# syamajala/cholesky

Measured on AMD Instinct MI355X. Metric: fp64 factorization GF/s (numeric level loop, F_ref flops) on 3-D Laplacian, higher is better.
Workload: dtype f64; 1 GPU; tests/lapl_3375x3375 (reference fixture: 7-point Laplacian, nested-dissection ordering from the fixture files); n=3375, levels=5, separators=31, B_alg_bytes=2932064, parallelism=single GPU, precision=fp64

## Files before the change

### cholesky_amd/_lib.py

```python
import ctypes as C
import os

_HERE = os.path.dirname(os.path.abspath(__file__))
LIB_PATH = os.environ.get("CHOLAMD_LIB") or os.path.join(_HERE, "lib", "libcholamd.so")
HEADER_PATH = os.path.join(os.path.dirname(_HERE), "include", "cholamd.h")


class Filled(C.Structure):
    _fields_ = [("filled", C.c_int), ("sep_x", C.c_int), ("sep_y", C.c_int), ("interval", C.c_int), ("cluster", C.c_int),
                ("lo_x", C.c_int), ("lo_y", C.c_int), ("hi_x", C.c_int), ("hi_y", C.c_int)]


class Op(C.Structure):
    _fields_ = [("op", C.c_int), ("level", C.c_int), ("m", C.c_int), ("n", C.c_int), ("k", C.c_int),
                ("a_sx", C.c_int), ("a_sy", C.c_int), ("a_z", C.c_int), ("b_sx", C.c_int), ("b_sy", C.c_int), ("b_z", C.c_int),
                ("c_sx", C.c_int), ("c_sy", C.c_int), ("c_z", C.c_int)]


class Region(C.Structure):
    _fields_ = [("ptr", C.c_void_p), ("ld", C.c_int), ("lo_x", C.c_int), ("lo_y", C.c_int), ("hi_x", C.c_int), ("hi_y", C.c_int),
                ("tile_row", C.POINTER(C.c_int))]


class SepInfo(C.Structure):
# ... 22 lines not shown
    L.cholamd_read_clusters.argtypes = [C.c_char_p, vp, vp, vp, i64, C.POINTER(i64)]
    L.cholamd_read_matrix.argtypes = [C.c_char_p, ci, vp, vp, vp]
    L.cholamd_read_vector.argtypes = [C.c_char_p, ci, vp]
    L.cholamd_write_solution.argtypes = [C.c_char_p, vp, ci, ci]
    L.cholamd_plan_create.argtypes = [C.c_char_p, C.c_char_p, C.c_char_p, C.POINTER(vp)]
    L.cholamd_plan_create_from_arrays.argtypes = [ci, ci, vp, vp, vp, vp, vp, i64, i64, vp, vp, vp, C.c_char_p, C.POINTER(vp)]
    L.cholamd_plan_destroy.argtypes = [vp]
    L.cholamd_generate_laplacian.argtypes = [ci, ci, ci, ci, ci, C.POINTER(vp)]
    L.cholamd_problem_destroy.argtypes = [vp]
    L.cholamd_problem_n.argtypes = [vp]
    L.cholamd_problem_nz.argtypes = [vp]
    L.cholamd_problem_write.argtypes = [vp, C.c_char_p]
    L.cholamd_plan_create_from_problem.argtypes = [vp, C.POINTER(vp)]
    L.cholamd_problem_rhs.argtypes = [vp, vp]
    for f in ("n", "nz", "levels", "num_separators", "max_int_size", "num_blocks"):
        getattr(L, "cholamd_plan_" + f).argtypes = [vp]
    for f in ("arena_doubles", "dropped_entries", "num_ops", "nnz_a", "nnz_l", "alg_bytes"):
        fn = getattr(L, "cholamd_plan_" + f)
        fn.argtypes = [vp]
        fn.restype = i64
    L.cholamd_plan_nnz_tiles.argtypes = [vp]
    L.cholamd_plan_nnz_tiles.restype = i64
    L.cholamd_plan_fmin.argtypes = [vp]
    L.cholamd_plan_fmin.restype = cd
    L.cholamd_plan_banner.argtypes = [vp]
    L.cholamd_plan_banner.restype = C.c_char_p
    for f in ("perm", "sep_sizes", "sep_offsets", "tree", "blocks", "ops"):
        getattr(L, "cholamd_plan_" + f).argtypes = [vp, vp]
    L.cholamd_plan_snapshot_count.argtypes = [vp, ci]
    L.cholamd_plan_snapshot_count.restype = i64
    L.cholamd_plan_snapshot.argtypes = [vp, ci, vp]
    L.cholamd_plan_counts.argtypes = [vp, ci, vp, vp]
    L.cholamd_plan_flops.argtypes = [vp]
    L.cholamd_plan_flops.restype = cd
    L.cholamd_plan_fill_host.argtypes = [vp, vp]
    L.cholamd_plan_arena_to_dense.argtypes = [vp, vp, vp]
    L.cholamd_plan_entries.argtypes = [vp, vp, vp]
    L.cholamd_plan_value_map.argtypes = [vp, vp]
    L.cholamd_plan_fill_host_values.argtypes = [vp, vp, i64, vp]
    L.cholamd_device_set_values.argtypes = [vp, vp, i64, ci, vp]
    L.cholamd_device_values_status.argtypes = [vp, vp, vp]
    L.cholamd_plan_fill_host_part.argtypes = [vp, vp, ci, ci, C.POINTER(i64)]
    L.cholamd_plan_level_work_counts.argtypes = [vp, ci, ci, ci, vp]
    L.cholamd_plan_level_work_volume.argtypes = [vp, ci, ci, ci, ci, vp]
    L.cholamd_plan_program_check.argtypes = [vp, ci, ci]
    L.cholamd_plan_program_check_opts.argtypes = [vp, ci, ci, ci, ci]
    L.cholamd_plan_program_counts.argtypes = [vp, ci, vp]
    L.cholamd_plan_program_jobs.argtypes = [vp, ci, i64, vp]
    L.cholamd_plan_program_jobs.restype = i64
    L.cholamd_plan_write_matrix.argtypes = [vp, vp, C.c_char_p, ci]
    L.cholamd_plan_write_debug_log.argtypes = [vp, vp]
    L.cholamd_device_create.argtypes = [vp, ci, C.POINTER(vp)]
    L.cholamd_device_destroy.argtypes = [vp]
    L.cholamd_device_set_partition.argtypes = [vp, ci, ci]
    L.cholamd_device_set_option.argtypes = [vp, C.c_char_p, ci]
    L.cholamd_comm_unique_id.argtypes = [vp]
    L.cholamd_comm_create.argtypes = [vp, ci, ci, vp, C.POINTER(vp)]
    L.cholamd_comm_create_local.argtypes = [vp, ci, vp]
    L.cholamd_factor_multi.argtypes = [vp, vp, vp, ci, vp]
    L.cholamd_gather_factor.argtypes = [vp, vp, ci, vp]
    L.cholamd_comm_adopt.argtypes = [vp, ci, ci, C.POINTER(vp)]
    L.cholamd_comm_destroy.argtypes = [vp]
    L.cholamd_comm_destroy.restype = None
    L.cholamd_comm_allreduce.argtypes = [vp, vp, i64, vp]
    L.cholamd_device_tail_offset.argtypes = [vp]
    L.cholamd_device_tail_offset.restype = i64
    L.cholamd_exchange_tail.argtypes = [vp, vp, vp, vp]
    L.cholamd_factor_sharded.argtypes = [vp, vp, vp, vp]
    L.cholamd_factor_sharded_f32.argtypes = [vp, vp, vp, vp]
    L.cholamd_gather_to_root.argtypes = [vp, vp, ci, vp, vp]
    L.cholamd_exchange_volume.argtypes = [vp, vp]
    L.cholamd_plan_exchange_volume.argtypes = [vp, ci, ci, ci, vp]
    L.cholamd_plan_exchange_pieces.argtypes = [vp, ci, ci, ci, vp]
    L.cholamd_plan_solve_counts.argtypes = [vp, ci, ci, ci, vp]
    L.cholamd_plan_solve_skips.argtypes = [vp, ci, vp, vp]
    L.cholamd_solve_sharded.argtypes = [vp, vp, vp, vp, vp, vp]
    L.cholamd_solve_sharded_f32.argtypes = [vp, vp, vp, vp, vp, vp]
    L.cholamd_solve_refine_sharded.argtypes = [vp, vp, vp, vp, ci, C.c_double, vp, vp, vp, vp]
    L.cholamd_solve_multi.argtypes = [vp, vp, vp, vp, vp, ci, vp]
    L.cholamd_solve_refine_multi.argtypes = [vp, vp, vp, vp, ci, C.c_double, vp, vp, vp, ci, vp]
    L.cholamd_follow_rounds.argtypes = [ci, ci, ci, vp, vp]
    L.cholamd_plan_program_followers.argtypes = [vp, i64, vp]
    L.cholamd_plan_program_followers.restype = i64
    L.cholamd_factor_multi_f32.argtypes = [vp, vp, vp, ci, vp]
    L.cholamd_gather_factor_f32.argtypes = [vp, vp, ci, vp]
    L.cholamd_device_alloc.argtypes = [vp, i64, C.POINTER(vp)]
    L.cholamd_device_free.argtypes = [vp, vp]
    L.cholamd_device_upload.argtypes = [vp, vp, vp, i64, vp]
    L.cholamd_device_download.argtypes = [vp, vp, vp, i64, vp]
    L.cholamd_device_sync.argtypes = [vp, vp]
    L.cholamd_device_fill.argtypes = [vp, vp, vp]
    L.cholamd_factor.argtypes = [vp, vp, vp]
    L.cholamd_factor_levels.argtypes = [vp, vp, ci, ci, vp]
    L.cholamd_device_program_trace.argtypes = [vp, vp, vp, i64, vp, C.POINTER(ci)]
    L.cholamd_debug_live_buffers.argtypes = []
    L.cholamd_debug_live_buffers.restype = i64
    L.cholamd_factor_info.argtypes = [vp, C.POINTER(ci)]
    L.cholamd_solve.argtypes = [vp, vp, vp, vp, vp]
    L.cholamd_device_fill_f32.argtypes = [vp, vp, vp]
    L.cholamd_factor_f32.argtypes = [vp, vp, vp]
    L.cholamd_factor_levels_f32.argtypes = [vp, vp, ci, ci, vp]
    L.cholamd_solve_f32.argtypes = [vp, vp, vp, vp, vp]
    L.cholamd_solve_refine.argtypes = [vp, vp, vp, vp, ci, cd, C.POINTER(ci), C.POINTER(cd), vp]
    L.cholamd_residual.argtypes = [vp, vp, vp, vp, C.POINTER(cd), vp]
    L.cholamd_solve_nrhs.argtypes = [vp, vp, vp, i64, vp, i64, ci, vp]
    L.cholamd_solve_nrhs_f32.argtypes = [vp, vp, vp, i64, vp, i64, ci, vp]
    L.cholamd_solve_refine_nrhs.argtypes = [vp, vp, vp, i64, vp, i64, ci, ci, cd, C.POINTER(ci), vp, vp]
    L.cholamd_apply.argtypes = [vp, vp, vp, vp]
    L.cholamd_apply_nrhs.argtypes = [vp, vp, i64, vp, i64, ci, vp]
    L.cholamd_plan_apply_host.argtypes = [vp, vp, vp, vp]
    for name in ("cholamd_solve_pcg", "cholamd_solve_pcg_f32"):
        getattr(L, name).argtypes = [vp, vp, vp, vp, ci, cd, ci, vp, vp, vp, vp]
    for name in ("cholamd_solve_pcg_nrhs", "cholamd_solve_pcg_nrhs_f32"):
        getattr(L, name).argtypes = [vp, vp, vp, i64, vp, i64, ci, ci, cd, ci, vp, vp, vp, vp]
    L.cholamd_solve_half.argtypes = [vp, vp, vp, vp, ci, vp]
    L.cholamd_solve_half_f32.argtypes = [vp, vp, vp, vp, ci, vp]
    L.cholamd_solve_half_nrhs.argtypes = [vp, vp, vp, i64, vp, i64, ci, ci, vp]
    L.cholamd_solve_half_nrhs_f32.argtypes = [vp, vp, vp, i64, vp, i64, ci, ci, vp]
    for name in ("cholamd_multiply_half", "cholamd_multiply_half_f32"):
        getattr(L, name).argtypes = [vp, vp, vp, vp, ci, vp]
    for name in ("cholamd_multiply", "cholamd_multiply_f32"):
        getattr(L, name).argtypes = [vp, vp, vp, vp, vp]
    for name in ("cholamd_factor_residual", "cholamd_factor_residual_f32"):
        getattr(L, name).argtypes = [vp, vp, vp, C.POINTER(cd), vp]
    for name in ("cholamd_multiply_half_nrhs", "cholamd_multiply_half_nrhs_f32"):
        getattr(L, name).argtypes = [vp, vp, vp, i64, vp, i64, ci, ci, vp]
    for name in ("cholamd_multiply_nrhs", "cholamd_multiply_nrhs_f32"):
        getattr(L, name).argtypes = [vp, vp, vp, i64, vp, i64, ci, vp]
    L.cholamd_plan_multiply_host.argtypes = [vp, vp, ci, vp, vp]
    L.cholamd_plan_multiply_host_nrhs.argtypes = [vp, vp, ci, vp, i64, vp, i64, ci]
    L.cholamd_plan_multiply_counts.argtypes = [vp, vp]
    L.cholamd_plan_solve_det_host.argtypes = [vp, vp, ci, vp, vp]
    L.cholamd_plan_solve_det_host_nrhs.argtypes = [vp, vp, ci, vp, i64, vp, i64, ci]
    L.cholamd_plan_solve_det_counts.argtypes = [vp, vp]
    L.cholamd_plan_solve_det_lists.argtypes = [vp, ci, vp, vp, vp]
    L.cholamd_factor_logdet.argtypes = [vp, vp, C.POINTER(cd), vp]
    L.cholamd_factor_logdet_f32.argtypes = [vp, vp, C.POINTER(cd), vp]
    L.cholamd_factor_diag.argtypes = [vp, vp, vp, vp]
    L.cholamd_factor_diag_f32.argtypes = [vp, vp, vp, vp]
    L.cholamd_plan_diag_list.argtypes = [vp, vp, vp, vp, vp, vp, vp]
    L.cholamd_selinv.argtypes = [vp, vp, vp, vp]
    L.cholamd_selinv_diag.argtypes = [vp, vp, vp, vp]
    L.cholamd_selinv_entries.argtypes = [vp, vp, vp, i64, vp]
    L.cholamd_plan_selinv_blocks.argtypes = [vp, ci]
    L.cholamd_plan_selinv_front.argtypes = [vp, ci, ci, ci, vp, vp, vp]
    L.cholamd_values_grad_pairs.argtypes = [vp, vp, i64, vp, i64, ci, cd, cd, vp, i64, vp]
    L.cholamd_values_grad_logdet.argtypes = [vp, vp, cd, cd, vp, i64, vp]
    L.cholamd_plan_values_grad_pairs_host.argtypes = [vp, vp, i64, vp, i64, ci, cd, cd, vp, i64]
    L.cholamd_plan_values_grad_logdet_host.argtypes = [vp, vp, cd, cd, vp, i64]
    L.cholamd_plan_duplicate_entries.argtypes = [vp]
    L.cholamd_plan_duplicate_entries.restype = i64
    L.cholamd_plan_schur_size.argtypes = [vp, ci]
    L.cholamd_plan_schur_dofs.argtypes = [vp, ci, vp]
    L.cholamd_plan_schur_list.argtypes = [vp, ci, i64, vp]
    L.cholamd_plan_schur_host.argtypes = [vp, ci, vp, vp, i64]
    L.cholamd_schur_factor.argtypes = [vp, vp, ci, vp]
    L.cholamd_schur.argtypes = [vp, vp, ci, vp, i64, vp]
    for f in (L.cholamd_schur_condense, L.cholamd_schur_condense_f32, L.cholamd_schur_expand, L.cholamd_schur_expand_f32):
        f.argtypes = [vp, vp, ci, vp, vp, vp, vp]
    for f in (L.cholamd_schur_condense_nrhs, L.cholamd_schur_condense_nrhs_f32, L.cholamd_schur_expand_nrhs, L.cholamd_schur_expand_nrhs_f32):
        f.argtypes = [vp, vp, ci, vp, i64, vp, i64, vp, i64, ci, vp]
    L.cholamd_device_schur_launches.argtypes = [vp, vp]
    L.cholamd_plan_schur_condense_host_nrhs.argtypes = [vp, ci, vp, vp, i64, vp, i64, vp, i64, ci]
    L.cholamd_plan_schur_expand_host_nrhs.argtypes = [vp, ci, vp, vp, i64, vp, i64, vp, i64, ci]
    L.cholamd_plan_schur_det_counts.argtypes = [vp, ci, vp]
    L.cholamd_plan_schur_det_lists.argtypes = [vp, ci, ci, vp, vp, vp]
# ... 66 lines not shown
```

### cholesky_amd/csrc/chol_api.cpp

```cpp
#include "chol_device.h"

int no_device_error()
{
  chol_set_error("no usable HIP device (libcholamd has no CPU fallback)");
  return CHOLAMD_ERR_NO_DEVICE;
}
bool ranges_overlap(const void *a, size_t na, const void *b, size_t nb)
{
  const char *pa = (const char *)a, *pb = (const char *)b;
  return pa < pb + nb && pb < pa + na;
}

extern "C" int cholamd_device_count(void)
{
  int n = 0;
  if (hipGetDeviceCount(&n) != hipSuccess) return 0;
  return n;
}

#define CHOL_POISON_GUARD ((size_t)64 << 10)
static bool poison_on()
{
  const char *e = std::getenv("CHOLAMD_POISON");
  return e && *e && atoi(e) != 0;
// ... 109 lines not shown
      d->prog_ready = d->n_job > 0;
    }
  }
  return 0;
}

extern "C" int cholamd_device_create(const cholamd_plan *plan, int device_id, cholamd_device **out)
{
  *out = nullptr;
  if (!plan) { chol_set_error("null plan"); return CHOLAMD_ERR_ARG; }
  int ndev = 0;
  if (hipGetDeviceCount(&ndev) != hipSuccess || ndev <= 0) return no_device_error();
  if (device_id < 0 || device_id >= ndev) { chol_set_error("device %d out of range (%d devices)", device_id, ndev); return CHOLAMD_ERR_NO_DEVICE; }
  HIPCHK(hipSetDevice(device_id));
  cholamd_device *d = new cholamd_device();
  d->plan = plan; d->dev = device_id;
  chol_sched_opts_from_env(&d->opt);
  { const char *e = getenv("CHOLAMD_SOLVE_REFERENCE_SHAPE"); d->solve_reference_shape = e && *e && atoi(e) != 0; }
  { const char *e = getenv("CHOLAMD_SOLVE_DETERMINISTIC"); d->solve_deterministic = e && *e && atoi(e) != 0; }
  { const char *e = getenv("CHOLAMD_SOLVE_DETERMINISTIC_BLOCK"); d->solve_deterministic_block = e && *e && atoi(e) != 0; }
  { const char *e = getenv("CHOLAMD_SCHUR_DETERMINISTIC"); d->schur_deterministic = e && *e && atoi(e) != 0; }
  { const char *e = getenv("CHOLAMD_MULTIPLY_NRHS_MIN"); d->multiply_nrhs_min = e && *e ? atoi(e) : 0; }
  int rc = build_levels(d);
  if (!rc) rc = d->ws.alloc((size_t)(plan->ws_doubles > 0 ? plan->ws_doubles : 1));
  if (!rc) rc = d->info.alloc_zero(4);
  if (!rc) rc = d->progress.alloc_zero((size_t)(plan->nsep + 2));
  if (!rc) rc = d->a_dst.upload(plan->a_dst, (size_t)plan->nnz_a);
  if (!rc) rc = d->a_val.upload(plan->a_val, (size_t)plan->nnz_a);
  if (!rc) rc = d->perm.upload(plan->perm, (size_t)plan->n);
  if (rc) { cholamd_device_destroy(d); return rc; }
  *out = d;
  return 0;
}

extern "C" void cholamd_device_destroy(cholamd_device *d)
{
  if (!d) return;
  (void)hipSetDevice(d->dev);
  for (auto &a : d->vmm) {
    (void)hipDeviceSynchronize();
    (void)hipMemUnmap(a.va, a.total);
    for (auto h : a.handles) (void)hipMemRelease(h);
    (void)hipMemAddressFree(a.va, a.total);
  }
  for (auto &t : d->tl) { d->pool.push_back(t.a); d->pool.push_back(t.b); }
  for (auto e : d->pool) (void)hipEventDestroy(e);
  delete d;
}

extern "C" int cholamd_device_set_partition(cholamd_device *d, int rank, int world)
{
  HIPCHK(hipSetDevice(d->dev));
  if (world < 1 || (world & (world - 1)) || rank < 0 || rank >= world || chol_split_level(world) > d->plan->levels - 1) {
    chol_set_error("bad partition: rank %d of %d for a %d-level tree", rank, world, d->plan->levels);
    return CHOLAMD_ERR_ARG;
  }
  d->rank = rank; d->world = world;
  free_solve_lists(d);
  return build_levels(d);
}

extern "C" int cholamd_device_bcast_phases(const cholamd_device *d)
{
  int n = 0;
  for (const level_dev &l : d->lv) for (const chol_phase &ph : l.phase) n += ph.kind == 6;
  return n;
}
extern "C" int cholamd_device_set_option(cholamd_device *d, const char *name, int value)
{
  HIPCHK(hipSetDevice(d->dev));
  const std::string n(name ? name : "");
  bool rebuild = true;
  if (n == "split_min") d->opt.split_min = value;
  else if (n == "split_nb") d->opt.split_nb = value;
  else if (n == "fuse") d->opt.fuse = value != 0;
  else if (n == "fuse_update_max") d->opt.fuse_update_max = value;
  else if (n == "mt_min_tiles") d->opt.mt_min_tiles = value;
  else if (n == "cells") d->opt.cells = value != 0;
  else if (n == "program") d->opt.program = value != 0;
  else if (n == "follow") d->opt.follow = value != 0;
  else if (n == "super_blocks") d->opt.super_blocks = value;
  else if (n == "follow_tail") d->opt.follow_tail = value;
  else if (n == "follow_tail_split") d->opt.follow_tail_split = value;
  else if (n == "staged") d->opt.staged = value != 0;
  else if (n == "fine_upd") d->opt.fine_upd = value != 0;
  else if (n == "skyline") d->opt.skyline = value != 0;
  else if (n == "merge_targets") d->opt.merge_targets = value != 0;
  else if (n == "leaf_envelope") d->opt.leaf_envelope = value != 0;
  else if (n == "trsm_wt_min") d->opt.trsm_wt_min = value < 0 ? 0 : value;
  else if (n == "stage_chunk") d->opt.stage_chunk = value < 0 ? 0 : value;
  else if (n == "dist_top") d->opt.dist_top = value;
  else if (n == "solve_reference_shape") { d->solve_reference_shape = value != 0; rebuild = false; }
  else if (n == "solve_deterministic") { d->solve_deterministic = value != 0; rebuild = false; }
  else if (n == "solve_deterministic_block") { d->solve_deterministic_block = value != 0; rebuild = false; }
  else if (n == "schur_deterministic") { d->schur_deterministic = value != 0; rebuild = false; }
  else if (n == "multiply_nrhs_min") { d->multiply_nrhs_min = value; rebuild = false; }
  else { chol_set_error("unknown option '%s'", n.c_str()); return CHOLAMD_ERR_ARG; }
  return rebuild ? build_levels(d) : 0;
}

extern "C" int cholamd_device_alloc(cholamd_device *d, int64_t doubles, double **dptr)
{
  HIPCHK(hipSetDevice(d->dev));
  HIPCHK(fp_malloc((void **)dptr, (size_t)doubles * sizeof(double)));
  return 0;
}
extern "C" int cholamd_device_free(cholamd_device *d, double *dptr)
{
  HIPCHK(hipSetDevice(d->dev));
  HIPCHK(hipFree(dptr));
  return 0;
}
extern "C" int cholamd_device_upload(cholamd_device *d, double *d_dst, const double *h_src, int64_t doubles, void *stream)
{
  HIPCHK(hipSetDevice(d->dev));
  HIPCHK(hipMemcpyAsync(d_dst, h_src, (size_t)doubles * sizeof(double), hipMemcpyHostToDevice, (hipStream_t)stream));
  HIPCHK(hipStreamSynchronize((hipStream_t)stream));
  return 0;
}
extern "C" int cholamd_device_download(cholamd_device *d, double *h_dst, const double *d_src, int64_t doubles, void *stream)
{
  HIPCHK(hipSetDevice(d->dev));
  HIPCHK(hipMemcpyAsync(h_dst, d_src, (size_t)doubles * sizeof(double), hipMemcpyDeviceToHost, (hipStream_t)stream));
  HIPCHK(hipStreamSynchronize((hipStream_t)stream));
  return 0;
}
extern "C" int cholamd_device_sync(cholamd_device *d, void *stream)
{
  HIPCHK(hipSetDevice(d->dev));
  HIPCHK(hipStreamSynchronize((hipStream_t)stream));
  return 0;
}

static void owned_ranges(const cholamd_device *d, std::vector<std::pair<int64_t, int64_t>> &out)
{
  const cholamd_plan *p = d->plan;
  out.clear();
  if (d->world <= 1 || d->rank == 0) { out.push_back({ 0, p->arena }); return; }
  for (int s = 1; s <= p->nsep; s++) {
    const int o = chol_owner_of(p, s, d->world);
    if (o >= 0 && o != d->rank) continue;
    const int64_t lo = p->panel_off[s], hi = s < p->nsep ? p->panel_off[s + 1] : p->arena;
    if (!out.empty() && out.back().second == lo) out.back().second = hi; else out.push_back({ lo, hi });
  }
}
static int clear_owned(cholamd_device *d, void *arena, size_t elem, hipStream_t st)
{
  bool sharded = false;
  for (const auto &v : d->vmm) if (v.va == arena) sharded = true;
  if (!sharded) { HIPCHK(hipMemsetAsync(arena, 0, (size_t)d->plan->arena * elem, st)); return 0; }
  std::vector<std::pair<int64_t, int64_t>> r;
  owned_ranges(d, r);
  for (auto &x : r) HIPCHK(hipMemsetAsync((char *)arena + (size_t)x.first * elem, 0, (size_t)(x.second - x.first) * elem, st));
  return 0;
}
#define CHOL_VMM_CHUNK ((size_t)2 << 20)
#define CHOL_VMM_SCRATCH ((size_t)64 << 20)
extern "C" int cholamd_device_alloc_arena(cholamd_device *d, int elem_bytes, void **dptr, int64_t *backed_bytes)
{
  HIPCHK(hipSetDevice(d->dev));
  if (elem_bytes != 4 && elem_bytes != 8) { chol_set_error("alloc_arena: element size %d", elem_bytes); return CHOLAMD_ERR_ARG; }
  const size_t full = (size_t)d->plan->arena * (size_t)elem_bytes;
  if (d->world <= 1 || d->rank == 0) {
    HIPCHK(fp_malloc(dptr, full > 0 ? full : 1));
    if (backed_bytes) *backed_bytes = (int64_t)full;
    return 0;
// ... 1880 lines not shown
```

### cholesky_amd/csrc/chol_kernels.hip

```cpp
#include <hip/hip_runtime.h>
#include <float.h>
#include <stdint.h>

#include "chol_plan.h"
#include "chol_kernels.h"

typedef double d4 __attribute__((ext_vector_type(4)));

__device__ __forceinline__ void lds_barrier()
{
  asm volatile("s_waitcnt lgkmcnt(0)\n\ts_barrier" ::: "memory");
}


template <bool PUB> __device__ __forceinline__ void gstore(double *p, double v)
{
  if (PUB) __hip_atomic_store(p, v, __ATOMIC_RELAXED, __HIP_MEMORY_SCOPE_AGENT);
  else *p = v;
}
template <bool PUB> __device__ __forceinline__ double gload(const double *p)
{
  if (PUB) return __hip_atomic_load(p, __ATOMIC_RELAXED, __HIP_MEMORY_SCOPE_AGENT);
  return *p;
}
// ... 727 lines not shown
{
  while (__builtin_amdgcn_readfirstlane(__hip_atomic_load(flag, __ATOMIC_RELAXED, __HIP_MEMORY_SCOPE_WORKGROUP)) < target)
    __builtin_amdgcn_s_sleep(1);
  asm volatile("" ::: "memory");
}
__device__ __forceinline__ int lds_wait_ge_v(int *flag, int target)
{
  int v;
  while ((v = __builtin_amdgcn_readfirstlane(__hip_atomic_load(flag, __ATOMIC_RELAXED, __HIP_MEMORY_SCOPE_WORKGROUP))) < target)
    __builtin_amdgcn_s_sleep(1);
  asm volatile("" ::: "memory");
  return v;
}
__device__ __forceinline__ void lds_wait_both_ge(int *pair, int target)
{
  for (;;) {
    const long long v = __hip_atomic_load((long long *)pair, __ATOMIC_RELAXED, __HIP_MEMORY_SCOPE_WORKGROUP);
    const int lo = __builtin_amdgcn_readfirstlane((int)v), hi = __builtin_amdgcn_readfirstlane((int)(v >> 32));
    if (lo >= target && hi >= target) break;
    __builtin_amdgcn_s_sleep(1);
  }
  asm volatile("" ::: "memory");
}
__device__ __forceinline__ void lds_set(int *flag, int value, int lane)
{
  asm volatile("s_waitcnt lgkmcnt(0)" ::: "memory");
  if (lane == 0) __hip_atomic_store(flag, value, __ATOMIC_RELAXED, __HIP_MEMORY_SCOPE_WORKGROUP);
}
__device__ __forceinline__ void lds_wait_set(int *flag, int *info, int lane)
{
  for (int it = 0; __builtin_amdgcn_readfirstlane(__hip_atomic_load(flag, __ATOMIC_RELAXED, __HIP_MEMORY_SCOPE_WORKGROUP)) == 0; ++it) {
    if (it >= (1 << 25)) { if (lane == 0) report_stall(info); break; }
    __builtin_amdgcn_s_sleep(1);
  }
  asm volatile("" ::: "memory");
}
__device__ __forceinline__ void lds_inc(int *cnt, int lane)
{
  asm volatile("s_waitcnt lgkmcnt(0)" ::: "memory");
  if (lane == 0) __hip_atomic_fetch_add(cnt, 1, __ATOMIC_RELAXED, __HIP_MEMORY_SCOPE_WORKGROUP);
}
template <bool PUB> __device__ __forceinline__ d4 load_tile(const double *A, int lda, int n, int ti, int tj, int r15, int g)
{
  const int row = ti * TS + r15;
  const bool rowok = row < n;
  const double *src = A + row + (int64_t)(tj * TS + g) * lda;
  d4 v;
#pragma unroll
  for (int q = 0; q < 4; ++q) {
    const int c = g + 4 * q, col = tj * TS + c;
    double e = (row == col) ? 1.0 : 0.0;
    if (rowok && col < n) e = (ti > tj || c <= r15) ? gload<PUB>(&src[(int64_t)(4 * q) * lda]) : 0.0;
    v[q] = e;
  }
  return v;
}
#define FOLLOW_SLOTS 4
#define FOLLOW_LOADS ((CHOL_FOLLOW_MAXT * TS * TS + RR_THREADS - 1) / RR_THREADS)
template <int SLEEP = 0>
__device__ __forceinline__ void wait_list(const chol_wait *__restrict__ wl, int n, const int *ctr, const int *__restrict__ ctr_total, int epoch, int lane, int *info)
{
  for (int b0 = 0; b0 < n; b0 += 64) {
    int c = 0, need = 0;
    const bool mine = b0 + lane < n;
    if (mine) { const chol_wait wt = wl[b0 + lane]; c = wt.ctr; need = wt.value + epoch * ctr_total[wt.ctr]; }
    for (int it = 0;; ++it) {
      const bool ok = !mine || __hip_atomic_load(&ctr[c], __ATOMIC_RELAXED, __HIP_MEMORY_SCOPE_AGENT) >= need;
      if (!__ballot(!ok)) break;
      if (it >= (1 << 21)) { if (lane == 0) report_stall(info); break; }
#ifndef WAIT_SLEEP
#define WAIT_SLEEP 32
#endif
      __builtin_amdgcn_s_sleep(SLEEP ? SLEEP : WAIT_SLEEP);
    }
  }
}
__device__ __forceinline__ bool wait_list_holds(const chol_wait *__restrict__ wl, int n, const int *ctr, const int *__restrict__ ctr_total, int epoch, int lane)
{
  bool ok = true;
  for (int b0 = 0; b0 < n; b0 += 64)
    if (b0 + lane < n) { const chol_wait wt = wl[b0 + lane]; ok = ok && __hip_atomic_load(&ctr[wt.ctr], __ATOMIC_RELAXED, __HIP_MEMORY_SCOPE_AGENT) >= wt.value + epoch * ctr_total[wt.ctr]; }
  return !__ballot(!ok);
}
struct follow_args { const chol_ext *ext; int n_ext; const int *ctr; const int *ctr_total; int epoch; const chol_wait *wl; int n_wl; unsigned long long *stamp, *xstamp; };
__device__ __forceinline__ int ext_ready(const follow_args &f, int from, int lane)
{
  bool ok = true;
  if (from + lane < f.n_ext) {
    const int c = f.ext[from + lane].ctr;
    ok = __hip_atomic_load(&f.ctr[c], __ATOMIC_RELAXED, __HIP_MEMORY_SCOPE_AGENT) - f.epoch * f.ctr_total[c] >= f.ext[from + lane].need;
  }
  const unsigned long long notok = __ballot(!ok);
  const int lead = notok ? __builtin_ctzll(notok) : 64;
  return min(from + lead, f.n_ext);
}
template <bool UPD, bool PUB, bool TR = false>
__device__ __forceinline__ void follow_external(const double *__restrict__ base, const follow_args f, int T, int n, double *sE, d4 (&tile)[11], d4 (&stage)[3],
                                                const int (&ijp)[12], int w, int lane, int tid, int *info, const double *A, int lda, int r15, int g, int *sReady)
{
  const int lp = lane;
  int buf = 0;
  int ready = 0, ng = 0;
  double va[FOLLOW_LOADS], vb[FOLLOW_LOADS];
#ifndef FOLLOW_OWN_SLEEP
#define FOLLOW_OWN_SLEEP 4
#endif
#ifndef FOLLOW_OWN_LAST_MAX
#define FOLLOW_OWN_LAST_MAX 0
#endif
  static_assert(CHOL_FOLLOW_PAIR_MAXT == RR_MAXT, "a pair of followed column tiles shares one LDS buffer of RR_MAXT tiles");
  const int own_at = f.n_ext <= FOLLOW_OWN_LAST_MAX ? f.n_ext : chol_follow_own_at(f.n_ext, T);
#define EXT_ROUND(I_) chol_follow_round(I_, f.n_ext, T)
#define EXT_LOAD(I_, V_)                                                                                             \
  {                                                                                                                  \
    const chol_ext xl_ = f.ext[I_];                                                                                  \
    const double *src_ = base + xl_.off;                                                                             \
    _Pragma("unroll") for (int it = 0; it < FOLLOW_LOADS; ++it) {                                                    \
      const int idx = tid + it * RR_THREADS;                                                                         \
      const int row = (idx >> 8) * TS + (idx & 15), col = (idx >> 4) & 15;                                           \
      V_[it] = (idx < T * TS * TS && row < n && col < xl_.ncol) ? gload<true>(&src_[row + (int64_t)col * xl_.ld]) : 0.0; \
    }                                                                                                                \
  }
#define EXT_LOAD_ROUND(I_)                                                                                           \
  {                                                                                                                  \
    EXT_LOAD(I_, va);                                                                                                \
    ng = EXT_ROUND(I_);                                                                                              \
    if (ng == 2) { EXT_LOAD((I_) + 1, vb); }                                                                         \
  }
#define EXT_UPDATE(acc_, ti_, tj_)                                                                                   \
  {                                                                                                                  \
    _Pragma("unroll") for (int st = 0; st < 4; ++st)                                                                 \
      acc_ = __builtin_amdgcn_mfma_f64_16x16x4f64(sB[(tj_) * (TS * TS) + st * 64 + lp], -sB[(ti_) * (TS * TS) + st * 64 + lp], acc_, 0, 0, 0); \
    if (G == 2) {                                                                                                    \
      _Pragma("unroll") for (int st = 0; st < 4; ++st)                                                               \
        acc_ = __builtin_amdgcn_mfma_f64_16x16x4f64(sB2[(tj_) * (TS * TS) + st * 64 + lp], -sB2[(ti_) * (TS * TS) + st * 64 + lp], acc_, 0, 0, 0); \
    }                                                                                                                \
  }
#define OWN_TILES()                                                                                                  \
  {                                                                                                                  \
  \
      if (!UPD) wait_list<FOLLOW_OWN_SLEEP>(f.wl, f.n_wl, f.ctr, f.ctr_total, f.epoch, lane, info);  \
      if (TR && !UPD && f.xstamp && lane == 0) f.xstamp[0] = __builtin_amdgcn_s_memrealtime(); \
      lds_barrier(); \
      if (UPD) { \
        int rx = r15, gx = g;  \
        asm volatile("" : "+v"(rx), "+v"(gx)); \
    _Pragma("unroll")                                                                                            \
        for (int it = 0; it < 3; ++it) { \
          const int u = min(w + it * RR_NW, 2 * T - 2); \
          stage[it] += load_tile<PUB>(A, lda, n, u < T ? u : u - T + 1, u < T ? 0 : 1, rx, gx); \
        } \
        __builtin_amdgcn_sched_barrier(0);  \
    _Pragma("unroll")                                                                                            \
        for (int s = 0; s < FOLLOW_SLOTS; ++s) \
          if (ijp[s] != 0xffff) tile[s] += load_tile<PUB>(A, lda, n, ijp[s] & 0xff, ijp[s] >> 8, rx, gx); \
        __builtin_amdgcn_sched_barrier(0); \
      } \
 \
  }
  for (int i = 0; i < f.n_ext;) {
    if (f.n_wl > 0 && i == own_at) OWN_TILES();
    if (ng == 0) {
      const int need = i + EXT_ROUND(i);
      if (ready < need) {
        if (!UPD) {
          ready = ext_ready(f, i, lane);
          for (int it = 0; ready < need; ++it) {
            if (it >= (1 << 24)) { if (lane == 0) report_stall(info); ready = f.n_ext; break; }
#ifndef EXT_SLEEP
#define EXT_SLEEP 4
#endif
            __builtin_amdgcn_s_sleep(EXT_SLEEP);
            ready = ext_ready(f, i, lane);
          }
          if (lane == 0) __hip_atomic_store(sReady, ready, __ATOMIC_RELAXED, __HIP_MEMORY_SCOPE_WORKGROUP);
        } else {
          for (int it = 0;; ++it) {
            ready = __builtin_amdgcn_readfirstlane(__hip_atomic_load(sReady, __ATOMIC_RELAXED, __HIP_MEMORY_SCOPE_WORKGROUP));
            if (ready >= need) break;
            if (it >= (1 << 25)) { if (lane == 0) report_stall(info); ready = f.n_ext; break; }
            __builtin_amdgcn_s_sleep(2);
          }
        }
      }
      EXT_LOAD_ROUND(i);
    }
    const int G = ng;
    if (TR && !UPD && f.xstamp && lane == 0 && i < 44) { f.xstamp[1] = f.n_ext; f.xstamp[2 + i] = __builtin_amdgcn_s_memrealtime(); }
    double *sB = sE + buf * (RR_MAXT * TS * TS), *sB2 = sB + T * TS * TS;
#pragma unroll
    for (int it = 0; it < FOLLOW_LOADS; ++it) {
      const int idx = tid + it * RR_THREADS;
      if (idx < T * TS * TS) { sB[idx] = va[it]; if (G == 2) sB2[idx] = vb[it]; }
    }
    const int j = i + G;
    ng = 0;
    int pv = 0, pneed = 0;
    bool polled = false;
    if (j < f.n_ext && j + EXT_ROUND(j) <= ready) { EXT_LOAD_ROUND(j); }
    else if (j < f.n_ext && !UPD) {
      polled = true;
      if (j + lane < f.n_ext) { const int c = f.ext[j + lane].ctr; pv = __hip_atomic_load(&f.ctr[c], __ATOMIC_RELAXED, __HIP_MEMORY_SCOPE_AGENT); pneed = f.epoch * f.ctr_total[c] + f.ext[j + lane].need; }
    }
    lds_barrier();
    if (UPD) {
#pragma unroll
      for (int it = 0; it < 3; ++it) {
        const int u = w + it * RR_NW;
        if (u < 2 * T - 1) { const int tj = u < T ? 0 : 1, ti = u < T ? u : u - T + 1; EXT_UPDATE(stage[it], ti, tj); }
      }
#pragma unroll
      for (int s = 0; s < FOLLOW_SLOTS; ++s)
        if (ijp[s] != 0xffff) { const int ti = ijp[s] & 0xff, tj = ijp[s] >> 8; EXT_UPDATE(tile[s], ti, tj); }
    }
    buf ^= 1;
    if (polled) {
      const unsigned long long notok = __ballot(j + lane < f.n_ext && pv < pneed);
      const int r2 = min(j + (notok ? __builtin_ctzll(notok) : 64), f.n_ext);
      if (r2 > ready) { ready = r2; if (lane == 0) __hip_atomic_store(sReady, ready, __ATOMIC_RELAXED, __HIP_MEMORY_SCOPE_WORKGROUP); }
    } else if (UPD && j < f.n_ext && ready < j + EXT_ROUND(j)) {
      const int r2 = __builtin_amdgcn_readfirstlane(__hip_atomic_load(sReady, __ATOMIC_RELAXED, __HIP_MEMORY_SCOPE_WORKGROUP));
      ready = r2 > ready ? r2 : ready;
    }
    i = j;
  }
  if (f.n_wl > 0 && own_at >= f.n_ext) OWN_TILES();
#undef OWN_TILES
#undef EXT_LOAD_ROUND
#undef EXT_ROUND
#undef EXT_UPDATE
#undef EXT_LOAD
}

template <bool PUB, bool FOLLOW = false, bool TR = false>
__device__ __forceinline__ void potrf_rr_body(double *__restrict__ base, double *__restrict__ ws, const chol_potrf_desc d, int *__restrict__ info,
                                              int *__restrict__ progress, int progress_base, double *smem, const unsigned char *__restrict__ sky, const follow_args fa = follow_args(), const int tid = threadIdx.x)
{
  double (*const sRaw)[TS * TS] = (double (*)[TS * TS])(smem);
  double (*const sSol)[RR_MAXT][TS * TS] = (double (*)[RR_MAXT][TS * TS])(smem + RR_OFF_SOL);
  double (*const sDg)[TS * TS] = (double (*)[TS * TS])(smem + RR_OFF_DG);
  double (*const sLW)[4 * TS][TS + 1] = (double (*)[4 * TS][TS + 1])(smem + RR_OFF_LW);
  double (*const sConv)[TS + 1] = (double (*)[TS + 1])(smem + RR_OFF_CONV);
  double (*const sOv)[TS * TS] = (double (*)[TS * TS])(smem + RR_OFF_OV);
  unsigned short *const sIJ = (unsigned short *)(smem + RR_OFF_IJ);
  int *const sFlag = (int *)(smem + RR_OFF_FLAG);
  unsigned char *const sKm = (unsigned char *)(smem + RR_OFF_KM);
  int *const sMask = (int *)(smem + RR_OFF_MASK);
  unsigned char *const sSky = (unsigned char *)(smem + RR_OFF_SKY);
  int *const fL = &sFlag[0], *const fP = &sFlag[1], *const cSol = &sFlag[2], *const cUpd = &sFlag[3];
  int *const cRaw = &sFlag[4];
  int *const fA = &sFlag[6];
  int *const fD = &sFlag[7];
  int *const f00 = &sFlag[8];

  double *A = base + d.a_off;
  double *W = ws + d.dinv_off;
  const int n = d.n, lda = d.lda;
  const int T = (n + TS - 1) / TS;
  const int ntl = T * (T + 1) / 2;
  const int lane = tid & 63;
  const int wave = __builtin_amdgcn_readfirstlane(tid >> 6);
  const int r15 = lane & 15, g = lane >> 4;
  const int lp0 = g * TS + r15;

#define PSTAMP(i_) do { if (TR && fa.xstamp && fa.n_ext == 0 && tid == 64) fa.xstamp[24 + (i_)] = __builtin_amdgcn_s_memrealtime(); } while (0)
  PSTAMP(0);
  d4 stage[3];
  const bool stage_early = !(FOLLOW && fa.n_ext > 0) && wave != 0;
  if (stage_early) {
#pragma unroll
    for (int it = 0; it < 3; ++it) {
      const int u = min(wave - 1 + it * RR_NW, 2 * T - 2);
      stage[it] = load_tile<PUB>(A, lda, n, u < T ? u : u - T + 1, u < T ? 0 : 1, r15, g);
    }
  }
  const unsigned char *const tab = d.tab > 0 ? sky - __builtin_offsetof(chol_potrf_desc, sky) + d.tab : nullptr;
  if (tab) {
    static_assert((RR_MAXT * RR_NW) % 1 == 0 && RR_THREADS >= RR_MAXT * RR_NW + RR_SLOTS * RR_NW / 2 + RR_SLOTS * RR_NW / 4, "one pass copies the tables");
    if (tid < RR_MAXT * RR_NW) sMask[tid] = ((const int *)(tab + CHOL_RR_TAB_MASK))[tid];
    else if (tid < RR_MAXT * RR_NW + RR_SLOTS * RR_NW / 2) ((int *)sIJ)[tid - RR_MAXT * RR_NW] = ((const int *)(tab + CHOL_RR_TAB_IJ))[tid - RR_MAXT * RR_NW];
    else if (tid < RR_MAXT * RR_NW + RR_SLOTS * RR_NW / 2 + RR_SLOTS * RR_NW / 4) ((int *)sKm)[tid - RR_MAXT * RR_NW - RR_SLOTS * RR_NW / 2] = ((const int *)(tab + CHOL_RR_TAB_KM))[tid - RR_MAXT * RR_NW - RR_SLOTS * RR_NW / 2];
  } else {
    for (int t = tid; t < RR_SLOTS * RR_NW; t += RR_THREADS) { sIJ[t] = (unsigned short)0xffff; sKm[t] = 0; }
    for (int t = tid; t < RR_MAXT * RR_NW; t += RR_THREADS) sMask[t] = 0;
  }
  if (tid < 24) sSky[tid] = sky[tid];
  if (tid < 10) sFlag[tid] = 0;
  if (tid < TS * TS) sConv[TS + (tid >> 4)][tid & 15] = (tid >> 4) == (tid & 15) ? 1.0 : 0.0;
  __syncthreads();
  PSTAMP(1);
  const int ntl2 = (T - 2) * (T - 1) / 2;
  if (!tab) {
  for (int t = tid + 2 * T - 1; t < ntl; t += RR_THREADS) {
    int ti, tj, ow, os;
    tile_of_index(t, T, ti, tj);
    rr_owner(ntl - 1 - t, ntl2, ow, os);
    sIJ[os * RR_NW + ow] = (unsigned short)(ti | (tj << 8));
    const int kmin = max(sky[min(ti, 23)], sky[min(tj, 23)]);
    sKm[os * RR_NW + ow] = kmin | (tj < sky[min(ti, 23)] ? CHOL_RR_KM_ZERO : 0);
    const int last = ti == tj ? tj - 2 : tj - 1;
    for (int k = min(kmin, last); k <= last; ++k) atomicOr(&sMask[k * RR_NW + ow], 1 << os);
  }
  for (int t = tid; t < T * T; t += RR_THREADS) {
    const int k = t / T, i = t % T;
    if (i >= k + 2 && sky[min(i, 23)] <= k) {
      const int hv = i % RR_NHEAVY;
      atomicOr(&sMask[k * RR_NW + hv + hv / 3], 1 << (i < k + 2 + RR_NHEAVY ? RR_M_SOLVE0 : RR_M_SOLVE1));
    }
  }
  __syncthreads();
  }
  PSTAMP(2);

  if (wave == 0) {
    __builtin_amdgcn_s_setprio(3);
    if (FOLLOW && fa.n_ext > 0) {
      d4 tdummy[RR_RSLOTS], sdummy[3];
      int idummy[RR_SLOTS];
      follow_external<false, PUB, TR>(base, fa, T, n, smem + RR_OFF_SOL, tdummy, sdummy, idummy, 0, lane, tid, info, A, lda, r15, g, &sFlag[5]);
      lds_barrier();
      if (TR && fa.stamp && lane == 0) *fa.stamp = __builtin_amdgcn_s_memrealtime();
    }
    __builtin_amdgcn_s_setprio(3);
    lds_wait_ge(f00, 1);
    d4 dk;
#pragma unroll
    for (int q = 0; q < 4; ++q) dk[q] = sDg[0][q * 64 + lp0];
    STAMP_DECL;
    POLL_DECL;
    for (int k = 0; k < T; ++k) {
      STAMPK(0);
      double a[TS], unused;
#pragma unroll
      for (int q = 0; q < 4; ++q) sConv[r15][g + 4 * q] = dk[q];
#pragma unroll
      for (int c = 0; c < TS; ++c) a[c] = sConv[lane & 31][c];
      const int cupd_early = __hip_atomic_load(cUpd, __ATOMIC_RELAXED, __HIP_MEMORY_SCOPE_WORKGROUP);
      STAMPK(1);
      if (TR && fa.xstamp && lane == 0 && k < 24) fa.xstamp[72 + k] = __builtin_amdgcn_s_memrealtime();
      const bool more = k + 1 < T;
      const int kn = more ? k + 1 : k;
      long long fl = 0;
      d4 raw, dn;
      const int bad = chol16_rows(a, unused, r15, [&]() {
        fl = __hip_atomic_load((long long *)fA, __ATOMIC_RELAXED, __HIP_MEMORY_SCOPE_WORKGROUP);
        asm volatile("" ::: "memory");
#pragma unroll
        for (int q = 0; q < 4; ++q) { raw[q] = sRaw[kn][q * 64 + lp0]; dn[q] = sDg[kn & 1][q * 64 + lp0]; }
      });
      STAMPK(2);
      if (bad && k * TS + bad <= n && lane == 0) {
        if (atomicCAS(&info[0], 0, d.col0 + k * TS + bad) == 0) info[1] = d.sep;
      }
      const int par = k & 1;
      if (__builtin_amdgcn_readfirstlane(cupd_early) < RR_NW * k) { POLL_ADD(2, 1); lds_wait_ge(cUpd, RR_NW * k); }
#pragma unroll
      for (int c = 0; c < TS; ++c) sLW[par][lane][c] = a[c];
      double wv[4];
#pragma unroll
      for (int st = 0; st < 4; ++st) wv[st] = sLW[par][TS + 4 * st + g][r15];
      lds_set(fL, k + 1, lane);
      STAMPK(3);
      if (!more) break;
      if (__builtin_amdgcn_readfirstlane((int)fl) < k + 1 || __builtin_amdgcn_readfirstlane((int)(fl >> 32)) < k + 1) {
        POLL_ADD(0, 1);
        lds_wait_both_ge(fA, k + 1);
#pragma unroll
        for (int q = 0; q < 4; ++q) { raw[q] = sRaw[k + 1][q * 64 + lp0]; dn[q] = sDg[(k + 1) & 1][q * 64 + lp0]; }
      }
      STAMPK(4);
      const d4 p = solve16(raw, wv);
#pragma unroll
      for (int q = 0; q < 4; ++q) sSol[par][k + 1][q * 64 + lp0] = p[q];
#pragma unroll
      for (int st = 0; st < 4; ++st) dn = __builtin_amdgcn_mfma_f64_16x16x4f64(p[st], -p[st], dn, 0, 0, 0);
      __builtin_amdgcn_sched_barrier(0);
      lds_set(fP, k + 1, lane);
      STAMPK(5);
      dk = dn;
      STAMPK(6);
    }
    STAMP_FLUSH;
    POLL_FLUSH;
    __builtin_amdgcn_s_setprio(0);
  } else {
    d4 tile[RR_RSLOTS];
    const int w = wave - 1;
    const int hw = rr_heavy_index(w);
    int ijp[RR_SLOTS];
#pragma unroll
    for (int s = 0; s < RR_SLOTS; ++s) ijp[s] = __builtin_amdgcn_readfirstlane((int)sIJ[s * RR_NW + w]);
    int kmn[RR_SLOTS];
#pragma unroll
    for (int s = 0; s < RR_SLOTS; ++s) kmn[s] = __builtin_amdgcn_readfirstlane((int)sKm[s * RR_NW + w]);
    unsigned zmask = 0;
#pragma unroll
    for (int s = 0; s < RR_SLOTS; ++s) { zmask |= (kmn[s] & CHOL_RR_KM_ZERO) ? 1u << s : 0u; kmn[s] &= CHOL_RR_KM_ZERO - 1; }
    PSTAMP(5);

    if (FOLLOW && fa.n_ext > 0) {
      const bool early = fa.n_wl == 0;
      const d4 zero4 = { 0.0, 0.0, 0.0, 0.0 };
#pragma unroll
      for (int it = 0; it < 3; ++it) {
        const int u = min(w + it * RR_NW, 2 * T - 2);
        stage[it] = zero4;
        if (early) stage[it] = load_tile<PUB>(A, lda, n, u < T ? u : u - T + 1, u < T ? 0 : 1, r15, g);
      }
#pragma unroll
      for (int s = 0; s < FOLLOW_SLOTS; ++s) {
        d4 v = zero4;
        if (early && ijp[s] != 0xffff) v = load_tile<PUB>(A, lda, n, ijp[s] & 0xff, ijp[s] >> 8, r15, g);
        tile[s] = v;
      }
      follow_external<true, PUB, TR>(base, fa, T, n, smem + RR_OFF_SOL, tile, stage, ijp, w, lane, tid, info, A, lda, r15, g, &sFlag[5]);
#pragma unroll
      for (int s = FOLLOW_SLOTS; s < RR_RSLOTS; ++s) tile[s] = zero4;
      lds_barrier();
    } else {
    PSTAMP(6);
#pragma unroll
    for (int s = 0; s < RR_RSLOTS; ++s) {
      d4 v = { 0.0, 0.0, 0.0, 0.0 };
      if (ijp[s] != 0xffff && !(zmask & (1u << s))) v = load_tile<PUB>(A, lda, n, ijp[s] & 0xff, ijp[s] >> 8, r15, g);
      tile[s] = v;
    }
    }
    PSTAMP(3);
#pragma unroll
    for (int it = 0; it < 3; ++it) {
      const int u = w + it * RR_NW;
      if (u < 2 * T - 1) {
        const int tj = u < T ? 0 : 1, ti = u < T ? u : u - T + 1;
        double *park = ti == tj ? &sDg[ti][0] : tj == 0 ? &sRaw[ti][0] : &sSol[1][ti][0];
#pragma unroll
        for (int q = 0; q < 4; ++q) park[q * 64 + lp0] = stage[it][q];
        if (u == 0) lds_set(f00, 1, lane);
        if (ti == 1) lds_set(tj == 0 ? fA : fD, 1, lane);
        if (tj == 0 && ti > 0) lds_inc(cRaw, lane);
      }
    }
    if (ijp[RR_RSLOTS] != 0xffff) {
      const d4 v = load_tile<PUB>(A, lda, n, ijp[RR_RSLOTS] & 0xff, ijp[RR_RSLOTS] >> 8, r15, g);
#pragma unroll
      for (int q = 0; q < 4; ++q) sOv[hw][q * 64 + lp0] = v[q];
    }
    lds_inc(cUpd, lane);
    PSTAMP(4);
    STAMP_DECL;
    POLL_DECL;
    for (int k = 0; k < T; ++k) {
      STAMPK(0);
      int lp = lp0;
      asm volatile("" : "+v"(lp));
      int k2 = k + 2;
      asm volatile("" : "+s"(k2));
      const int par = k & 1;
      const int mk = __builtin_amdgcn_readfirstlane(sMask[k * RR_NW + w]);
      POLL_WAIT(0, fL, k + 1);
      STAMPK(1);
      POLL_WAIT(1, cRaw, (k + 1) * (T - 1) - k * (k + 1) / 2);
      STAMPK(2);
      if (mk & ((1 << RR_M_SOLVE0) | (1 << RR_M_SOLVE1))) {
        const int i0 = k + 2 + ((hw + RR_NHEAVY - ((k + 2) % RR_NHEAVY)) % RR_NHEAVY), i1 = i0 + RR_NHEAVY;
        double wv[4];
#pragma unroll
        for (int st = 0; st < 4; ++st) wv[st] = sLW[par][TS + 4 * st + g][r15];
        double *const col = A + (int64_t)(k * TS + g) * lda;
        if (((mk >> RR_M_SOLVE0) & 3) == 3) {
          const int row0 = i0 * TS + r15, row1 = i1 * TS + r15;
          d4 raw0, raw1, x0 = { 0.0, 0.0, 0.0, 0.0 }, x1 = { 0.0, 0.0, 0.0, 0.0 };
#pragma unroll
          for (int q = 0; q < 4; ++q) { raw0[q] = sRaw[i0][q * 64 + lp]; raw1[q] = sRaw[i1][q * 64 + lp]; }
#pragma unroll
          for (int st = 0; st < 4; ++st) {
            x0 = __builtin_amdgcn_mfma_f64_16x16x4f64(wv[st], raw0[st], x0, 0, 0, 0);
            x1 = __builtin_amdgcn_mfma_f64_16x16x4f64(wv[st], raw1[st], x1, 0, 0, 0);
          }
#pragma unroll
          for (int q = 0; q < 4; ++q) {
            sSol[par][i0][q * 64 + lp] = x0[q];
            sSol[par][i1][q * 64 + lp] = x1[q];
            if (row0 < n) gstore<PUB>(&col[row0 + (int64_t)(4 * q) * lda], x0[q]);
            if (row1 < n) gstore<PUB>(&col[row1 + (int64_t)(4 * q) * lda], x1[q]);
          }
        } else {
          const int i = (mk & (1 << RR_M_SOLVE0)) ? i0 : i1;
          const int row = i * TS + r15;
          d4 raw, x = { 0.0, 0.0, 0.0, 0.0 };
#pragma unroll
          for (int q = 0; q < 4; ++q) raw[q] = sRaw[i][q * 64 + lp];
#pragma unroll
          for (int st = 0; st < 4; ++st) x = __builtin_amdgcn_mfma_f64_16x16x4f64(wv[st], raw[st], x, 0, 0, 0);
#pragma unroll
          for (int q = 0; q < 4; ++q) {
            sSol[par][i][q * 64 + lp] = x[q];
            if (row < n) gstore<PUB>(&col[row + (int64_t)(4 * q) * lda], x[q]);
          }
        }
      }
      STAMPK(3);
      lds_inc(cSol, lane);
      POLL_WAIT(2, cSol, RR_NW * (k + 1));
      STAMPK(4);
      if (k + 1 < T) POLL_WAIT(3, fP, k + 1);
      STAMPK(5);
      const double *const sS = &sSol[par][0][0];
      if (k == 0) {
        for (int i = 2 + w; i < T; i += RR_NW) {
          d4 acc;
#pragma unroll
          for (int q = 0; q < 4; ++q) acc[q] = sSol[1][i][q * 64 + lp];
          if (sSky[min(i, 23)] == 0) {
#pragma unroll
          for (int st = 0; st < 4; ++st)
            acc = __builtin_amdgcn_mfma_f64_16x16x4f64(sS[1 * (TS * TS) + st * 64 + lp], -sS[i * (TS * TS) + st * 64 + lp], acc, 0, 0, 0);
          }
#pragma unroll
          for (int q = 0; q < 4; ++q) sRaw[i][q * 64 + lp] = acc[q];
          lds_inc(cRaw, lane);
          if (i == 2) lds_set(fA, 2, lane);
        }
      }
// ... 367 lines not shown
  __shared__ double smem[RR_SMEM_DOUBLES];
  const int wave = __builtin_amdgcn_readfirstlane(threadIdx.x >> 6);
  const int lane = threadIdx.x & 63;
  const int grp = wave >> 2;
  const int n_tg = (n_trsm + 2) / 3;
  if ((int)blockIdx.x < n_potrf) {
    potrf_rr_body<true>(base, ws, pdescs[blockIdx.x], info, progress + blockIdx.x, progress_base, smem, pdescs[blockIdx.x].sky);
  } else if ((int)blockIdx.x < n_potrf + n_tg) {
    double (*sX)[3][TS * TS] = (double (*)[3][TS * TS])smem;
    const int id = ((int)blockIdx.x - n_potrf) * 3 + grp;
    chol_trsm_desc d = tdescs[min(id, n_trsm - 1)];
    if (id >= n_trsm) d.m = 0;
    trsm_rr_body<true, FUSED_SLOTS>(base, ws, d, sX[grp], wave & 3, lane, progress + d.flag, progress_base, info);
    if (n_task > 0) {
      asm volatile("s_waitcnt vmcnt(0)" ::: "memory");
      lds_barrier();
      if (threadIdx.x == 0) __hip_atomic_fetch_add(done, 1, __ATOMIC_RELAXED, __HIP_MEMORY_SCOPE_AGENT);
    }
  } else {
    double (*sAcc)[3][3][4][64] = (double (*)[3][3][4][64])smem;
    const int u = (int)blockIdx.x - n_potrf - n_tg;
    int round = 0;
    for (int t0 = u * 3; t0 < n_task; t0 += n_upd_wg * 3, ++round) {
      const int tid = t0 + grp;
      const bool live = tid < n_task;
      update_task_body<true>(base, tasks[live ? tid : t0], srcs, sAcc[round & 1][grp], wave & 3, lane, live, round == 0 ? done : nullptr, done_target, info);
    }
  }
}

#define PROG_XFLAGS 32
#define PROG_OFF_XFLAG (3 * RR_MAXT * TS * TS)
static_assert(PROG_XFLAGS >= 4 * ((CHOL_RR_MAXN / TS + 3) / 4) && PROG_XFLAGS >= 4 * FUSED_SLOTS && PROG_OFF_XFLAG + (3 * PROG_XFLAGS + 1) / 2 <= RR_SMEM_DOUBLES, "the strips' slots and flags fit the image");
static_assert(CHOL_RR_MAXN <= RR_MAXT * TS && CHOL_FUSE_MAXN <= CHOL_RR_MAXN, "one slot per column tile of the widest strip");
template <bool TR>
__global__ __launch_bounds__(RR_THREADS) void k_program(double *__restrict__ base, double *__restrict__ ws, const chol_job *__restrict__ jobs, int njobs,
                                                        const chol_wait *__restrict__ waits, const chol_potrf_desc *__restrict__ pdescs,
                                                        const chol_trsm_desc *__restrict__ tdescs, const chol_upd_task *__restrict__ tasks,
                                                        const chol_upd_src *__restrict__ srcs, const chol_ext *__restrict__ exts,
                                                        int *__restrict__ ctr, const int *__restrict__ ctr_total, int epoch, int *__restrict__ head, int head_base,
                                                        int *__restrict__ info, int *__restrict__ info_next, unsigned long long *__restrict__ trace)
{
  if (info_next && blockIdx.x == 0 && threadIdx.x == 0) { info_next[0] = 0; info_next[1] = 0; }
  __shared__ double smem[RR_SMEM_DOUBLES];
  __shared__ int s_job;
  const int wave_id = __builtin_amdgcn_readfirstlane(threadIdx.x >> 6);
  for (;;) {
#ifdef TID_PLAIN
    int tid = threadIdx.x;
#else
    int tid = wave_id * 64 + (int)__builtin_amdgcn_mbcnt_hi(~0u, __builtin_amdgcn_mbcnt_lo(~0u, 0u));
#endif
    asm volatile("" : "+v"(tid));
    const int wave = wave_id;
    const int lane = tid & 63;
    const int grp = wave >> 2;
    __syncthreads();
    if (tid == 0) s_job = atomicAdd(head, 1) - head_base;
    __syncthreads();
    const int j = s_job;
    if (j >= njobs) break;
    const chol_job jb = jobs[j];
    if (TR && trace && tid == 0) { trace[4 * j] = __builtin_amdgcn_s_memrealtime(); trace[4 * j + 3] = blockIdx.x; }
    int *const xflags = (int *)(smem + PROG_OFF_XFLAG);
    if (jb.kind == 1 && tid < 3 * PROG_XFLAGS) xflags[tid] = 0;
    bool fenced = false;
    chol_upd_task tpre;
    if (jb.kind == 2) {
      const int tk = jb.first + min(jb.mode == 0 ? wave : grp, jb.n - 1);
      tpre = tasks[tk];
      int touch = 0;
      for (int sx = tpre.src_begin; sx < tpre.src_end; ++sx) touch += srcs[sx].k;
      asm volatile("" :: "s"(touch));
    }
    if (jb.n_pre > 0 && !(jb.kind == 0 && jb.n_ext > 0)) {
      if (wave == 0) wait_list(waits + jb.wait_first, jb.n_pre, ctr, ctr_total, epoch, lane, info);
      lds_barrier();
      fenced = true;
    }
    if (TR && trace && tid == 0) trace[4 * j + 1] = __builtin_amdgcn_s_memrealtime();
    if (jb.kind == 0) {
      const chol_potrf_desc pd = pdescs[jb.first];
      follow_args fa;
      fa.ext = exts + jb.ext_first; fa.n_ext = jb.n_ext; fa.ctr = ctr; fa.ctr_total = ctr_total; fa.epoch = epoch; fa.wl = waits + jb.wait_first; fa.n_wl = jb.n_wait; fa.stamp = TR && trace ? &trace[4 * j + 1] : nullptr; fa.xstamp = TR && trace ? &trace[4 * njobs + CHOL_TRACE_X * j] : nullptr;
      potrf_rr_body<true, true, TR>(base, ws, pd, info, ctr + pd.ctr, epoch * ctr_total[pd.ctr], smem, pdescs[jb.first].sky, fa, tid);
    } else if (jb.kind == 1) {
      double (*sX)[RR_MAXT][TS * TS] = (double (*)[RR_MAXT][TS * TS])smem;
      chol_trsm_desc d = tdescs[jb.first + min(grp, jb.n - 1)];
      if (grp >= jb.n) d.m = 0;
      if (!fenced) lds_barrier();
      if (d.band > 0)
        trsm_rr_body<true, (CHOL_RR_MAXN / TS + 3) / 4, true, TR, true>(base, ws, d, sX[grp], wave & 3, lane, ctr + d.flag, epoch * ctr_total[d.flag], info, d.chan >= 0 ? ctr + d.chan : nullptr,
                                                                         TR && trace && grp == 0 ? &trace[4 * njobs + CHOL_TRACE_X * j] : nullptr, xflags + grp * PROG_XFLAGS);
      else
        trsm_rr_body<true, FUSED_SLOTS, false, TR, true>(base, ws, d, sX[grp], wave & 3, lane, ctr + d.flag, epoch * ctr_total[d.flag], info, d.chan >= 0 ? ctr + d.chan : nullptr,
                                                         TR && trace && grp == 0 ? &trace[4 * njobs + CHOL_TRACE_X * j] : nullptr, xflags + grp * PROG_XFLAGS);
    } else {
      stage_waits sw;
      sw.w = waits + jb.wait_first + jb.n_pre; sw.n = jb.n_wait - jb.n_pre; sw.ctr = ctr; sw.ctr_total = ctr_total; sw.epoch = epoch; sw.info = info;
      unsigned long long *const xs = TR && trace && wave == 0 ? &trace[4 * njobs + CHOL_TRACE_X * j] : nullptr;
      if (jb.mode == 0) {
        for (int t0 = jb.first; t0 < jb.first + jb.n; t0 += RR_NW + 1) {
          const int tk = t0 + wave;
          if (tk < jb.first + jb.n) update_task_wave<true, TR>(base, t0 == jb.first ? tpre : tasks[tk], srcs, lane, sw, xs);
        }
      } else {
        double (*sAcc)[3][3][4][64] = (double (*)[3][3][4][64])smem;
        int round = 0;
        for (int t0 = jb.first; t0 < jb.first + jb.n; t0 += 3, ++round) {
          const int tk = t0 + grp;
          const bool live = tk < jb.first + jb.n;
          update_task_body<true, TR>(base, t0 == jb.first ? tpre : tasks[live ? tk : t0], srcs, sAcc[round & 1][grp], wave & 3, lane, live, nullptr, 0, info, sw, xs);
        }
      }
    }
    if (jb.sig[0] >= 0) {
      asm volatile("s_waitcnt vmcnt(0)" ::: "memory");
      lds_barrier();
      if (tid == 0) {
        __hip_atomic_fetch_add(&ctr[jb.sig[0]], jb.sig_add, __ATOMIC_RELAXED, __HIP_MEMORY_SCOPE_AGENT);
        if (jb.sig[1] >= 0) __hip_atomic_fetch_add(&ctr[jb.sig[1]], jb.sig_add, __ATOMIC_RELAXED, __HIP_MEMORY_SCOPE_AGENT);
      }
    }
    if (TR && trace && tid == 0) trace[4 * j + 2] = __builtin_amdgcn_s_memrealtime();
  }
}

#define TW_MAXT ((CHOL_TRSM_W_MAXN + TS - 1) / TS)
template <int T, int NT> __device__ __forceinline__ void trsm_w_solve(d4 (&tile)[NT], const double *s0, double *__restrict__ B, int n, int ldb,
                                                              bool vrow, int r15, int g)
{
#pragma unroll
  for (int J = 0; J < T; ++J) {
    const double *sd = s0 + (J * T - J * (J - 1) / 2) * (TS * TS);
    double wv[4];
#pragma unroll
    for (int st = 0; st < 4; ++st) wv[st] = sd[st * 64];
    const d4 x = solve16(tile[J], wv);
    if (vrow) {
      int ro = r15;
      asm volatile("" : "+v"(ro));
#pragma unroll
      for (int q = 0; q < 4; ++q) {
        const int col = J * TS + g + 4 * q;
        if (J + 1 < T || col < n) B[ro + (int64_t)col * ldb] = x[q];
      }
    }
    double nx[4];
#pragma unroll
    for (int st = 0; st < 4; ++st) {
      nx[st] = -x[st];
      asm volatile("" : "+v"(nx[st]));
    }
#pragma unroll
    for (int j = J + 1; j < T; ++j) {
      d4 acc = tile[j];
#pragma unroll
      for (int st = 0; st < 4; ++st) acc = __builtin_amdgcn_mfma_f64_16x16x4f64(sd[(j - J) * (TS * TS) + st * 64], nx[st], acc, 0, 0, 0);
      tile[j] = acc;
    }
  }
}
__global__ __launch_bounds__(256) void k_trsm_w(double *__restrict__ base, const double *__restrict__ ws,
                                                const chol_trsm_desc *__restrict__ descs, int ndesc)
{
  __shared__ double sT[TW_MAXT * (TW_MAXT + 1) / 2][TS * TS];
  const int tid = threadIdx.x, lane = tid & 63;
// ... 1389 lines not shown
```

### cholesky_amd/csrc/chol_plan.h

```cpp
#ifndef CHOL_PLAN_H
#define CHOL_PLAN_H

#include <stdint.h>
#include "cholamd.h"

#ifdef __cplusplus
extern "C" {
#endif

#define CHOL_ENTRY_OUT 0
#define CHOL_ENTRY_IN 1
#define CHOL_ENTRY_DROPPED 2
#define CHOL_NB 16
#define CHOL_RR_MAXN 272
#ifndef CHOL_FOLLOW_ALL_MAXT
#define CHOL_FOLLOW_ALL_MAXT 4
#endif
#define CHOL_FOLLOW_TAIL 3
#define CHOL_FOLLOW_MAXT 10
#define CHOL32_TRSM_GROUP 16
#define CHOL32_MAXN 128

typedef struct {
  int n_int;
// ... 41 lines not shown
#define CHOL_RR_TAB_MASK 0
#define CHOL_RR_TAB_IJ (CHOL_RR_MAXT * CHOL_RR_NW * 4)
#define CHOL_RR_TAB_KM (CHOL_RR_TAB_IJ + CHOL_RR_SLOTS * CHOL_RR_NW * 2)
#define CHOL_RR_TAB_BYTES ((CHOL_RR_TAB_KM + CHOL_RR_SLOTS * CHOL_RR_NW + 15) / 16 * 16)
#ifdef __HIPCC__
#define CHOL_HD __host__ __device__ __forceinline__
#else
#define CHOL_HD static inline
#endif
CHOL_HD void chol_rr_tile_of_index(int idx, int T, int *ti, int *tj)
{
  int j = 0;
  while (j < T && idx >= T - j) { idx -= T - j; ++j; }
  if (j >= T) { *ti = -1; *tj = 1 << 20; } else { *ti = j + idx; *tj = j; }
}
CHOL_HD void chol_rr_owner(int idx, int ntl2, int *w, int *slot)
{
  if (ntl2 <= CHOL_RR_HEAVY_ONLY) { const int off = idx % CHOL_RR_NHEAVY; *w = off + off / 3; *slot = idx / CHOL_RR_NHEAVY; return; }
  const int cyc = idx / 51, pos = idx % 51;
  const int round = pos < 11 ? 0 : pos < 20 ? 1 : pos < 31 ? 2 : pos < 40 ? 3 : 4;
  const int off = pos - (round == 0 ? 0 : round == 1 ? 11 : round == 2 ? 20 : round == 3 ? 31 : 40);
  if (off < CHOL_RR_NHEAVY) {
    *w = off + off / 3;
    *slot = cyc * 5 + round;
  } else {
    *w = off == CHOL_RR_NHEAVY ? 3 : 7;
    *slot = cyc * 3 + round / 2;
  }
}
void chol_potrf_table(int n, const unsigned char *sky, unsigned char *out);

typedef struct {
  int64_t l_off;
  int64_t dinv_off;
  int64_t b_off;
  int n, ldl, m, ldb;
  int flag;
  int chan;
  int band, pad;
} chol_trsm_desc;

#define CHOL_TRSM_W_MAXN 64
#define CHOL_TRSM_WT_MAXN 144
#define CHOL_TRSM_WT_GROUP 12
#define CHOL_TRSM_WT_MIN 2048
#define CHOL_FUSE_MAXN 192
#define CHOL_FUSE_UPDATE_MAX 0
#define CHOL_TRSM_ROWS 16

typedef struct {
  int64_t a_off, b_off;
  int lda, ldb, k;
  int range;
  int stage, pad;
} chol_upd_src;

typedef struct {
  int64_t c_off;
  int ldc;
  short mv, nv;
  int lower;
  int src_begin, src_end;
  int ar, br;
  int blk;
} chol_upd_task;

typedef struct { int ctr, value; } chol_wait;
typedef struct {
  int kind;
  int first, n;
  int wait_first, n_wait;
  int sig[2], sig_add;
  int ext_first, n_ext;
  int mode, n_pre;
} chol_job;
typedef struct {
  int64_t off;
  int ld, ncol;
  int ctr, need;
} chol_ext;
#define CHOL_FOLLOW_PAIR_MAXT 17
#define CHOL_FOLLOW_SINGLE_TAIL 0
#define CHOL_FOLLOW_OWN_BEFORE 2
#if defined(__HIPCC__)
#define CHOL_HD __host__ __device__ __forceinline__
#else
#define CHOL_HD static inline
#endif
CHOL_HD int chol_follow_round(int i, int n_ext, int T)
{
  const int pair_lim = 2 * T <= CHOL_FOLLOW_PAIR_MAXT ? n_ext - CHOL_FOLLOW_SINGLE_TAIL : 0;
  return i + 1 < pair_lim ? 2 : 1;
}
CHOL_HD int chol_follow_own_at(int n_ext, int T)
{
  int own_at = 0;
  for (int i = 0; i < n_ext; i += chol_follow_round(i, n_ext, T))
    if (i <= n_ext - CHOL_FOLLOW_OWN_BEFORE) own_at = i;
  return own_at;
}

typedef struct {
  int n_job; chol_job *job;
  int n_wait; chol_wait *wait;
  int n_ext; chol_ext *ext;
  int n_ctr; int *ctr_total;
  int follow;
} chol_program;

typedef struct {
  int kind;
  int first, n, first2, n2, first3, n3;
} chol_phase;
typedef struct { int64_t off, count; int owner, heap; } chol_bcast;
static inline unsigned chol_top_contributors(int heap, int world)
{
  int d = 0, l = 0;
  while ((1 << d) < world) d++;
  while ((heap >> (l + 1)) > 0) l++;
  const int lo = (heap << (d - l)) - (1 << d), hi = ((heap + 1) << (d - l)) - (1 << d);
  unsigned m = 0u;
  for (int g = lo; g < hi; g++) m |= 1u << g;
  return m;
}

#define CHOL_DIST_MIN 1024
#define CHOL_MT_MIN_TILES 8192
typedef struct {
  int split_min, split_nb;
  int fuse;
  int fuse_update_max;
  int mt_min_tiles;
  int trsm_group;
  int trsm_wt_min;
  int cells;
  int program;
  int follow;
  int dist_top;
  int skyline;
  int stage_chunk;
  int fine_upd;
  int staged;
  int follow_tail_split;
  int follow_tail;
  int merge_targets;
  int leaf_envelope;
  int super_blocks;
} chol_sched_opts;
#define CHOL_SUPER_BLOCKS 3
#define CHOL_STAGE_CHUNK 0
void chol_sched_opts_default(chol_sched_opts *o);
void chol_sched_opts_from_env(chol_sched_opts *o);

#define CHOL_SPLIT_MIN 144
#ifndef CHOL_PROG_SPLIT_MIN
#define CHOL_PROG_SPLIT_MIN 176
#endif
#define CHOL_SPLIT_NB 144

typedef struct {
  int level;
  int n_phase; chol_phase *phase;
  int n_potrf; chol_potrf_desc *potrf;
  int n_trsm; chol_trsm_desc *trsm;
  int n_task; chol_upd_task *task;
  int n_task_mt; chol_upd_task *task_mt;
  int n_src; chol_upd_src *src;
  int n_bcast; chol_bcast *bcast;
} chol_level_work;

typedef struct {
  int64_t a_off; int n, lda; int x_off; int sep;
  int64_t dinv_off;
  int band;
} chol_trsv_desc;
typedef struct {
  int64_t a_off; int m, n, lda; int x_off, y_off;
  int c_lo;
} chol_gemv_desc;

struct cholamd_plan {
  int n, nz_file, levels, nsep, max_int_size;
  char banner[160];
  MM_typecode typecode;
  int *perm;
  int *iperm;
  int *sep_of_pos;
  int *sep_size, *sep_off;
  int *tree;
  int *heap_of, *level_of;
  chol_clusters *cl;
  int nblk; chol_block *blk;
  int *blk_index;
  int64_t *panel_off; int *panel_ld, *panel_rows;
  int compact;
  int64_t arena_dense;
  int64_t arena;
  int64_t ws_doubles;
  int64_t *dinv_off;
  int64_t nnz_a, dropped; int64_t *a_dst; double *a_val;
  int64_t *csr_ptr; int *csr_col; double *csr_val;
  int *e_row, *e_col, *a_src, *csr_src; unsigned char *e_cls;
  int64_t duplicates; int dup_first;
  int64_t *snap_n; cholamd_filled **snap;
  int64_t nops, cap_ops; cholamd_op *ops;
  int64_t calls[16][4]; double flops[16][4];
  int64_t nnz_l;
  int64_t nnz_tiles;
  double fmin;
};

int chol_values_grad_plan_ok(const struct cholamd_plan *p, int64_t count, const char *what);
int chol_plan_finish(struct cholamd_plan *p, int nz, const int *a_row, const int *a_col, const double *a_val);
const chol_block *chol_plan_block(const struct cholamd_plan *p, int r, int c);
int chol_ntiles(const struct cholamd_plan *p, int sep, int interval);
int chol_build_program(const struct cholamd_plan *p, const chol_sched_opts *opts, chol_level_work *w, chol_program *prog);
void chol_program_free(chol_program *prog);
int chol_program_check(const struct cholamd_plan *p, const chol_sched_opts *opts, int workers);
int chol_program_check_built(const struct cholamd_plan *p, const chol_sched_opts *opts, int workers, const chol_level_work *w, const chol_program *g);
int chol_build_level_work(const struct cholamd_plan *p, const chol_sched_opts *opts , int level, int rank, int world, chol_level_work *out);
void chol_level_work_free(chol_level_work *w);
int chol_owner_of(const struct cholamd_plan *p, int label, int world);
int chol_split_level(int world);
typedef struct {
  int n_trsv; chol_trsv_desc *trsv;
  int n_fw; chol_gemv_desc *fw;
  int n_grp; int *grp_start; int *grp_rows;
  int n_bw; chol_gemv_desc *bw; int *bw_start;
  int n_ifw; int *ifw;
  int n_ibw; int *ibw;
// ... 97 lines not shown
```

### cholesky_amd/csrc/chol_schedule.c

```c
#define _GNU_SOURCE
#include <stdlib.h>
#include <string.h>

#include "chol_plan.h"
#include "cholamd.h"

typedef struct cholamd_plan plan_t;
#define BIDX(p, r, c) ((p)->blk_index[(size_t)(r) * ((p)->nsep + 1) + (c)])

int chol_split_level(int world)
{
  int d = 0;
  while ((1 << d) < world) d++;
  return d;
}

int chol_owner_of(const plan_t *p, int label, int world)
{
  int d = chol_split_level(world), lvl = p->level_of[label];
  if (lvl < d) return -1;
  return (p->heap_of[label] >> (lvl - d)) - (1 << d);
}

typedef struct {
  int64_t key;
  int64_t seq;
  int64_t c_off, a_off, b_off;
  int ldc, lda, ldb, m, n, k, syrk;
  int bc, crow, ccol;
  int src_sep;
} upd_tuple;

typedef struct { int i, e, bc, crow, ccol, m, n, syrk; int64_t c_off; int ldc, dead; } tgt_group;
static int cmp_group_rows(const void *x, const void *y)
{
  const tgt_group *a = x, *b = y;
  if (a->bc != b->bc) return a->bc < b->bc ? -1 : 1;
  if (a->ccol != b->ccol) return a->ccol < b->ccol ? -1 : 1;
  if (a->n != b->n) return a->n < b->n ? -1 : 1;
  return a->crow < b->crow ? -1 : (a->crow > b->crow);
}
static int cmp_group_first(const void *x, const void *y)
{
  const tgt_group *a = x, *b = y;
  return a->i < b->i ? -1 : (a->i > b->i);
}
static int cmp_group_source(const void *x, const void *y, void *tu_)
{
  const tgt_group *a = x, *b = y;
  const upd_tuple *cmp_group_tu = tu_;
  const int sa = cmp_group_tu[a->i].src_sep, sb = cmp_group_tu[b->i].src_sep;
  if (sa != sb) return sa < sb ? -1 : 1;
  return a->i < b->i ? -1 : (a->i > b->i);
}
static int same_sources(const upd_tuple *tu, const tgt_group *a, const tgt_group *b, int dr, int dc);

static int cmp_tuple(const void *x, const void *y)
{
  const upd_tuple *a = x, *b = y;
  if (a->key != b->key) return a->key < b->key ? -1 : 1;
  return a->seq < b->seq ? -1 : (a->seq > b->seq);
}

static int same_sources(const upd_tuple *tu, const tgt_group *a, const tgt_group *b, int dr, int dc)
{
  if (a->e - a->i != b->e - b->i) return 0;
  for (int q = 0; q < a->e - a->i; q++) {
    const upd_tuple *x = &tu[a->i + q], *y = &tu[b->i + q];
    if (x->src_sep != y->src_sep || x->lda != y->lda || x->ldb != y->ldb || x->k != y->k || y->a_off != x->a_off + dr || y->b_off != x->b_off + dc) return 0;
  }
  return 1;
}

static void index_snapshot(const plan_t *p, int lbl, int64_t *first, int *count)
{
  for (int b = 0; b < p->nblk; b++) { first[b] = 0; count[b] = 0; }
  const cholamd_filled *v = p->snap[lbl];
  for (int64_t i = 0; i < p->snap_n[lbl]; i++) {
    int b = BIDX(p, v[i].sep_x, v[i].sep_y);
    if (count[b] == 0) first[b] = i;
    count[b]++;
  }
}

typedef struct { int64_t c_off; int ldc, m, n, syrk, src_begin, src_end, blk, ar0, br0; } upd_target;
typedef struct { chol_level_work *w; const chol_sched_opts *o; int force_fine; int cur_blk; const int *follow_lim;
  int dist_world, dist_rank; const struct cholamd_plan *dist_plan; int tgt_sep, tgt_col0; int cap_b;
  const int *sw_of;
  int cur_band; const int *bw_of;
  int cap_p, cap_t, cap_k, cap_km, cap_s, cap_ph; upd_target *pend; int n_pend, cap_pend; } builder;
static int env_int(const char *name, int dflt) { const char *e = getenv(name); return e && *e ? atoi(e) : dflt; }
void chol_sched_opts_default(chol_sched_opts *o)
{
  o->split_min = CHOL_SPLIT_MIN; o->split_nb = CHOL_SPLIT_NB; o->fuse = 1; o->fuse_update_max = CHOL_FUSE_UPDATE_MAX;
  o->mt_min_tiles = CHOL_MT_MIN_TILES; o->trsm_wt_min = CHOL_TRSM_WT_MIN; o->trsm_group = 0; o->cells = 1; o->program = 1; o->follow = 1; o->super_blocks = CHOL_SUPER_BLOCKS; o->dist_top = 2; o->follow_tail = CHOL_FOLLOW_TAIL; o->follow_tail_split = CHOL_FOLLOW_TAIL; o->staged = 1; o->fine_upd = 1; o->skyline = 1; o->stage_chunk = CHOL_STAGE_CHUNK; o->merge_targets = 1; o->leaf_envelope = 1;
}
void chol_sched_opts_from_env(chol_sched_opts *o)
{
  chol_sched_opts_default(o);
  o->split_min = env_int("CHOLAMD_SPLIT_MIN", o->split_min);
  o->split_nb = env_int("CHOLAMD_SPLIT_NB", o->split_nb);
  o->fuse = !env_int("CHOLAMD_NO_FUSE", 0);
  o->fuse_update_max = env_int("CHOLAMD_FUSE_UPDATE_MAX", o->fuse_update_max);
  o->mt_min_tiles = env_int("CHOLAMD_MT_MIN_TILES", o->mt_min_tiles);
  o->trsm_wt_min = env_int("CHOLAMD_TRSM_WT_MIN", o->trsm_wt_min);
  o->cells = !env_int("CHOLAMD_NO_CELLS", 0);
  o->program = !env_int("CHOLAMD_NO_PROGRAM", 0);
  o->follow = !env_int("CHOLAMD_NO_FOLLOW", 0);
  o->dist_top = env_int("CHOLAMD_DIST_TOP", o->dist_top);
  o->super_blocks = env_int("CHOLAMD_SUPER_BLOCKS", o->super_blocks);
  o->follow_tail = env_int("CHOLAMD_FOLLOW_TAIL", o->follow_tail);
  o->follow_tail_split = env_int("CHOLAMD_FOLLOW_TAIL_SPLIT", o->follow_tail_split);
  o->staged = !env_int("CHOLAMD_NO_STAGED", 0);
  o->fine_upd = !env_int("CHOLAMD_NO_FINE_UPD", 0);
  o->skyline = !env_int("CHOLAMD_NO_SKYLINE", 0);
  o->merge_targets = !env_int("CHOLAMD_NO_MERGE_TARGETS", 0);
  o->leaf_envelope = !env_int("CHOLAMD_NO_LEAF_ENVELOPE", 0);
  o->stage_chunk = env_int("CHOLAMD_STAGE_CHUNK", o->stage_chunk);
}
static int split_nb(const chol_sched_opts *o) { int v = o->split_nb; if (v > CHOL_RR_MAXN) v = CHOL_RR_MAXN; v = (v + 15) / 16 * 16; if (v < 16) v = 16; return v; }
static int pivot_blocks(const chol_sched_opts *o, int n) { return n > o->split_min || n > CHOL_RR_MAXN ? (n + split_nb(o) - 1) / split_nb(o) : 1; }
static int pivot_block_width(const chol_sched_opts *o, int n) { const int nb = pivot_blocks(o, n); return nb == 1 ? n : ((n + nb - 1) / nb + 15) / 16 * 16; }


static void push_phase_f(builder *B, int kind, int first, int n, int force);
static void push_phase(builder *B, int kind, int first, int n) { push_phase_f(B, kind, first, n, 0); }
static void push_phase_f(builder *B, int kind, int first, int n, int force)
{
  if (n <= 0 && !force) return;
  if (n < 0) n = 0;
  chol_level_work *w = B->w;
  if (w->n_phase == B->cap_ph) { B->cap_ph = B->cap_ph ? 2 * B->cap_ph : 16; w->phase = realloc(w->phase, B->cap_ph * sizeof(chol_phase)); }
  chol_phase ph = { kind, first, n, 0, 0, 0, 0 };
  w->phase[w->n_phase++] = ph;
}
void chol_potrf_table(int n, const unsigned char *sky, unsigned char *out)
{
  int *mask = (int *)(out + CHOL_RR_TAB_MASK);
  unsigned short *ij = (unsigned short *)(out + CHOL_RR_TAB_IJ);
  unsigned char *km = out + CHOL_RR_TAB_KM;
  memset(out, 0, CHOL_RR_TAB_BYTES);
  for (int t = 0; t < CHOL_RR_SLOTS * CHOL_RR_NW; t++) ij[t] = 0xffff;
  const int T = (n + CHOL_NB - 1) / CHOL_NB, ntl = T * (T + 1) / 2, ntl2 = (T - 2) * (T - 1) / 2;
  for (int t = 2 * T - 1; t < ntl; t++) {
    int ti, tj, ow, os;
    chol_rr_tile_of_index(t, T, &ti, &tj);
    chol_rr_owner(ntl - 1 - t, ntl2, &ow, &os);
    ij[os * CHOL_RR_NW + ow] = (unsigned short)(ti | (tj << 8));
    const int si = sky[ti < 23 ? ti : 23], sj = sky[tj < 23 ? tj : 23], kmin = si > sj ? si : sj;
    km[os * CHOL_RR_NW + ow] = (unsigned char)(kmin | (tj < si ? CHOL_RR_KM_ZERO : 0));
    const int last = ti == tj ? tj - 2 : tj - 1;
    for (int k = kmin < last ? kmin : last; k <= last; k++) mask[k * CHOL_RR_NW + ow] |= 1 << os;
  }
  for (int k = 0; k < T; k++)
    for (int i = k + 2; i < T; i++)
      if (sky[i < 23 ? i : 23] <= k) {
        const int hv = i % CHOL_RR_NHEAVY;
        mask[k * CHOL_RR_NW + hv + hv / 3] |= 1 << (i < k + 2 + CHOL_RR_NHEAVY ? CHOL_RR_M_SOLVE0 : CHOL_RR_M_SOLVE1);
      }
}
static void push_potrf(builder *B, chol_potrf_desc d)
{
  chol_level_work *w = B->w;
  if (w->n_potrf == B->cap_p) { B->cap_p = B->cap_p ? 2 * B->cap_p : 32; w->potrf = realloc(w->potrf, B->cap_p * sizeof(chol_potrf_desc)); }
  w->potrf[w->n_potrf++] = d;
}
static void push_trsm_run(builder *B, int64_t l_off, int64_t dinv_off, int64_t b_off, int n, int ld, int m, int flag)
{
  chol_level_work *w = B->w;
  for (int r0 = 0; r0 < m; r0 += CHOL_TRSM_ROWS) {
    if (w->n_trsm == B->cap_t) { B->cap_t = B->cap_t ? 2 * B->cap_t : 64; w->trsm = realloc(w->trsm, B->cap_t * sizeof(chol_trsm_desc)); }
    const int mm = m - r0 < CHOL_TRSM_ROWS ? m - r0 : CHOL_TRSM_ROWS;
    chol_trsm_desc td = { l_off, dinv_off, b_off + r0, n, ld, mm, ld, flag, -1, B->cur_band, 0 };
    w->trsm[w->n_trsm++] = td;
  }
}
static void pad_trsm_group(builder *B, int phase_first, int group, int64_t l_off, int64_t dinv_off, int64_t b_off, int n, int ld, int flag)
{
  chol_level_work *w = B->w;
  while ((w->n_trsm - phase_first) % group != 0) {
    if (w->n_trsm == B->cap_t) { B->cap_t = B->cap_t ? 2 * B->cap_t : 64; w->trsm = realloc(w->trsm, B->cap_t * sizeof(chol_trsm_desc)); }
    chol_trsm_desc td = { l_off, dinv_off, b_off, n, ld, 0, ld, flag, -1, B->cur_band, 0 };
    w->trsm[w->n_trsm++] = td;
  }
}
static int push_src(builder *B, chol_upd_src sd)
{
  chol_level_work *w = B->w;
  if (w->n_src == B->cap_s) { B->cap_s = B->cap_s ? 2 * B->cap_s : 256; w->src = realloc(w->src, B->cap_s * sizeof(chol_upd_src)); }
  w->src[w->n_src] = sd;
  return w->n_src++;
}
#ifndef MT_ORDER
#define MT_ORDER 8
#endif
// ... 656 lines not shown
          w->src[q].stage = st;
        }
        for (int a = tk->src_begin + 1; a < tk->src_end; a++) {
          const chol_upd_src x = w->src[a];
          int b = a - 1;
          while (b >= tk->src_begin && w->src[b].stage > x.stage) { w->src[b + 1] = w->src[b]; b--; }
          w->src[b + 1] = x;
        }
      }
    } else for (int t = i; t < e; t++) for (int q = w->task[t].src_begin; q < w->task[t].src_end; q++) w->src[q].stage = 0;
    const int hpc = p->heap_of[Bc->c] / 2;
    const int is_par = P->c_updp && Bc->r != Bc->c && hpc >= 1 && Bc->r == p->tree[hpc];
    j->sig[0] = c_upd[Bc->c]; j->sig[1] = Bc->r == Bc->c ? c_updd[Bc->c] : is_par ? P->c_updp[Bc->c] : -1; j->sig_add = 1;
    cnt_upd[Bc->c]++;
    if (Bc->r == Bc->c) cnt_updd[Bc->c]++;
    if (is_par) P->cnt_updp[Bc->c]++;
    i = e;
  }
}

static unsigned char **leaf_skylines(const plan_t *p)
{
  const int ns = p->nsep, L = p->levels;
  unsigned char **sky = calloc(ns + 1, sizeof(unsigned char *));
  int **first = calloc(ns + 1, sizeof(int *));
  for (int h = 1 << (L - 1); h <= ns; h++) {
    const int s = p->tree[h], n = p->sep_size[s];
    if (n <= 0) continue;
    first[s] = malloc(n * sizeof(int));
    for (int r = 0; r < n; r++) first[s][r] = r;
  }
  for (int64_t e = 0; e < p->nnz_a; e++) {
    const int64_t off = p->a_dst[e];
    int lo = 1, hi = ns;
    while (lo < hi) { const int mid = (lo + hi + 1) / 2; if (p->panel_off[mid] <= off) lo = mid; else hi = mid - 1; }
    const int s = lo;
    if (!first[s]) continue;
    const int64_t rel = off - p->panel_off[s];
    const int ld = p->panel_ld[s], row = (int)(rel % ld), col = (int)(rel / ld);
    if (row < p->sep_size[s] && col < first[s][row]) first[s][row] = col;
  }
  for (int s = 1; s <= ns; s++) {
    if (!first[s]) continue;
    const int n = p->sep_size[s], T = (n + CHOL_NB - 1) / CHOL_NB;
    sky[s] = malloc(T);
    for (int i = 0; i < T; i++) {
      int f = n;
      for (int r = i * CHOL_NB; r < n && r < (i + 1) * CHOL_NB; r++) if (first[s][r] < f) f = first[s][r];
      sky[s][i] = (unsigned char)(f / CHOL_NB);
    }
    free(first[s]);
  }
  free(first);
  return sky;
}
static void free_skylines(unsigned char **sky, int ns) { if (!sky) return; for (int s = 1; s <= ns; s++) free(sky[s]); free(sky); }
static int **leaf_row_first(const plan_t *p)
{
  const int ns = p->nsep, L = p->levels;
  int **first = calloc(ns + 1, sizeof(int *));
  for (int h = 1 << (L - 1); h <= ns; h++) {
    const int s = p->tree[h], n = p->sep_size[s], ld = p->panel_ld[s];
    if (n <= 0) continue;
    first[s] = malloc((size_t)ld * sizeof(int));
    for (int r = 0; r < ld; r++) first[s][r] = r < n ? r : n;
  }
  for (int64_t e = 0; e < p->nnz_a; e++) {
    const int64_t off = p->a_dst[e];
    int lo = 1, hi = ns;
    while (lo < hi) { const int mid = (lo + hi + 1) / 2; if (p->panel_off[mid] <= off) lo = mid; else hi = mid - 1; }
    const int s = lo;
    if (!first[s]) continue;
    const int64_t rel = off - p->panel_off[s];
    const int ld = p->panel_ld[s], row = (int)(rel % ld), col = (int)(rel / ld);
    if (col < first[s][row]) first[s][row] = col;
  }
  return first;
}

typedef struct { int64_t off; int ld, k, ctr, need; } early_src;
#ifndef EARLY_CHUNK
#define EARLY_CHUNK 2
#endif
static void emit_early_cells(pbuild *P, builder *B, const plan_t *p, int64_t c_off, int ldc, int lim, int blk, const early_src *es, int nes,
                             const int *c_upd, const int *c_updd, int *snap_upd, int *cnt_upd, int *cnt_updd)
{
  chol_level_work *w = B->w;
  int nst = 0, maxch = 0;
  for (int q = 0; q < nes; q++) if (es[q].k > 0) { const int ch = ((es[q].k + CHOL_NB - 1) / CHOL_NB + EARLY_CHUNK - 1) / EARLY_CHUNK; nst += ch; if (ch > maxch) maxch = ch; }
  if (nst == 0) return;
  int *sc = malloc(nst * sizeof(int)), *sn = malloc(nst * sizeof(int)), *sq = malloc(nst * sizeof(int)), *sch = malloc(nst * sizeof(int));
  nst = 0;
  for (int c = 0; c < maxch; c++)
    for (int q = 0; q < nes; q++) {
      if (es[q].k <= 0) continue;
      const int et = (es[q].k + CHOL_NB - 1) / CHOL_NB;
      if (c * EARLY_CHUNK >= et) continue;
      const int last = (c + 1) * EARLY_CHUNK < et ? (c + 1) * EARLY_CHUNK - 1 : et - 1;
      sc[nst] = es[q].ctr - (et - 1) + last; sn[nst] = es[q].need; sq[nst] = q; sch[nst] = c; nst++;
    }
  const int staged = B->o->staged;
  const int k0 = w->n_task, Tl = (lim + CHOL_NB - 1) / CHOL_NB;
  for (int I = 0; I < Tl; I++)
    for (int J = 0; J <= I; J++) {
      const int sb = w->n_src;
      for (int z = 0; z < nst; z++) {
        const early_src *e = &es[sq[z]];
        const int col0 = sch[z] * EARLY_CHUNK * CHOL_NB, kc = e->k - col0 < EARLY_CHUNK * CHOL_NB ? e->k - col0 : EARLY_CHUNK * CHOL_NB;
        chol_upd_src sd = { e->off + CHOL_NB * I + (int64_t)col0 * e->ld, e->off + CHOL_NB * J + (int64_t)col0 * e->ld, e->ld, e->ld, kc, 0, staged ? z + 1 : 0, 0 };
        push_src(B, sd);
      }
      if (w->n_task == B->cap_k) { B->cap_k = B->cap_k ? 2 * B->cap_k : 256; w->task = realloc(w->task, B->cap_k * sizeof(chol_upd_task)); }
      chol_upd_task *t = &w->task[w->n_task++];
      memset(t, 0, sizeof *t);
      t->c_off = c_off + CHOL_NB * I + (int64_t)(CHOL_NB * J) * ldc; t->ldc = ldc;
      t->mv = (short)(lim - CHOL_NB * I < CHOL_NB ? lim - CHOL_NB * I : CHOL_NB);
      t->nv = (short)(lim - CHOL_NB * J < CHOL_NB ? lim - CHOL_NB * J : CHOL_NB);
      t->lower = I == J;
      t->src_begin = sb; t->src_end = w->n_src;
      t->blk = blk;
    }
  const int col_sep = p->blk[blk].c;
  snap_upd[col_sep] = cnt_upd[col_sep];
  emit_update_jobs(P, B, p, k0, c_upd, c_updd, snap_upd, cnt_upd, cnt_updd, sc, sn, nst, staged ? sq : NULL);
  free(sc); free(sn); free(sq); free(sch);
}

static chol_sched_opts chol_program_opts(const chol_sched_opts *o)
{
  chol_sched_opts r = *o;
  if (r.split_min == CHOL_SPLIT_MIN && r.split_nb == CHOL_SPLIT_NB) r.split_min = CHOL_PROG_SPLIT_MIN;
  return r;
}
int chol_build_program(const plan_t *p, const chol_sched_opts *opts, chol_level_work *w, chol_program *pg)
{
  memset(w, 0, sizeof *w);
  memset(pg, 0, sizeof *pg);
  w->level = -1;
  chol_sched_opts dflt, prog;
  if (!opts) { chol_sched_opts_default(&dflt); opts = &dflt; }
  prog = chol_program_opts(opts); opts = &prog;
  builder Bd; memset(&Bd, 0, sizeof Bd); Bd.w = w; Bd.o = opts; Bd.force_fine = 1;
  builder *B = &Bd;
  pbuild Pd; memset(&Pd, 0, sizeof Pd); Pd.pg = pg;
  pbuild *P = &Pd;
  const int L = p->levels, ns = p->nsep;
  int rc = 0;
  unsigned char **sky = opts->skyline ? leaf_skylines(p) : calloc(ns + 1, sizeof(unsigned char *));
  int *bw_of = malloc((ns + 1) * sizeof(int)), *band_of = calloc(ns + 1, sizeof(int));
  for (int s = 1; s <= ns; s++) {
    const int n = p->sep_size[s];
    bw_of[s] = pivot_block_width(opts, n);
    if (sky[s] && n > CHOL_FUSE_MAXN && n <= CHOL_RR_MAXN && pivot_blocks(opts, n) > 1) {
      int band = 1;
      for (int i = 0; i * CHOL_NB < n; i++) if (i - sky[s][i] > band) band = i - sky[s][i];
      if (band <= 4) { bw_of[s] = n; band_of[s] = band; }
    }
  }
  B->bw_of = bw_of;
  int *sw_of = malloc((ns + 1) * sizeof(int));
  for (int s = 1; s <= ns; s++) {
    sw_of[s] = bw_of[s];
    if (band_of[s] && opts->staged && opts->stage_chunk > 0 && opts->stage_chunk * CHOL_NB < p->sep_size[s]) sw_of[s] = opts->stage_chunk * CHOL_NB;
  }
  B->sw_of = sw_of;
  for (int s = 1; s <= ns && !rc; s++) {
    const int bw = bw_of[s];
    if ((bw > CHOL_FUSE_MAXN && !band_of[s]) || bw > CHOL_RR_MAXN) { chol_set_error("program launch: pivot block of %d columns (separator %d) exceeds %d", bw, s, CHOL_FUSE_MAXN); rc = CHOLAMD_ERR_ARG; }
  }
  {
    double est = 0;
    for (int s = 1; s <= ns; s++) {
      const int n = p->sep_size[s], rows = p->panel_rows[s];
      if (n <= 0) continue;
      const int bw = bw_of[s], nbk = (n + bw - 1) / bw;
      for (int st = 0; st + 1 < nbk; st++) est += (double)((rows - (st + 1) * bw) / 16 + 1) * ((n - (st + 1) * bw) / 16 + 1);
      est += (double)(rows / 16 + 1) * (n / 16 + 1) * (L - 1 - p->level_of[s]);
    }
    if (est > 2.0 * PROG_MAX_TASKS) { chol_set_error("program launch: about %.0f update tasks", est); rc = CHOLAMD_ERR_ARG; }
  }
  if (rc) { free_skylines(sky, ns); free(bw_of); free(band_of); free(sw_of); return rc; }
  const int follow = opts->follow && opts->cells;
  pg->follow = follow;
  int64_t *first = malloc(p->nblk * sizeof(int64_t));
  int *count = malloc(p->nblk * sizeof(int));
  int *c_upd = malloc((ns + 1) * sizeof(int)), *c_updd = malloc((ns + 1) * sizeof(int));
  if (opts->fine_upd && opts->follow && opts->cells) { P->c_updp = malloc((ns + 1) * sizeof(int)); P->cnt_updp = calloc(ns + 1, sizeof(int)); }
  int *cnt_upd = calloc(ns + 1, sizeof(int)), *cnt_updd = calloc(ns + 1, sizeof(int)), *snap_upd = calloc(ns + 1, sizeof(int));
  int *nblk_of = calloc(ns + 1, sizeof(int));
  pblock **pb = calloc(ns + 1, sizeof(pblock *));
  int *follow_lim = calloc(p->nblk, sizeof(int));
  for (int s = 1; s <= ns; s++) {
    c_upd[s] = new_ctr(P, 0); c_updd[s] = new_ctr(P, 0);
    if (P->c_updp) P->c_updp[s] = new_ctr(P, 0);
    const int n = p->sep_size[s];
    const int bw = bw_of[s], nbk = n > 0 ? (n + bw - 1) / bw : 0;
    nblk_of[s] = nbk;
    pb[s] = calloc(nbk > 0 ? nbk : 1, sizeof(pblock));
    for (int st = 0; st < nbk; st++) {
      pblock *b = &pb[s][st];
      b->c0 = st * bw; b->nb = n - b->c0 < bw ? n - b->c0 : bw;
      b->potrf = -1; b->ch_below = b->ch_par = b->ch_rest = -1;
      b->c_prog = new_ctr(P, (b->nb + CHOL_NB - 1) / CHOL_NB);
      b->c_strips = new_ctr(P, 0);
    }
  }
  int *est_start = calloc(ns + 1, sizeof(int));
  for (int h = ns; h >= 1; h--) {
    int st0 = 0;
    for (int c = 2 * h; c <= 2 * h + 1 && c <= ns; c++) {
      const int k = p->tree[c];
      const int end = est_start[k] + (p->sep_size[k] + CHOL_NB - 1) / CHOL_NB;
      if (end > st0) st0 = end;
    }
    est_start[p->tree[h]] = st0;
  }
  #define EMIT_POTRF(s_, st_, ext_first_)                                                                        \
    do {                                                                                                          \
      pblock *b_ = &pb[s_][st_];                                                                                  \
      const int ld_ = p->panel_ld[s_];                                                                            \
      const int64_t diag_ = p->panel_off[s_] + b_->c0 + (int64_t)b_->c0 * ld_;                                    \
      const int64_t dinv_ = p->dinv_off[s_] + (int64_t)(b_->c0 / CHOL_NB) * CHOL_NB * CHOL_NB;                    \
      chol_potrf_desc pd_ = { diag_, dinv_, b_->nb, ld_, s_, b_->c0, b_->c_prog, 0, { 0 } };                      \
      if (sky[s_])                               \
        for (int i_ = 0; i_ * CHOL_NB < b_->nb && i_ < 24; i_++) {                                                \
          const int f_ = sky[s_][b_->c0 / CHOL_NB + i_] - b_->c0 / CHOL_NB;                                       \
          pd_.sky[i_] = (unsigned char)(f_ > 0 ? f_ : 0);                                                         \
        }                                                                                                         \
      push_potrf(B, pd_);                                                                                         \
      b_->potrf = w->n_potrf - 1;                                                                                 \
      const int wf_ = pg->n_wait;                                                                                 \
      add_wait(P, c_updd[s_], cnt_updd[s_]);                                                                      \
      chol_job *j_ = add_job(P, 0, b_->potrf, 1, wf_);                                                            \
      j_->ext_first = (ext_first_); j_->n_ext = pg->n_ext - (ext_first_);                                         \
      b_->emitted = 1;                                                                                            \
    } while (0)

  for (int level = L - 1; level >= 0 && !rc; level--) {
    const int lbl = L - 1 - level;
    index_snapshot(p, lbl, first, count);
    const cholamd_filled *snap = p->snap[lbl];
    const int h0 = 1 << level, h1 = (1 << (level + 1)) - 1;
    int *hs = malloc((h1 - h0 + 1) * sizeof(int)), nh = 0, steps = 0;
    for (int h = h0; h <= h1; h++) {
      const int s = p->tree[h];
      if (count[BIDX(p, s, s)] == 0 || p->sep_size[s] == 0) continue;
      hs[nh++] = h;
      if (nblk_of[s] > steps) steps = nblk_of[s];
    }
    for (int st = 0; st < steps; st++) {
      for (int q = 0; q < nh; q++) {
        const int s = p->tree[hs[q]];
        if (st < nblk_of[s] && !pb[s][st].emitted) EMIT_POTRF(s, st, pg->n_ext);
      }
      for (int q = 0; q < nh; q++) {
        const int h = hs[q], s = p->tree[h], n = p->sep_size[s], ld = p->panel_ld[s];
        if (st >= nblk_of[s]) continue;
        pblock *b = &pb[s][st];
        const int c0 = b->c0, nb = b->nb;
        const int64_t diag = p->panel_off[s] + c0 + (int64_t)c0 * ld;
        const int64_t dinv = p->dinv_off[s] + (int64_t)(c0 / CHOL_NB) * CHOL_NB * CHOL_NB;
        const int64_t colbase = (int64_t)c0 * ld;
        const int below = n - c0 - nb;
        const int t0 = w->n_trsm;
        B->cur_band = band_of[s];
        int nb1 = 0;
        if (below > 0) {
          nb1 = pb[s][st + 1].nb;
          const int fol = follow && (nb1 + CHOL_NB - 1) / CHOL_NB <= CHOL_FOLLOW_MAXT;
          if (fol) { b->ns_below = (nb1 + CHOL_TRSM_ROWS - 1) / CHOL_TRSM_ROWS; b->ch_below = new_ctr(P, b->ns_below); for (int e = 1; e < (nb + CHOL_NB - 1) / CHOL_NB; e++) new_ctr(P, b->ns_below); }
          push_trsm_run(B, diag, dinv, p->panel_off[s] + (c0 + nb) + colbase, nb, ld, nb1, b->c_prog);
          for (int i = w->n_trsm - (nb1 + CHOL_TRSM_ROWS - 1) / CHOL_TRSM_ROWS; i < w->n_trsm; i++) w->trsm[i].chan = fol ? b->ch_below : -1;
        }
        int par_lim = 0;
        const int hp = h / 2;
        if (hp >= 1 && follow) {
          const int par = p->tree[hp];
          if (nblk_of[par] > 0 && (pb[par][0].nb + CHOL_NB - 1) / CHOL_NB <= CHOL_FOLLOW_MAXT && count[BIDX(p, par, s)] > 0) {
            par_lim = pb[par][0].nb;
            const int tb = w->n_trsm;
            const int nstr = push_block_rows(B, p, par, s, 0, par_lim, snap, first, count, diag, dinv, nb, ld, colbase, b->c_prog, -2);
            if (nstr > 0) {
              b->ns_par = nstr; b->ch_par = new_ctr(P, nstr);
              for (int e = 1; e < (nb + CHOL_NB - 1) / CHOL_NB; e++) new_ctr(P, nstr);
              for (int i = tb; i < w->n_trsm; i++) w->trsm[i].chan = b->ch_par;
              b->par_off = p->blk[BIDX(p, par, s)].off + colbase;
            } else par_lim = 0;
          }
        }
        const int t_rest = w->n_trsm;
        if (below - nb1 > 0) push_trsm_run(B, diag, dinv, p->panel_off[s] + (c0 + nb + nb1) + colbase, nb, ld, below - nb1, b->c_prog);
        for (int ha = hp; ha >= 1; ha /= 2) {
          const int anc = p->tree[ha];
          if (BIDX(p, anc, s) < 0) continue;
          push_block_rows(B, p, anc, s, ha == hp ? par_lim : 0, p->sep_size[anc], snap, first, count, diag, dinv, nb, ld, colbase, b->c_prog, -1);
        }
        if (sw_of[s] < bw_of[s] && w->n_trsm > t_rest) {
          b->ns_rest = w->n_trsm - t_rest; b->ch_rest = new_ctr(P, b->ns_rest);
          for (int e = 1; e < (nb + CHOL_NB - 1) / CHOL_NB; e++) new_ctr(P, b->ns_rest);
          for (int i = t_rest; i < w->n_trsm; i++) w->trsm[i].chan = b->ch_rest;
        }
        B->cur_band = 0;
        b->n_groups = emit_trsm_jobs(P, B, t0, c_upd[s], cnt_upd[s], b->c_strips, b->ch_par, P->c_updp ? P->c_updp[s] : -1, P->c_updp ? P->cnt_updp[s] : 0, b->ch_below, c_updd[s], cnt_updd[s]);
        pg->ctr_total[b->c_strips] = b->n_groups;
      }
      for (int q = 0; q < nh; q++) {
        const int s = p->tree[hs[q]];
        if (st + 1 >= nblk_of[s] || pb[s][st].ch_below < 0) continue;
        const pblock *b = &pb[s][st];
        const int ld = p->panel_ld[s];
        ext_item *items = NULL; int nit = 0, capit = 0;
        const int64_t e_off = p->panel_off[s] + (b->c0 + b->nb) + (int64_t)b->c0 * ld;
        const int nb1 = pb[s][st + 1].nb, nt = (b->nb + CHOL_NB - 1) / CHOL_NB;
        int bt = 0;
        if (opts->follow_tail_split > 0 && (nb1 + CHOL_NB - 1) / CHOL_NB > CHOL_FOLLOW_ALL_MAXT && nt > opts->follow_tail_split) bt = nt - opts->follow_tail_split;
        if (bt > 0 && sky[s]) {
          int fmin = 1 << 20;
          for (int i = (b->c0 + b->nb) / CHOL_NB; i * CHOL_NB < b->c0 + b->nb + nb1; i++) if (sky[s][i] < fmin) fmin = sky[s][i];
          if (fmin - b->c0 / CHOL_NB >= bt) bt = 0;
        }
        if (bt > 0) {
          const early_src es = { e_off, ld, bt * CHOL_NB, b->ch_below + bt - 1, b->ns_below };
          emit_early_cells(P, B, p, p->panel_off[s] + (b->c0 + b->nb) + (int64_t)(b->c0 + b->nb) * ld, ld, nb1, BIDX(p, s, s), &es, 1, c_upd, c_updd, snap_upd, cnt_upd, cnt_updd);
        }
        const int ef = pg->n_ext;
        push_ext_items(&items, &nit, &capit, e_off, ld, b->nb, b->ch_below, b->ns_below, 0, bt);
        for (int i = 0; i < nit; i++) add_ext(P, items[i].x);
        free(items);
        EMIT_POTRF(s, st + 1, ef);
      }
      {
        memcpy(snap_upd, cnt_upd, (ns + 1) * sizeof(int));
        for (int q = 0; q < nh; q++) {
          const int h = hs[q], s = p->tree[h], n = p->sep_size[s], ld = p->panel_ld[s];
          if (st >= nblk_of[s]) continue;
          const pblock *b = &pb[s][st];
          const int c0 = b->c0, nb = b->nb, below = n - c0 - nb;
          if (below <= 0) continue;
          const int64_t colbase = (int64_t)c0 * ld;
          const int64_t x_piv = p->panel_off[s] + (c0 + nb) + colbase;
          const int hpp_ = h / 2, par_ = hpp_ >= 1 ? p->tree[hpp_] : -1, blkp_ = par_ >= 0 ? BIDX(p, par_, s) : -1;
          const int fast = P->c_updp && b->ch_par >= 0 && b->ch_below >= 0 && blkp_ >= 0 && count[blkp_] > 0;
          const int fast_cols = fast ? pb[s][st + 1].nb : 0;
          if (fast) {
            const chol_block *Bk = &p->blk[blkp_];
            const int plim = pb[par_][0].nb, kf0 = w->n_task, ntl_ = (nb + CHOL_NB - 1) / CHOL_NB;
            B->cur_blk = blkp_;
            int run_lo = -1, run_hi = -1;
            for (int q2 = 0; q2 <= count[blkp_]; q2++) {
              int a0 = -1, a1 = -1;
              if (q2 < count[blkp_]) {
                const cholamd_filled *f = &snap[first[blkp_] + q2];
                a0 = f->lo_x - Bk->lo_x; a1 = f->hi_x - Bk->lo_x + 1;
                if (a1 > plim) a1 = plim;
                if (a0 >= a1) continue;
                if (run_hi == a0) { run_hi = a1; continue; }
              }
              if (run_lo >= 0) {
                const int sb_ = w->n_src;
                for (int c = 0; c * EARLY_CHUNK < ntl_; c++) {
                  const int col0 = c * EARLY_CHUNK * CHOL_NB, kc = nb - col0 < EARLY_CHUNK * CHOL_NB ? nb - col0 : EARLY_CHUNK * CHOL_NB;
                  chol_upd_src sa = { chol_block_row(Bk, run_lo) + colbase + (int64_t)col0 * ld, x_piv + (int64_t)col0 * ld, ld, ld, kc, 0, opts->staged ? 2 * c + 2 : 0, 0 };
                  push_src(B, sa);
                }
                push_tasks(B, chol_block_row(Bk, run_lo) + (int64_t)(c0 + nb) * ld, ld, run_hi - run_lo, fast_cols, 0, sb_, w->n_src);
              }
              run_lo = a0; run_hi = a1;
            }
            flush_targets(B);
            int scf[2 * 32], snf[2 * 32], nwf = 0;
            for (int c = 0; c * EARLY_CHUNK < ntl_ && nwf < 62; c++) {
              const int last = (c + 1) * EARLY_CHUNK < ntl_ ? (c + 1) * EARLY_CHUNK - 1 : ntl_ - 1;
              scf[nwf] = b->ch_par + last; snf[nwf++] = b->ns_par;
              scf[nwf] = b->ch_below + last; snf[nwf++] = b->ns_below;
            }
            emit_update_jobs(P, B, p, kf0, c_upd, c_updd, snap_upd, cnt_upd, cnt_updd, scf, snf, nwf, opts->staged ? scf : NULL);
          }
          const int k0 = w->n_task;
          B->cur_blk = BIDX(p, s, s);
          if (b->ch_below >= 0) {
            const int nb1 = pb[s][st + 1].nb, r2 = below - nb1;
            if (r2 > 0) {
              const int64_t x2 = x_piv + nb1;
              chol_upd_src s1 = { x2, x_piv, ld, ld, nb, 0, 0, 0 }, s2 = { x2, x2, ld, ld, nb, 0, 0, 0 };
              const int i1 = push_src(B, s1);
              push_tasks(B, p->panel_off[s] + (c0 + nb + nb1) + (int64_t)(c0 + nb) * ld, ld, r2, nb1, 0, i1, i1 + 1);
              const int i2 = push_src(B, s2);
              push_tasks(B, p->panel_off[s] + (c0 + nb + nb1) + (int64_t)(c0 + nb + nb1) * ld, ld, r2, r2, 1, i2, i2 + 1);
            }
          } else {
            chol_upd_src sp = { x_piv, x_piv, ld, ld, nb, 0, 0, 0 };
            const int sidx = push_src(B, sp);
            push_tasks(B, p->panel_off[s] + (c0 + nb) + (int64_t)(c0 + nb) * ld, ld, below, below, 1, sidx, sidx + 1);
          }
          const int hpp = h / 2, hgp = h / 4;
          const int par = hpp >= 1 ? p->tree[hpp] : -1;
          const int blk_par = par >= 0 ? BIDX(p, par, s) : -1;
          const int blk_rest = hgp >= 1 && BIDX(p, p->tree[hgp], s) >= 0 ? BIDX(p, p->tree[hgp], s) : blk_par;
          const int fine = P->c_updp && b->ch_par >= 0 && blk_par >= 0 && count[blk_par] > 0;
          const int par_lim = fine ? pb[par][0].nb : 0;
          if (fine) {
            const chol_block *Bk = &p->blk[blk_par];
            B->cur_blk = blk_par;
            int run_lo = -1, run_hi = -1;
            for (int q2 = 0; q2 <= count[blk_par]; q2++) {
              int a0 = -1, a1 = -1;
              if (q2 < count[blk_par]) {
                const cholamd_filled *f = &snap[first[blk_par] + q2];
                a0 = f->lo_x - Bk->lo_x; a1 = f->hi_x - Bk->lo_x + 1;
                if (a1 > par_lim) a1 = par_lim;
                if (a0 >= a1) continue;
                if (run_hi == a0) { run_hi = a1; continue; }
              }
              if (run_lo >= 0 && below > fast_cols) {
                chol_upd_src sa = { chol_block_row(Bk, run_lo) + colbase, x_piv + fast_cols, ld, ld, nb, 0, 0, 0 };
                const int si = push_src(B, sa);
                push_tasks(B, chol_block_row(Bk, run_lo) + (int64_t)(c0 + nb + fast_cols) * ld, ld, run_hi - run_lo, below - fast_cols, 0, si, si + 1);
              }
              run_lo = a0; run_hi = a1;
            }
          }
          B->cur_blk = blk_rest;
          for (int ha = hpp; ha >= 1; ha /= 2) {
            const int anc = p->tree[ha], ba = BIDX(p, anc, s);
            if (ba < 0) continue;
            const chol_block *Bk = &p->blk[ba];
            const int lo = (fine && ha == hpp) ? par_lim : 0;
            int run_lo = -1, run_hi = -1;
            for (int q2 = 0; q2 <= count[ba]; q2++) {
              int a0 = -1, a1 = -1;
              if (q2 < count[ba]) {
                const cholamd_filled *f = &snap[first[ba] + q2];
                a0 = f->lo_x - Bk->lo_x; a1 = f->hi_x - Bk->lo_x + 1;
                if (a0 < lo) a0 = lo;
                if (a0 >= a1) continue;
                if (run_hi == a0) { run_hi = a1; continue; }
              }
              if (run_lo >= 0) {
                chol_upd_src sa = { chol_block_row(Bk, run_lo) + colbase, x_piv, ld, ld, nb, 0, 0, 0 };
                const int si = push_src(B, sa);
                push_tasks(B, chol_block_row(Bk, run_lo) + (int64_t)(c0 + nb) * ld, ld, run_hi - run_lo, below, 0, si, si + 1);
              }
              run_lo = a0; run_hi = a1;
            }
          }
          flush_targets(B);
          const int sc[1] = { b->c_strips }, sn[1] = { b->n_groups };
          emit_update_jobs(P, B, p, k0, c_upd, c_updd, snap_upd, cnt_upd, cnt_updd, sc, sn, 1, NULL);
        }
      }
    }
    if (level == 0) { free(hs); break; }
    memset(follow_lim, 0, p->nblk * sizeof(int));
    if (follow)
      for (int hp = h0 / 2; hp <= h1 / 2; hp++) {
        const int par = p->tree[hp];
        if (nblk_of[par] == 0 || pb[par][0].emitted || count[BIDX(p, par, par)] == 0) continue;
        int kids[2] = { p->tree[2 * hp], p->tree[2 * hp + 1] };
        if (p->sep_size[kids[0]] > p->sep_size[kids[1]]) { const int t = kids[0]; kids[0] = kids[1]; kids[1] = t; }
        const int ef = pg->n_ext;
        int all = 1;
        for (int c = 0; c < 2; c++)
          for (int st = 0; st < nblk_of[kids[c]]; st++)
            if (count[BIDX(p, par, kids[c])] > 0 && pb[kids[c]][st].ch_par < 0) all = 0;
        if (!all) continue;
        ext_item *items = NULL; int nit = 0, capit = 0;
        const int lim = pb[par][0].nb, wide = opts->follow_tail > 0 && (lim + CHOL_NB - 1) / CHOL_NB > CHOL_FOLLOW_ALL_MAXT;
        early_src es[2 * 32]; int nes = 0;
        for (int c = 0; c < 2; c++) {
          int total = 0;
          for (int st = 0; st < nblk_of[kids[c]]; st++) total += (pb[kids[c]][st].nb + CHOL_NB - 1) / CHOL_NB;
          const int bt = wide && total > opts->follow_tail ? total - opts->follow_tail : 0;
          int before = 0;
          for (int st = 0; st < nblk_of[kids[c]]; st++) {
            const pblock *b = &pb[kids[c]][st];
            const int nt = (b->nb + CHOL_NB - 1) / CHOL_NB;
            const int et = bt - before < 0 ? 0 : bt - before > nt ? nt : bt - before;
            if (b->ch_par >= 0) {
              if (et > 0 && nes < 64) { const early_src e1 = { b->par_off, p->panel_ld[kids[c]], et * CHOL_NB < b->nb ? et * CHOL_NB : b->nb, b->ch_par + et - 1, b->ns_par }; es[nes++] = e1; }
              push_ext_items(&items, &nit, &capit, b->par_off, p->panel_ld[kids[c]], b->nb, b->ch_par, b->ns_par, est_start[kids[c]] + before, et);
            }
            before += nt;
          }
        }
        if (nes > 0) {
          const chol_block *Bp = &p->blk[BIDX(p, par, par)];
          emit_early_cells(P, B, p, Bp->off, Bp->ld, lim, BIDX(p, par, par), es, nes, c_upd, c_updd, snap_upd, cnt_upd, cnt_updd);
        }
        qsort(items, nit, sizeof(ext_item), cmp_ext_item);
        for (int i = 0; i < nit; i++) add_ext(P, items[i].x);
        free(items);
        if (pg->n_ext == ef) continue;
        follow_lim[BIDX(p, par, par)] = pb[par][0].nb;
        EMIT_POTRF(par, 0, ef);
      }
    {
      int cap_u = 256, ntu = 0;
      upd_tuple *tu = malloc(cap_u * sizeof(upd_tuple));
      int64_t seq = 0;
      for (int q = 0; q < nh; q++) {
        const int h = hs[q], s = p->tree[h], n = p->sep_size[s];
        for (int hp = h / 2; hp >= 1; hp /= 2) {
          const int par = p->tree[hp], bb = BIDX(p, par, s);
          const chol_block *Bb = &p->blk[bb];
          for (int hg = hp; hg >= 1; hg /= 2) {
            const int gp = p->tree[hg], ba = BIDX(p, gp, s), bc = BIDX(p, gp, par);
            const chol_block *Ba = &p->blk[ba], *Bc = &p->blk[bc];
            for (int i = 0; i < count[ba]; i++) {
              const cholamd_filled *fa = &snap[first[ba] + i];
              for (int j = 0; j < count[bb]; j++) {
                const cholamd_filled *fb_ = &snap[first[bb] + j];
                if (gp == par && fb_->cluster > fa->cluster) continue;
                if (ntu == cap_u) { cap_u *= 2; tu = realloc(tu, cap_u * sizeof(upd_tuple)); }
                upd_tuple *u = &tu[ntu++];
                const int crow = fa->lo_x - Bc->lo_x, ccol = fb_->lo_x - Bc->lo_y;
                u->key = ((int64_t)bc << 40) | ((int64_t)crow << 20) | (int64_t)ccol;
                u->seq = seq++;
                u->c_off = chol_block_row(Bc, crow) + (int64_t)ccol * Bc->ld; u->ldc = Bc->ld;
                u->a_off = chol_block_row(Ba, fa->lo_x - Ba->lo_x); u->lda = Ba->ld;
                u->b_off = chol_block_row(Bb, fb_->lo_x - Bb->lo_x); u->ldb = Bb->ld;
                u->m = fa->hi_x - fa->lo_x + 1; u->n = fb_->hi_x - fb_->lo_x + 1; u->k = n;
                u->syrk = (gp == par && fb_->cluster == fa->cluster);
                u->bc = bc; u->crow = crow; u->ccol = ccol; u->src_sep = s;
              }
            }
          }
        }
      }
      qsort(tu, ntu, sizeof(upd_tuple), cmp_tuple);
      const int k0 = w->n_task;
      memcpy(snap_upd, cnt_upd, (ns + 1) * sizeof(int));
      int any_follow = 0;
      for (int b = 0; b < p->nblk; b++) any_follow |= follow_lim[b] > 0;
      if (any_follow && !tuples_are_small(opts, tu, ntu)) { chol_set_error("program launch: followers need the grid-cell extend-add"); rc = CHOLAMD_ERR_ARG; }
      if (!rc) {
        if (tuples_are_small(opts, tu, ntu) || any_follow) { B->follow_lim = follow_lim; emit_cell_tasks(B, p, tu, ntu); B->follow_lim = NULL; }
        else {
          for (int i = 0; i < ntu;) {
            int e = i + 1;
            while (e < ntu && tu[e].key == tu[i].key) e++;
            const int sb = w->n_src;
            for (int q = i; q < e; q++) { chol_upd_src sd = { tu[q].a_off, tu[q].b_off, tu[q].lda, tu[q].ldb, tu[q].k, 0, -(64 * tu[q].src_sep + 63) - 1, 0 }; push_src(B, sd); }
            B->cur_blk = tu[i].bc;
            push_tasks(B, tu[i].c_off, tu[i].ldc, tu[i].m, tu[i].n, tu[i].syrk, sb, w->n_src);
            i = e;
          }
          flush_targets(B);
        }
        typedef struct { int i, e, prio; } blk_range;
        int nrg = 0, caprg = 64;
        blk_range *rg = malloc(caprg * sizeof(blk_range));
        for (int i = k0; i < w->n_task;) {
          int e = i + 1;
          while (e < w->n_task && w->task[e].blk == w->task[i].blk) e++;
          const chol_block *Bc = &p->blk[w->task[i].blk];
          if (nrg == caprg) { caprg *= 2; rg = realloc(rg, caprg * sizeof(blk_range)); }
          rg[nrg].i = i; rg[nrg].e = e;
          rg[nrg].prio = (L - p->level_of[Bc->c]) * 4 * L + (Bc->r == Bc->c ? 0 : 1 + (p->level_of[Bc->c] - p->level_of[Bc->r]));
          nrg++;
          i = e;
        }
        for (int a = 1; a < nrg; a++) {
          blk_range t = rg[a];
          int b = a - 1;
          while (b >= 0 && rg[b].prio > t.prio) { rg[b + 1] = rg[b]; b--; }
          rg[b + 1] = t;
        }
        for (int q = 0; q < nrg; q++) {
          const int i = rg[q].i, e = rg[q].e;
          const chol_block *Bc = &p->blk[w->task[i].blk];
          const int hpar = p->heap_of[Bc->c], dl = level - p->level_of[Bc->c];
          int nsc = 0, capsc = 1;
          for (int hh = hpar << dl; hh < ((hpar + 1) << dl); hh++) capsc += nblk_of[p->tree[hh]] + 2 * ((p->sep_size[p->tree[hh]] + CHOL_NB - 1) / CHOL_NB);
          int *sc = malloc(capsc * sizeof(int)), *sn = malloc(capsc * sizeof(int)), *ssep = malloc(capsc * sizeof(int)), *sest = malloc(capsc * sizeof(int));
          for (int hh = hpar << dl; hh < ((hpar + 1) << dl); hh++) {
            const int s = p->tree[hh];
            int through = 0;
// ... 1 lines not shown
              const pblock *b = &pb[s][st];
              if (sw_of[s] < bw_of[s] && b->n_groups > 0) {
                const int nt = (b->nb + CHOL_NB - 1) / CHOL_NB, ct = sw_of[s] / CHOL_NB;
                for (int c = 0; c * ct < nt; c++) {
                  const int last = (c + 1) * ct < nt ? (c + 1) * ct - 1 : nt - 1;
                  if (b->ch_par >= 0) { sc[nsc] = b->ch_par + last; sn[nsc] = b->ns_par; ssep[nsc] = 64 * s + c; sest[nsc] = est_start[s] + last + 1; nsc++; }
                  if (b->ch_rest >= 0) { sc[nsc] = b->ch_rest + last; sn[nsc] = b->ns_rest; ssep[nsc] = 64 * s + c; sest[nsc] = est_start[s] + last + 1; nsc++; }
                }
                through += nt;
                continue;
              }
              through += (b->nb + CHOL_NB - 1) / CHOL_NB;
              if (b->n_groups > 0) { sc[nsc] = b->c_strips; sn[nsc] = b->n_groups; ssep[nsc] = 64 * s + st; sest[nsc] = est_start[s] + through; nsc++; }
            }
          }
          for (int a = 1; a < nsc; a++) {
            const int c0_ = sc[a], n0_ = sn[a], s0_ = ssep[a], e0_ = sest[a];
            int b = a - 1;
            while (b >= 0 && sest[b] > e0_) { sc[b + 1] = sc[b]; sn[b + 1] = sn[b]; ssep[b + 1] = ssep[b]; sest[b + 1] = sest[b]; b--; }
            sc[b + 1] = c0_; sn[b + 1] = n0_; ssep[b + 1] = s0_; sest[b + 1] = e0_;
          }
          const int keep = w->n_task;
          w->n_task = e;
          emit_update_jobs(P, B, p, i, c_upd, c_updd, snap_upd, cnt_upd, cnt_updd, sc, sn, nsc, opts->staged ? ssep : NULL);
          w->n_task = keep;
          free(ssep); free(sest);
          free(sc); free(sn);
        }
        free(rg);
      }
      free(tu);
    }
    free(hs);
    if (w->n_task > PROG_MAX_TASKS && !rc) { chol_set_error("program launch: more than %d update tasks", PROG_MAX_TASKS); rc = CHOLAMD_ERR_ARG; }
  }
  #undef EMIT_POTRF
  if (!rc && w->n_task_mt > 0) { chol_set_error("program launch: macro-tile update phases"); rc = CHOLAMD_ERR_ARG; }
  if (!rc && w->n_task > PROG_MAX_TASKS) { chol_set_error("program launch: %d update tasks", w->n_task); rc = CHOLAMD_ERR_ARG; }
  for (int s = 1; s <= ns; s++) { pg->ctr_total[c_upd[s]] = cnt_upd[s]; pg->ctr_total[c_updd[s]] = cnt_updd[s]; if (P->c_updp) pg->ctr_total[P->c_updp[s]] = P->cnt_updp[s]; }
  free(P->c_updp); free(P->cnt_updp); P->c_updp = P->cnt_updp = NULL;
  for (int s = 1; s <= ns; s++) free(pb[s]);
  free_skylines(sky, ns); free(bw_of); free(band_of); free(sw_of);
  free(est_start); free(pb); free(nblk_of); free(first); free(count); free(c_upd); free(c_updd); free(cnt_upd); free(cnt_updd); free(snap_upd); free(follow_lim);
  free(B->pend);
  if (rc) { chol_level_work_free(w); chol_program_free(pg); }
  return rc;
}


typedef struct { int64_t a, b, c, d; } quad;
static int cmp_quad(const void *x, const void *y) { return memcmp(x, y, sizeof(quad)); }
int chol_program_check(const plan_t *p, const chol_sched_opts *opts, int workers)
{
  chol_level_work w;
  chol_program g;
  int rc = chol_build_program(p, opts, &w, &g);
  if (rc) return rc;
  rc = chol_program_check_built(p, opts, workers, &w, &g);
  chol_level_work_free(&w);
  chol_program_free(&g);
  return rc;
}
int chol_program_check_built(const plan_t *p, const chol_sched_opts *opts, int workers, const chol_level_work *wp, const chol_program *gp)
{
  const chol_level_work w = *wp;
  const chol_program g = *gp;
  int rc = 0;
  int *val = calloc(g.n_ctr > 0 ? g.n_ctr : 1, sizeof(int));
  char *state = calloc(g.n_job > 0 ? g.n_job : 1, 1);
  int next = 0, running = 0, done = 0;
  while (done < g.n_job && !rc) {
    while (running < workers && next < g.n_job) { state[next++] = 1; running++; }
    int progressed = 0;
    for (int j = 0; j < next; j++) {
      if (state[j] != 1) continue;
      const chol_job *jb = &g.job[j];
      int ok = 1;
      for (int q = 0; q < jb->n_wait && ok; q++) {
        const chol_wait *wt = &g.wait[jb->wait_first + q];
        if (wt->ctr < 0 || wt->ctr >= g.n_ctr || wt->value > g.ctr_total[wt->ctr]) { chol_set_error("program job %d waits for %d on counter %d (total %d)", j, wt->value, wt->ctr, wt->ctr >= 0 && wt->ctr < g.n_ctr ? g.ctr_total[wt->ctr] : -1); rc = CHOLAMD_ERR_ARG; ok = 0; break; }
        if (val[wt->ctr] < wt->value) ok = 0;
      }
      if (rc) break;
      if (ok && jb->kind == 0)
        for (int x = 0; x < jb->n_ext && ok; x++) {
          const chol_ext *e = &g.ext[jb->ext_first + x];
          if (val[e->ctr] < e->need) ok = 0;
        }
      if (ok && jb->kind == 1 && val[w.trsm[jb->first].flag] < g.ctr_total[w.trsm[jb->first].flag]) ok = 0;
      if (!ok) continue;
      if (jb->kind == 0) val[w.potrf[jb->first].ctr] = g.ctr_total[w.potrf[jb->first].ctr];
      if (jb->kind == 1)
        for (int i = jb->first; i < jb->first + jb->n; i++)
          if (w.trsm[i].chan >= 0 && w.trsm[i].m > 0)
            for (int t = 0; t < (w.trsm[i].n + CHOL_NB - 1) / CHOL_NB; t++) val[w.trsm[i].chan + t]++;
      for (int q = 0; q < 2; q++) if (jb->sig[q] >= 0) val[jb->sig[q]] += jb->sig_add;
      state[j] = 2; running--; done++; progressed = 1;
    }
    if (!rc && !progressed && (running == workers || next == g.n_job)) {
      int j = 0;
      while (j < next && state[j] != 1) j++;
      chol_set_error("program dead-locks with %d resident workgroups: job %d (kind %d) can never run; %d of %d jobs done", workers, j, j < g.n_job ? g.job[j].kind : -1, done, g.n_job);
      rc = CHOLAMD_ERR_ARG;
    }
  }
  for (int c = 0; c < g.n_ctr && !rc; c++)
    if (val[c] != g.ctr_total[c]) { chol_set_error("program counter %d ends at %d, total %d", c, val[c], g.ctr_total[c]); rc = CHOLAMD_ERR_ARG; }
  free(val); free(state);
  if (!rc) {
    quad *a = NULL, *b = NULL;
    int64_t na = 0, nb = 0, ca = 0, cb = 0;
#define PUSHQ(V_, N_, C_, A_, B_, C2_, D_) do { if (N_ == C_) { C_ = C_ ? 2 * C_ : 4096; V_ = realloc(V_, C_ * sizeof(quad)); } quad q_ = { A_, B_, C2_, D_ }; V_[N_++] = q_; } while (0)
    for (int l = 0; l < p->levels && !rc; l++) {
      chol_level_work lw;
      chol_sched_opts lo = *opts; lo.leaf_envelope = 0;
      rc = chol_build_level_work(p, &lo, l, 0, 1, &lw);
      if (rc) break;
      for (int i = 0; i < lw.n_potrf; i++) for (int ct = 0; ct * CHOL_NB < lw.potrf[i].n; ct++) for (int r = ct * CHOL_NB; r < lw.potrf[i].n; r++) PUSHQ(a, na, ca, -1, lw.potrf[i].a_off + r + (int64_t)ct * CHOL_NB * lw.potrf[i].lda, 0, 0);
      for (int i = 0; i < lw.n_trsm; i++) for (int r = 0; r < lw.trsm[i].m; r++) for (int ct = 0; ct * CHOL_NB < lw.trsm[i].n; ct++) PUSHQ(a, na, ca, -1, lw.trsm[i].b_off + r + (int64_t)ct * CHOL_NB * lw.trsm[i].ldb, 0, 0);
      chol_level_work_free(&lw);
    }
    for (int i = 0; i < w.n_potrf; i++) for (int ct = 0; ct * CHOL_NB < w.potrf[i].n; ct++) for (int r = ct * CHOL_NB; r < w.potrf[i].n; r++) PUSHQ(b, nb, cb, -1, w.potrf[i].a_off + r + (int64_t)ct * CHOL_NB * w.potrf[i].lda, 0, 0);
    for (int i = 0; i < w.n_trsm; i++) for (int r = 0; r < w.trsm[i].m; r++) for (int ct = 0; ct * CHOL_NB < w.trsm[i].n; ct++) PUSHQ(b, nb, cb, -1, w.trsm[i].b_off + r + (int64_t)ct * CHOL_NB * w.trsm[i].ldb, 0, 0);
#undef PUSHQ
    if (!rc) {
      qsort(a, na, sizeof(quad), cmp_quad);
      qsort(b, nb, sizeof(quad), cmp_quad);
      if (na != nb || (na > 0 && memcmp(a, b, na * sizeof(quad)))) { chol_set_error("program pivot blocks / TRSM rows differ from the level lists (%lld vs %lld items)", (long long)nb, (long long)na); rc = CHOLAMD_ERR_ARG; }
    }
    free(a); free(b);
  }
  return rc;
}
int cholamd_plan_program_check(const cholamd_plan *p, int follow, int workers)
{
  chol_sched_opts o;
  chol_sched_opts_default(&o);
  o.follow = follow;
  return chol_program_check(p, &o, workers);
}
int cholamd_plan_program_check_opts(const cholamd_plan *p, int follow_tail, int split_min, int split_nb, int workers)
{
  chol_sched_opts o;
  chol_sched_opts_from_env(&o);
  if (follow_tail >= 0) o.follow_tail = follow_tail;
  if (split_min >= 0) o.split_min = split_min;
  if (split_nb >= 0) o.split_nb = split_nb;
  return chol_program_check(p, &o, workers);
}
int64_t cholamd_plan_program_jobs(const cholamd_plan *p, int follow, int64_t cap, int *out)
{
  chol_sched_opts o;
  chol_sched_opts_default(&o);
  o.follow = follow;
  chol_level_work w; chol_program g;
  if (chol_build_program(p, &o, &w, &g)) return -1;
  const int64_t need = (int64_t)8 * g.n_job + (int64_t)3 * g.n_wait + 1;
  if (cap >= need) {
    int64_t k = 0;
    for (int j = 0; j < g.n_job; j++) {
      const chol_job *jb = &g.job[j];
      int a = 0, b = 0;
      if (jb->kind == 0) { a = w.potrf[jb->first].sep; b = w.potrf[jb->first].col0; }
      else if (jb->kind == 1) { for (int i = 0; i < w.n_potrf; i++) if (w.potrf[i].ctr == w.trsm[jb->first].flag) { a = w.potrf[i].sep; b = w.potrf[i].col0; } }
      else { a = p->blk[w.task[jb->first].blk].c; b = p->blk[w.task[jb->first].blk].r; }
      out[k++] = jb->kind; out[k++] = a; out[k++] = b; out[k++] = jb->first; out[k++] = jb->n; out[k++] = jb->sig[0]; out[k++] = jb->kind == 1 ? w.trsm[jb->first].chan : jb->sig[1]; out[k++] = jb->n_wait;
    }
    for (int j = 0; j < g.n_job; j++)
      for (int q = 0; q < g.job[j].n_wait; q++) { out[k++] = j; out[k++] = g.wait[g.job[j].wait_first + q].ctr; out[k++] = g.wait[g.job[j].wait_first + q].value; }
    out[k++] = g.n_job;
  }
  chol_level_work_free(&w); chol_program_free(&g);
  return need;
}
int cholamd_follow_rounds(int n_ext, int tile_columns, int cap, int *rounds_out, int *own_at_out)
{
  int n = 0;
  for (int i = 0; i < n_ext; i += chol_follow_round(i, n_ext, tile_columns), n++)
    if (n < cap && rounds_out) rounds_out[n] = chol_follow_round(i, n_ext, tile_columns);
  if (own_at_out) *own_at_out = chol_follow_own_at(n_ext, tile_columns);
  return n;
}
int64_t cholamd_plan_program_followers(const cholamd_plan *p, int64_t cap, int *out)
{
  chol_sched_opts o;
  chol_sched_opts_default(&o);
  chol_level_work w; chol_program g;
  if (chol_build_program(p, &o, &w, &g)) return -1;
  int64_t n = 0;
  for (int j = 0; j < g.n_job; j++) {
    const chol_job *jb = &g.job[j];
    if (jb->kind != 0 || jb->n_ext <= 0) continue;
    if (4 * n + 3 < cap) { out[4 * n] = j; out[4 * n + 1] = jb->n_ext; out[4 * n + 2] = (w.potrf[jb->first].n + CHOL_NB - 1) / CHOL_NB; out[4 * n + 3] = jb->n_wait; }
    n++;
  }
  chol_level_work_free(&w); chol_program_free(&g);
  return n;
}
int cholamd_plan_program_counts(const cholamd_plan *p, int follow, int out[6])
{
  chol_sched_opts o;
  chol_sched_opts_default(&o);
  o.follow = follow;
  chol_level_work w; chol_program g;
  int rc = chol_build_program(p, &o, &w, &g);
  if (rc) return rc;
  int nf = 0;
  for (int j = 0; j < g.n_job; j++) nf += g.job[j].kind == 0 && g.job[j].n_ext > 0;
  out[0] = g.n_job; out[1] = nf; out[2] = w.n_task; out[3] = w.n_trsm; out[4] = g.n_ctr; out[5] = g.n_ext;
  chol_level_work_free(&w); chol_program_free(&g);
  return 0;
}

static int level_work_volume(const cholamd_plan *p, const chol_sched_opts *o, int level, int rank, int world, int64_t out[6], int64_t counts[3])
{
  chol_level_work w;
  int rc = chol_build_level_work(p, o, level, rank, world, &w);
  if (rc) return rc;
  memset(out, 0, 6 * sizeof(int64_t));
  if (counts) { counts[0] = w.n_task; counts[1] = w.n_task_mt; counts[2] = 0; for (int i = 0; i < w.n_trsm; i++) counts[2] += w.trsm[i].m > 0; }
  for (int i = 0; i < w.n_potrf; i++) out[0] += w.potrf[i].n;
  for (int i = 0; i < w.n_trsm; i++) out[1] += (int64_t)w.trsm[i].m * w.trsm[i].n;
  for (int pass = 0; pass < 2; pass++) {
    const chol_upd_task *T = pass ? w.task_mt : w.task;
    const int nt = pass ? w.n_task_mt : w.n_task;
    for (int i = 0; i < nt; i++) {
      const chol_upd_task *t = &T[i];
      int64_t full = 0;
      for (int c = 0; c < t->nv; c++) full += t->lower ? (t->mv - c > 0 ? t->mv - c : 0) : t->mv;
      for (int q = t->src_begin; q < t->src_end; q++) {
        const chol_upd_src *sd = &w.src[q];
        const int r0 = sd->range & 255, r1 = (sd->range >> 8) & 255, c0 = (sd->range >> 16) & 255, c1 = (sd->range >> 24) & 255;
        out[2] += (sd->range ? (int64_t)(r1 - r0) * (c1 - c0) : full) * sd->k;
      }
    }
  }
  out[3] = w.n_bcast;
  for (int i = 0; i < w.n_bcast; i++) { out[4] += w.bcast[i].count; out[5] = (int64_t)((uint64_t)out[5] * 1000003u + (uint64_t)w.bcast[i].off * 31u + (uint64_t)w.bcast[i].owner + 7u * (uint64_t)w.bcast[i].count);  }
  int nb6 = 0;
  for (int i = 0; i < w.n_phase; i++) if (w.phase[i].kind == 6) nb6 += w.phase[i].n;
  if (nb6 != w.n_bcast) { chol_set_error("internal: %d broadcast entries, %d in phases", w.n_bcast, nb6); rc = CHOLAMD_ERR_ARG; }
  chol_level_work_free(&w);
  return rc;
}
int cholamd_plan_level_work_volume(const cholamd_plan *p, int level, int rank, int world, int dist_top, int64_t out[6])
{
  chol_sched_opts o;
  chol_sched_opts_default(&o);
  o.dist_top = dist_top;
  return level_work_volume(p, &o, level, rank, world, out, NULL);
}
int cholamd_plan_level_work_volume_opts(const cholamd_plan *p, int level, int merge_targets, int mt_min_tiles, int64_t out[9])
{
  chol_sched_opts o;
  chol_sched_opts_default(&o);
  o.merge_targets = merge_targets != 0;
  o.leaf_envelope = 0;
  if (mt_min_tiles >= 0) o.mt_min_tiles = mt_min_tiles;
  return level_work_volume(p, &o, level, 0, 1, out, out + 6);
}

int cholamd_plan_exchange_volume(const cholamd_plan *p, int rank, int world, int dist_top, int64_t out[4])
{
  chol_sched_opts o;
  chol_sched_opts_default(&o);
  o.dist_top = dist_top;
  const int d = chol_split_level(world);
  if (world < 1 || (1 << d) != world || d > p->levels - 1 || rank < 0 || rank >= world) { chol_set_error("bad partition rank %d of %d", rank, world); return CHOLAMD_ERR_ARG; }
  out[0] = out[1] = out[3] = 0;
  out[2] = world > 1 ? p->arena - p->panel_off[p->nsep - (world - 1) + 1] : 0;
  for (int lvl = d - 1; lvl >= 0; lvl--) {
    chol_level_work w;
    int rc = chol_build_level_work(p, &o, lvl, rank, world, &w);
    if (rc) return rc;
    for (int i = 0; i < w.n_bcast; i++) {
      out[3]++;
      const unsigned c = chol_top_contributors(w.bcast[i].heap, world);
      if (w.bcast[i].owner == rank) out[0] += w.bcast[i].count * __builtin_popcount(c & ~(1u << rank));
      else if (c & (1u << rank)) out[1] += w.bcast[i].count;
    }
// ... 1389 lines not shown
```

### cholesky_amd/plan.py

```python
import ctypes as C
import os

import numpy as np

from ._lib import Filled, Op, check, load

OP_NAMES = ("POTRF", "TRSM", "SYRK", "GEMM")


class Plan:
    def __init__(self, matrix_file=None, separator_file=None, clusters_file=None, _handle=None):
        self.L = load()
        if _handle is not None:
            self.h = _handle
        else:
            h = C.c_void_p()
            check(self.L.cholamd_plan_create(os.fsencode(matrix_file), os.fsencode(separator_file), os.fsencode(clusters_file), C.byref(h)),
                  "cholamd_plan_create")
            self.h = h
        g = self.L
        self.n = g.cholamd_plan_n(self.h)
        self.nz = g.cholamd_plan_nz(self.h)
        self.levels = g.cholamd_plan_levels(self.h)
        self.nsep = g.cholamd_plan_num_separators(self.h)
# ... 152 lines not shown
        a = np.zeros(self.arena_doubles, dtype=np.float64)
        tail = C.c_int64(0)
        check(self.L.cholamd_plan_fill_host_part(self.h, a.ctypes.data, rank, world, C.byref(tail)), "cholamd_plan_fill_host_part")
        return a, tail.value

    def level_work_counts(self, level, rank=0, world=1):
        out = np.zeros(4, dtype=np.int32)
        check(self.L.cholamd_plan_level_work_counts(self.h, level, rank, world, out.ctypes.data), "cholamd_plan_level_work_counts")
        return tuple(int(v) for v in out)

    def exchange_volume(self, rank, world, dist_top=2):
        out = np.zeros(4, dtype=np.int64)
        check(self.L.cholamd_plan_exchange_volume(self.h, rank, world, dist_top, out.ctypes.data), "cholamd_plan_exchange_volume")
        return tuple(int(v) for v in out)

    def solve_counts(self, level, rank=0, world=1):
        out = np.zeros(5, dtype=np.int64)
        check(self.L.cholamd_plan_solve_counts(self.h, level, rank, world, out.ctypes.data), "cholamd_plan_solve_counts")
        return tuple(int(v) for v in out)

    def solve_skips(self, level):
        cnt = self.solve_counts(level)
        seps = np.zeros((max(cnt[0], 1), 3), dtype=np.int32)
        runs = np.zeros((max(cnt[1], 1), 5), dtype=np.int32)
        check(self.L.cholamd_plan_solve_skips(self.h, level, seps.ctypes.data, runs.ctypes.data), "cholamd_plan_solve_skips")
        return seps[:cnt[0]], runs[:cnt[1]]

    def diag_list(self):
        m = self.nsep
        a_off = np.zeros(m, dtype=np.int64)
        cols, lda, x_off, sep = (np.zeros(m, dtype=np.int32) for _ in range(4))
        prefix = np.zeros(m + 1, dtype=np.int32)
        n = self.L.cholamd_plan_diag_list(self.h, a_off.ctypes.data, cols.ctypes.data, lda.ctypes.data, x_off.ctypes.data, sep.ctypes.data, prefix.ctypes.data)
        if n < 0:
            check(n, "cholamd_plan_diag_list")
        return a_off[:n], cols[:n], lda[:n], x_off[:n], sep[:n], prefix[:n + 1]

    SELINV_BLOCK = 64
    SELINV_FRONT_MAX = 8192

    def selinv_blocks(self, sep):
        n = self.L.cholamd_plan_selinv_blocks(self.h, int(sep))
        if n < 0:
            check(n, "cholamd_plan_selinv_blocks")
        return n

    def selinv_front(self, sep, block):
        cols = np.zeros(2, dtype=np.int32)
        m = self.L.cholamd_plan_selinv_front(self.h, int(sep), int(block), 0, cols.ctypes.data, None, None)
        if m < 0:
            check(m, "cholamd_plan_selinv_front")
        pos = np.zeros(max(m, 1), dtype=np.int32)
        off = np.zeros((max(m, 1), max(m, 1)), dtype=np.int64)
        m2 = self.L.cholamd_plan_selinv_front(self.h, int(sep), int(block), m, cols.ctypes.data, pos.ctypes.data, off.ctypes.data)
        if m2 < 0:
            check(m2, "cholamd_plan_selinv_front")
        return int(cols[0]), int(cols[1]), pos[:m], off[:m, :m]

    def exchange_pieces(self, world, dist_top=2):
        out = np.zeros((4096, 4), dtype=np.int64)
        n = self.L.cholamd_plan_exchange_pieces(self.h, world, dist_top, len(out), out.ctypes.data)
        if n < 0:
            check(n, "cholamd_plan_exchange_pieces")
        return out[:min(n, len(out))]

    def level_work_volume(self, level, rank=0, world=1, dist_top=2):
        out = np.zeros(6, dtype=np.int64)
        check(self.L.cholamd_plan_level_work_volume(self.h, level, rank, world, dist_top, out.ctypes.data), "cholamd_plan_level_work_volume")
        return tuple(int(v) for v in out)

    def level_work_volume_opts(self, level, merge_targets=1, mt_min_tiles=-1):
        out = np.zeros(9, dtype=np.int64)
        check(self.L.cholamd_plan_level_work_volume_opts(self.h, level, int(merge_targets), int(mt_min_tiles), out.ctypes.data), "cholamd_plan_level_work_volume_opts")
        return tuple(int(v) for v in out)

    def level_mt_fill(self, level):
        out = np.zeros(4, dtype=np.int64)
        check(self.L.cholamd_plan_level_mt_fill(self.h, level, out.ctypes.data), "cholamd_plan_level_mt_fill")
        return tuple(int(v) for v in out)

    def program_check(self, follow=True, workers=64):
        check(self.L.cholamd_plan_program_check(self.h, int(follow), int(workers)), "cholamd_plan_program_check")

    def program_check_opts(self, follow_tail=-1, split_min=-1, split_nb=-1, workers=64):
        check(self.L.cholamd_plan_program_check_opts(self.h, follow_tail, split_min, split_nb, int(workers)), "cholamd_plan_program_check_opts")

    def program_counts(self, follow=True):
        out = np.zeros(6, dtype=np.int32)
        check(self.L.cholamd_plan_program_counts(self.h, int(follow), out.ctypes.data), "cholamd_plan_program_counts")
        return dict(zip(("jobs", "followers", "tasks", "strips", "counters", "followed_panels"), (int(v) for v in out)))

    def program_jobs(self, follow=True):
        need = self.L.cholamd_plan_program_jobs(self.h, int(follow), 0, None)
        buf = np.zeros(need, dtype=np.int32)
        self.L.cholamd_plan_program_jobs(self.h, int(follow), need, buf.ctypes.data)
        nj = int(buf[-1])
        return buf[:8 * nj].reshape(nj, 8), buf[8 * nj:-1].reshape(-1, 3)

    SCHUR_RECORD = 7

    def schur_size(self, k):
        m = self.L.cholamd_plan_schur_size(self.h, int(k))
        if m < 0:
            check(m, "cholamd_plan_schur_size")
        return m

    def schur_dofs(self, k):
        m = self.schur_size(k)
        out = np.zeros(max(m, 1), dtype=np.int32)
        check(min(self.L.cholamd_plan_schur_dofs(self.h, int(k), out.ctypes.data), 0), "cholamd_plan_schur_dofs")
        return out[:m]

    def schur_list(self, k):
        cnt = self.L.cholamd_plan_schur_list(self.h, int(k), 0, None)
        if cnt < 0:
            check(cnt, "cholamd_plan_schur_list")
        out = np.zeros((max(cnt, 1), self.SCHUR_RECORD), dtype=np.int64)
        check(min(self.L.cholamd_plan_schur_list(self.h, int(k), cnt, out.ctypes.data), 0), "cholamd_plan_schur_list")
        return out[:cnt]

    def schur_host(self, k, arena, lds=None):
        arena = np.ascontiguousarray(arena, dtype=np.float64)
        assert arena.size == self.arena_doubles
        m = self.schur_size(k)
        ld = m if lds is None else int(lds)
        buf = np.full((max(m, 1), max(ld, 1)), np.nan, dtype=np.float64)
        check(self.L.cholamd_plan_schur_host(self.h, int(k), arena.ctypes.data, buf.ctypes.data, ld), "cholamd_plan_schur_host")
        return buf[:m, :].T if lds is not None else buf[:m, :m].T

    @staticmethod
    def _colmajor(M, rows, ld, fill):
        k = M.shape[1]
        buf = np.full((max(k, 1), max(ld, 1)), fill, dtype=np.float64)
        buf[:k, :rows] = M.T
        return buf

    def schur_condense_host_nrhs(self, k, arena, B, ldb=None, ldw=None, ldg=None):
        arena = np.ascontiguousarray(arena, dtype=np.float64)
        assert arena.size == self.arena_doubles
        B = np.asarray(B, dtype=np.float64)
        assert B.ndim == 2 and B.shape[0] == self.n
        n, m, c = self.n, self.schur_size(k), B.shape[1]
        ldb, ldw, ldg = int(ldb or n), int(ldw or n), int(ldg or m)
        bb = self._colmajor(B, n, ldb, -3.0)
        wb, gb = np.full((max(c, 1), max(ldw, 1)), np.nan), np.full((max(c, 1), max(ldg, 1)), np.nan)
        check(self.L.cholamd_plan_schur_condense_host_nrhs(self.h, int(k), arena.ctypes.data, bb.ctypes.data, ldb, wb.ctypes.data, ldw, gb.ctypes.data, ldg, c),
              "cholamd_plan_schur_condense_host_nrhs")
        assert np.isnan(wb[:, n:]).all() and np.isnan(gb[:, m:]).all(), "rows behind W or G were written"
        return wb[:c, :n].T.copy(), gb[:c, :m].T.copy()

    def schur_expand_host_nrhs(self, k, arena, W, XT, ldw=None, ldxt=None, ldx=None):
        arena = np.ascontiguousarray(arena, dtype=np.float64)
        assert arena.size == self.arena_doubles
        W, XT = np.asarray(W, dtype=np.float64), np.asarray(XT, dtype=np.float64)
        n, m = self.n, self.schur_size(k)
        assert W.ndim == 2 and W.shape[0] == n and XT.ndim == 2 and XT.shape == (m, W.shape[1])
        c = W.shape[1]
        ldw, ldxt, ldx = int(ldw or n), int(ldxt or m), int(ldx or n)
        wb, tb = self._colmajor(W, n, ldw, -3.0), self._colmajor(XT, m, ldxt, -3.0)
        w0 = wb.copy()
        xb = np.full((max(c, 1), max(ldx, 1)), np.nan)
        check(self.L.cholamd_plan_schur_expand_host_nrhs(self.h, int(k), arena.ctypes.data, wb.ctypes.data, ldw, tb.ctypes.data, ldxt, xb.ctypes.data, ldx, c),
              "cholamd_plan_schur_expand_host_nrhs")
        assert np.isnan(xb[:, n:]).all(), "rows n .. ldx - 1 of X were written"
        assert wb.tobytes() == w0.tobytes(), "the expand wrote W"
        return xb[:c, :n].T.copy()

    def schur_det_counts(self, k):
# ... 159 lines not shown
```

### include/cholamd.h

```cpp
#ifndef CHOLAMD_H
#define CHOLAMD_H

#include <stdint.h>
#include <stdio.h>

#ifdef __cplusplus
extern "C" {
#endif

#define CHOLAMD_OK 0
#define CHOLAMD_ERR_IO (-1)
#define CHOLAMD_ERR_FORMAT (-2)
#define CHOLAMD_ERR_INVARIANT (-3)
#define CHOLAMD_ERR_ARG (-4)
#define CHOLAMD_ERR_NO_DEVICE (-5)
#define CHOLAMD_ERR_HIP (-6)
#define CHOLAMD_ERR_NOMEM (-7)
#define CHOLAMD_ERR_COMM (-9)
#define CHOLAMD_ERR_STALL (-8)

const char *cholamd_last_error(void);
const char *cholamd_version(void);

typedef char MM_typecode[4];
// ... 9 lines not shown
int mm_read_mtx_crd_size(FILE *f, int *M, int *N, int *nz);
int mm_write_banner(FILE *f, MM_typecode matcode);
int mm_write_mtx_crd_size(FILE *f, int M, int N, int nz);
char *mm_typecode_to_str(MM_typecode matcode);

typedef struct cholamd_sepinfo { int levels; int num_separators; } cholamd_sepinfo;

int cholamd_read_separators(const char *file, int dim, int *idx_out, int *sep_out, cholamd_sepinfo *info);

int cholamd_read_clusters(const char *file, int *idx_out, int *interval_out, int *sep_out, int64_t cap, int64_t *count_out);

int cholamd_read_matrix(const char *file, int nz, int *row_out, int *col_out, double *val_out);

int cholamd_read_vector(const char *file, int n, double *out);

typedef struct cholamd_plan cholamd_plan;

typedef struct cholamd_filled {
  int filled;
  int sep_x, sep_y;
  int interval;
  int cluster;
  int lo_x, lo_y, hi_x, hi_y;
} cholamd_filled;

typedef struct cholamd_op {
  int op;
  int level;
  int m, n, k;
  int a_sx, a_sy, a_z;
  int b_sx, b_sy, b_z;
  int c_sx, c_sy, c_z;
} cholamd_op;

int cholamd_plan_create(const char *matrix_file, const char *separator_file, const char *clusters_file, cholamd_plan **out);
int cholamd_plan_create_from_arrays(int n, int levels, const int *perm, const int *sep_sizes,
                                    const int *cl_idx, const int *cl_interval, const int *cl_sep, int64_t cl_count,
                                    int64_t nz, const int *a_row, const int *a_col, const double *a_val,
                                    const char *banner, cholamd_plan **out);
void cholamd_plan_destroy(cholamd_plan *p);

int cholamd_plan_n(const cholamd_plan *p);
int cholamd_plan_nz(const cholamd_plan *p);
int cholamd_plan_levels(const cholamd_plan *p);
int cholamd_plan_num_separators(const cholamd_plan *p);
int cholamd_plan_max_int_size(const cholamd_plan *p);
int cholamd_plan_num_blocks(const cholamd_plan *p);
int64_t cholamd_plan_arena_doubles(const cholamd_plan *p);
int64_t cholamd_plan_arena_dense_doubles(const cholamd_plan *p);
int cholamd_plan_block_tile_map(const cholamd_plan *p, int r, int c, int *out);
int64_t cholamd_plan_dropped_entries(const cholamd_plan *p);
const char *cholamd_plan_banner(const cholamd_plan *p);
void cholamd_plan_perm(const cholamd_plan *p, int *out);
void cholamd_plan_sep_sizes(const cholamd_plan *p, int *out);
void cholamd_plan_sep_offsets(const cholamd_plan *p, int *out);
void cholamd_plan_tree(const cholamd_plan *p, int *out);
void cholamd_plan_blocks(const cholamd_plan *p, int *out);
int64_t cholamd_plan_snapshot_count(const cholamd_plan *p, int interval_lbl);
void cholamd_plan_snapshot(const cholamd_plan *p, int interval_lbl, cholamd_filled *out);
int64_t cholamd_plan_num_ops(const cholamd_plan *p);
void cholamd_plan_ops(const cholamd_plan *p, cholamd_op *out);
void cholamd_plan_counts(const cholamd_plan *p, int level , int64_t calls[4], double flops[4]);
double cholamd_plan_flops(const cholamd_plan *p);
int64_t cholamd_plan_nnz_a(const cholamd_plan *p);
int64_t cholamd_plan_nnz_l(const cholamd_plan *p);
int64_t cholamd_plan_nnz_tiles(const cholamd_plan *p);
double cholamd_plan_fmin(const cholamd_plan *p);
int64_t cholamd_plan_alg_bytes(const cholamd_plan *p);

int cholamd_plan_fill_host(const cholamd_plan *p, double *arena);
int cholamd_plan_entries(const cholamd_plan *p, int *row, int *col);
int cholamd_plan_value_map(const cholamd_plan *p, int64_t *src_out);
int cholamd_plan_fill_host_values(const cholamd_plan *p, const double *vals, int64_t count, double *arena);
int cholamd_plan_diag_list(const cholamd_plan *p, int64_t *a_off, int *cols, int *lda, int *x_off, int *sep, int *prefix);
int cholamd_plan_fill_host_part(const cholamd_plan *p, double *arena, int rank, int world, int64_t *tail_offset_out);
int cholamd_plan_level_work_counts(const cholamd_plan *p, int level, int rank, int world, int out[4]);
int cholamd_plan_level_work_volume_opts(const cholamd_plan *p, int level, int merge_targets, int mt_min_tiles, int64_t out[9]);
int cholamd_plan_level_mt_fill(const cholamd_plan *p, int level, int64_t out[4]);
int cholamd_plan_level_work_volume(const cholamd_plan *p, int level, int rank, int world, int dist_top, int64_t out[6]);
int cholamd_plan_exchange_volume(const cholamd_plan *p, int rank, int world, int dist_top, int64_t out[4]);
int cholamd_plan_exchange_pieces(const cholamd_plan *p, int world, int dist_top, int max, int64_t (*out)[4]);
int cholamd_plan_program_check(const cholamd_plan *p, int follow, int workers);
int cholamd_plan_program_check_opts(const cholamd_plan *p, int follow_tail, int split_min, int split_nb, int workers);
int cholamd_plan_program_counts(const cholamd_plan *p, int follow, int out[6]);
int cholamd_follow_rounds(int n_ext, int tile_columns, int cap, int *rounds_out, int *own_at_out);
int64_t cholamd_plan_program_followers(const cholamd_plan *p, int64_t cap, int *out);
int64_t cholamd_plan_program_jobs(const cholamd_plan *p, int follow, int64_t cap, int *out);
int cholamd_plan_arena_to_dense(const cholamd_plan *p, const double *arena, double *dense);
int cholamd_plan_write_matrix(const cholamd_plan *p, const double *arena, const char *file, int full_precision);
int cholamd_write_solution(const char *file, const double *x, int n, int full_precision);
int cholamd_plan_write_debug_log(const cholamd_plan *p, FILE *f);
int cholamd_plan_write_debug_header(const cholamd_plan *p, FILE *f);
int cholamd_plan_write_blocks_txt(const cholamd_plan *p, const double *arena, const char *file, const char *header);
int cholamd_plan_ntiles_at_level(const cholamd_plan *p, int sep, int level);

typedef struct cholamd_problem cholamd_problem;
int cholamd_generate_laplacian(int nx, int ny, int nz, int levels, int tile, cholamd_problem **out);
void cholamd_problem_destroy(cholamd_problem *g);
int cholamd_problem_n(const cholamd_problem *g);
int cholamd_problem_nz(const cholamd_problem *g);
int cholamd_problem_write(const cholamd_problem *g, const char *prefix);
int cholamd_plan_create_from_problem(const cholamd_problem *g, cholamd_plan **out);
void cholamd_problem_rhs(const cholamd_problem *g, double *b);

typedef struct cholamd_device cholamd_device;

int cholamd_device_count(void);
int cholamd_device_create(const cholamd_plan *plan, int device_id, cholamd_device **out);
void cholamd_device_destroy(cholamd_device *d);
int cholamd_device_alloc(cholamd_device *d, int64_t doubles, double **dptr);
int cholamd_device_free(cholamd_device *d, double *dptr);
int cholamd_device_upload(cholamd_device *d, double *d_dst, const double *h_src, int64_t doubles, void *stream);
int cholamd_device_download(cholamd_device *d, double *h_dst, const double *d_src, int64_t doubles, void *stream);
int cholamd_device_sync(cholamd_device *d, void *stream);
int cholamd_device_fill(cholamd_device *d, double *d_arena, void *stream);
#define CHOLAMD_VALUES_NOCHECK 1
int cholamd_device_set_values(cholamd_device *d, const double *d_vals, int64_t count, int flags, void *stream);
int cholamd_device_values_status(cholamd_device *d, void *stream, int64_t out[4]);
int cholamd_factor(cholamd_device *d, double *d_arena, void *stream);
int cholamd_factor_levels(cholamd_device *d, double *d_arena, int level_hi, int level_lo, void *stream);
int cholamd_device_set_partition(cholamd_device *d, int rank, int world);
int cholamd_device_program_trace(cholamd_device *d, double *d_arena, void *stream, int64_t cap, int64_t *out, int *njobs_out);
int64_t cholamd_debug_live_buffers(void);
int cholamd_factor_debug(cholamd_device *d, double *d_arena, const char *dir, int full_precision, void *stream);
int cholamd_factor_info(cholamd_device *d, int *sep_out);
int cholamd_device_set_option(cholamd_device *d, const char *name, int value);
int cholamd_device_bcast_phases(const cholamd_device *d);
int cholamd_solve(cholamd_device *d, const double *d_arena, const double *d_b, double *d_x, void *stream);
int cholamd_plan_solve_det_host(const cholamd_plan *p, const double *arena_host, int which, const double *b, double *x);
int cholamd_plan_solve_det_host_nrhs(const cholamd_plan *p, const double *arena_host, int which, const double *B, int64_t ldb, double *X, int64_t ldx, int nrhs);
int cholamd_plan_solve_det_counts(const cholamd_plan *p, int64_t out[8]);
int cholamd_plan_solve_det_lists(const cholamd_plan *p, int which, int64_t *steps, int64_t *items, int64_t *srcs);
int cholamd_device_fill_f32(cholamd_device *d, float *d_arena32, void *stream);
int cholamd_factor_f32(cholamd_device *d, float *d_arena32, void *stream);
int cholamd_factor_levels_f32(cholamd_device *d, float *d_arena32, int level_hi, int level_lo, void *stream);
int cholamd_solve_f32(cholamd_device *d, const float *d_arena32, const double *d_b, double *d_x, void *stream);
int cholamd_solve_refine(cholamd_device *d, const float *d_arena32, const double *d_b, double *d_x, int max_iter, double tol,
                         int *iters_out, double *relres_out, void *stream);
int cholamd_residual(cholamd_device *d, const double *d_b, const double *d_x, double *d_r, double *relres_out, void *stream);
int cholamd_solve_nrhs(cholamd_device *d, const double *d_arena, const double *d_B, int64_t ldb, double *d_X, int64_t ldx, int nrhs, void *stream);
int cholamd_solve_nrhs_f32(cholamd_device *d, const float *d_arena32, const double *d_B, int64_t ldb, double *d_X, int64_t ldx, int nrhs, void *stream);
int cholamd_solve_refine_nrhs(cholamd_device *d, const float *d_arena32, const double *d_B, int64_t ldb, double *d_X, int64_t ldx, int nrhs, int max_iter,
                              double tol, int *iters_out, double *relres_out , void *stream);
#define CHOLAMD_PCG_X0 1
int cholamd_apply(cholamd_device *d, const double *d_x, double *d_y, void *stream);
int cholamd_apply_nrhs(cholamd_device *d, const double *d_X, int64_t ldx, double *d_Y, int64_t ldy, int nrhs, void *stream);
int cholamd_plan_apply_host(const cholamd_plan *p, const double *values , const double *x, double *y);
int cholamd_solve_pcg(cholamd_device *d, const double *d_arena, const double *d_b, double *d_x, int max_iter, double tol, int flags,
                      int *iters_out, double *relres_out, int *status_out, void *stream);
int cholamd_solve_pcg_f32(cholamd_device *d, const float *d_arena32, const double *d_b, double *d_x, int max_iter, double tol, int flags,
                          int *iters_out, double *relres_out, int *status_out, void *stream);
int cholamd_solve_pcg_nrhs(cholamd_device *d, const double *d_arena, const double *d_B, int64_t ldb, double *d_X, int64_t ldx, int nrhs, int max_iter, double tol, int flags,
                           int *iters_out, double *relres_out, int *status_out, void *stream);
int cholamd_solve_pcg_nrhs_f32(cholamd_device *d, const float *d_arena32, const double *d_B, int64_t ldb, double *d_X, int64_t ldx, int nrhs, int max_iter, double tol, int flags,
                               int *iters_out, double *relres_out, int *status_out, void *stream);
#define CHOLAMD_HALF_FORWARD  0
#define CHOLAMD_HALF_BACKWARD 1
int cholamd_solve_half(cholamd_device *d, const double *d_arena, const double *d_b, double *d_x, int which, void *stream);
int cholamd_solve_half_f32(cholamd_device *d, const float *d_arena32, const double *d_b, double *d_x, int which, void *stream);
int cholamd_solve_half_nrhs(cholamd_device *d, const double *d_arena, const double *d_B, int64_t ldb, double *d_X, int64_t ldx, int nrhs, int which, void *stream);
int cholamd_solve_half_nrhs_f32(cholamd_device *d, const float *d_arena32, const double *d_B, int64_t ldb, double *d_X, int64_t ldx, int nrhs, int which, void *stream);
int cholamd_factor_logdet(cholamd_device *d, const double *d_arena, double *logdet_out, void *stream);
int cholamd_factor_logdet_f32(cholamd_device *d, const float *d_arena32, double *logdet_out, void *stream);
int cholamd_factor_diag(cholamd_device *d, const double *d_arena, double *d_diag, void *stream);
int cholamd_factor_diag_f32(cholamd_device *d, const float *d_arena32, double *d_diag, void *stream);
int cholamd_multiply_half(cholamd_device *d, const double *d_arena, const double *d_z, double *d_y, int which, void *stream);
int cholamd_multiply_half_f32(cholamd_device *d, const float *d_arena32, const double *d_z, double *d_y, int which, void *stream);
int cholamd_multiply(cholamd_device *d, const double *d_arena, const double *d_z, double *d_y, void *stream);
int cholamd_multiply_f32(cholamd_device *d, const float *d_arena32, const double *d_z, double *d_y, void *stream);
// ... 153 lines not shown
```

Before: 833.9 GF/s.

## Let followed POTRF jobs fold their own tiles last, with the choice made per job by the scheduler

The scheduler now picks, for each following POTRF job, the external-item index at which it adds its own tiles. The choice is stored in the job's mode field, and jobs fed by early update cells defer their own tiles until after all external rounds. The kernel polls the job's own wait list while it processes external tiles and prefetches its own tiles into spare register slots, then folds them in, so the own-tile wait and load overlap the follow loop. The change also adds a round-boundary check on the chosen index and a host-side hazard analysis, at the cost of extra register pressure and more complex kernel control flow.

Result: faster. 853.2 GF/s, median of 6 (+2.3%).

```diff
diff --git a/cholesky_amd/_lib.py b/cholesky_amd/_lib.py
--- a/cholesky_amd/_lib.py
+++ b/cholesky_amd/_lib.py
@@ -128,6 +128,10 @@
     L.cholamd_follow_rounds.argtypes = [ci, ci, ci, vp, vp]
     L.cholamd_plan_program_followers.argtypes = [vp, i64, vp]
     L.cholamd_plan_program_followers.restype = i64
+    L.cholamd_plan_program_follow_own.argtypes = [vp, ci, ci, ci, ci, ci, i64, vp]
+    L.cholamd_plan_program_follow_own.restype = i64
+    L.cholamd_plan_program_check_follow.argtypes = [vp, ci, ci, ci, ci, ci, ci]
+    L.cholamd_plan_program_hazards.argtypes = [vp, ci, ci, ci, ci, ci, vp]
     L.cholamd_factor_multi_f32.argtypes = [vp, vp, vp, ci, vp]
     L.cholamd_gather_factor_f32.argtypes = [vp, vp, ci, vp]
     L.cholamd_device_alloc.argtypes = [vp, i64, C.POINTER(vp)]
diff --git a/cholesky_amd/csrc/chol_api.cpp b/cholesky_amd/csrc/chol_api.cpp
--- a/cholesky_amd/csrc/chol_api.cpp
+++ b/cholesky_amd/csrc/chol_api.cpp
@@ -215,6 +215,7 @@
   else if (n == "super_blocks") d->opt.super_blocks = value;
   else if (n == "follow_tail") d->opt.follow_tail = value;
   else if (n == "follow_tail_split") d->opt.follow_tail_split = value;
+  else if (n == "follow_own") d->opt.follow_own = value < 0 ? 0 : value > 2 ? 2 : value;
   else if (n == "staged") d->opt.staged = value != 0;
   else if (n == "fine_upd") d->opt.fine_upd = value != 0;
   else if (n == "skyline") d->opt.skyline = value != 0;
diff --git a/cholesky_amd/csrc/chol_kernels.hip b/cholesky_amd/csrc/chol_kernels.hip
--- a/cholesky_amd/csrc/chol_kernels.hip
+++ b/cholesky_amd/csrc/chol_kernels.hip
@@ -833,7 +833,8 @@
     if (b0 + lane < n) { const chol_wait wt = wl[b0 + lane]; ok = ok && __hip_atomic_load(&ctr[wt.ctr], __ATOMIC_RELAXED, __HIP_MEMORY_SCOPE_AGENT) >= wt.value + epoch * ctr_total[wt.ctr]; }
   return !__ballot(!ok);
 }
-struct follow_args { const chol_ext *ext; int n_ext; const int *ctr; const int *ctr_total; int epoch; const chol_wait *wl; int n_wl; unsigned long long *stamp, *xstamp; };
+struct follow_args { const chol_ext *ext; int n_ext; const int *ctr; const int *ctr_total; int epoch; const chol_wait *wl; int n_wl; unsigned long long *stamp, *xstamp;
+                     int own_at;  };
 __device__ __forceinline__ int ext_ready(const follow_args &f, int from, int lane)
 {
   bool ok = true;
@@ -856,11 +857,13 @@
 #ifndef FOLLOW_OWN_SLEEP
 #define FOLLOW_OWN_SLEEP 4
 #endif
-#ifndef FOLLOW_OWN_LAST_MAX
-#define FOLLOW_OWN_LAST_MAX 0
-#endif
   static_assert(CHOL_FOLLOW_PAIR_MAXT == RR_MAXT, "a pair of followed column tiles shares one LDS buffer of RR_MAXT tiles");
-  const int own_at = f.n_ext <= FOLLOW_OWN_LAST_MAX ? f.n_ext : chol_follow_own_at(f.n_ext, T);
+  const int own_at = f.own_at;
+  const bool own_last = f.n_wl > 0 && own_at >= f.n_ext;
+  bool own_ok = false;
+  int own_c = 0, own_need = 0, own_v = 0;
+  const bool own_look = !UPD && own_last && f.n_wl <= 64;
+  if (own_look && lane < f.n_wl) { const chol_wait wt = f.wl[lane]; own_c = wt.ctr; own_need = wt.value + f.epoch * f.ctr_total[wt.ctr]; }
 #define EXT_ROUND(I_) chol_follow_round(I_, f.n_ext, T)
 #define EXT_LOAD(I_, V_)                                                                                             \
   {                                                                                                                  \
@@ -953,7 +956,10 @@
       polled = true;
       if (j + lane < f.n_ext) { const int c = f.ext[j + lane].ctr; pv = __hip_atomic_load(&f.ctr[c], __ATOMIC_RELAXED, __HIP_MEMORY_SCOPE_AGENT); pneed = f.epoch * f.ctr_total[c] + f.ext[j + lane].need; }
     }
+    const bool look = own_look && !own_ok;
+    if (look && lane < f.n_wl) own_v = __hip_atomic_load(&f.ctr[own_c], __ATOMIC_RELAXED, __HIP_MEMORY_SCOPE_AGENT);
     lds_barrier();
+    if (look) own_ok = !__ballot(lane < f.n_wl && own_v < own_need);
     if (UPD) {
 #pragma unroll
       for (int it = 0; it < 3; ++it) {
@@ -975,7 +981,26 @@
     }
     i = j;
   }
-  if (f.n_wl > 0 && own_at >= f.n_ext) OWN_TILES();
+  if (own_last) {
+    if (!UPD && !own_ok) wait_list<FOLLOW_OWN_SLEEP>(f.wl, f.n_wl, f.ctr, f.ctr_total, f.epoch, lane, info);
+    if (TR && !UPD && f.xstamp && lane == 0) f.xstamp[0] = __builtin_amdgcn_s_memrealtime();
+    lds_barrier();
+    if (UPD) {
+      int rx = r15, gx = g;
+      asm volatile("" : "+v"(rx), "+v"(gx));
+#pragma unroll
+      for (int it = 0; it < 3; ++it) {
+        const int u = min(w + it * RR_NW, 2 * T - 2);
+        tile[FOLLOW_SLOTS + it] = load_tile<PUB>(A, lda, n, u < T ? u : u - T + 1, u < T ? 0 : 1, rx, gx);
+      }
+#pragma unroll
+      for (int s = 0; s < FOLLOW_SLOTS; ++s) {
+        const d4 zero4 = { 0.0, 0.0, 0.0, 0.0 };
+        tile[FOLLOW_SLOTS + 3 + s] = zero4;
+        if (ijp[s] != 0xffff) tile[FOLLOW_SLOTS + 3 + s] = load_tile<PUB>(A, lda, n, ijp[s] & 0xff, ijp[s] >> 8, rx, gx);
+      }
+    }
+  }
 #undef OWN_TILES
 #undef EXT_LOAD_ROUND
 #undef EXT_ROUND
@@ -1017,6 +1042,7 @@
 #define PSTAMP(i_) do { if (TR && fa.xstamp && fa.n_ext == 0 && tid == 64) fa.xstamp[24 + (i_)] = __builtin_amdgcn_s_memrealtime(); } while (0)
   PSTAMP(0);
   d4 stage[3];
+  const bool own_pending = FOLLOW && fa.n_ext > 0 && fa.n_wl > 0 && fa.own_at >= fa.n_ext;
   const bool stage_early = !(FOLLOW && fa.n_ext > 0) && wave != 0;
   if (stage_early) {
 #pragma unroll
@@ -1165,9 +1191,11 @@
         tile[s] = v;
       }
       follow_external<true, PUB, TR>(base, fa, T, n, smem + RR_OFF_SOL, tile, stage, ijp, w, lane, tid, info, A, lda, r15, g, &sFlag[5]);
-#pragma unroll
-      for (int s = FOLLOW_SLOTS; s < RR_RSLOTS; ++s) tile[s] = zero4;
       lds_barrier();
+      if (own_pending) {
+#pragma unroll
+        for (int it = 0; it < 3; ++it) stage[it] += tile[FOLLOW_SLOTS + it];
+      }
     } else {
     PSTAMP(6);
 #pragma unroll
@@ -1190,6 +1218,17 @@
         if (ti == 1) lds_set(tj == 0 ? fA : fD, 1, lane);
         if (tj == 0 && ti > 0) lds_inc(cRaw, lane);
       }
+    }
+    if (FOLLOW && fa.n_ext > 0) {
+      static_assert(FOLLOW_SLOTS + 3 + FOLLOW_SLOTS <= RR_RSLOTS, "a follower's own tiles in flight fit the register tiles it does not use");
+      if (own_pending) {
+        __builtin_amdgcn_sched_barrier(0);
+#pragma unroll
+        for (int s = 0; s < FOLLOW_SLOTS; ++s) tile[s] += tile[FOLLOW_SLOTS + 3 + s];
+      }
+      const d4 zero4 = { 0.0, 0.0, 0.0, 0.0 };
+#pragma unroll
+      for (int s = FOLLOW_SLOTS; s < RR_RSLOTS; ++s) tile[s] = zero4;
     }
     if (ijp[RR_RSLOTS] != 0xffff) {
       const d4 v = load_tile<PUB>(A, lda, n, ijp[RR_RSLOTS] & 0xff, ijp[RR_RSLOTS] >> 8, r15, g);
@@ -1723,7 +1762,7 @@
     if (jb.kind == 0) {
       const chol_potrf_desc pd = pdescs[jb.first];
       follow_args fa;
-      fa.ext = exts + jb.ext_first; fa.n_ext = jb.n_ext; fa.ctr = ctr; fa.ctr_total = ctr_total; fa.epoch = epoch; fa.wl = waits + jb.wait_first; fa.n_wl = jb.n_wait; fa.stamp = TR && trace ? &trace[4 * j + 1] : nullptr; fa.xstamp = TR && trace ? &trace[4 * njobs + CHOL_TRACE_X * j] : nullptr;
+      fa.ext = exts + jb.ext_first; fa.n_ext = jb.n_ext; fa.ctr = ctr; fa.ctr_total = ctr_total; fa.epoch = epoch; fa.wl = waits + jb.wait_first; fa.n_wl = jb.n_wait; fa.own_at = jb.mode; fa.stamp = TR && trace ? &trace[4 * j + 1] : nullptr; fa.xstamp = TR && trace ? &trace[4 * njobs + CHOL_TRACE_X * j] : nullptr;
       potrf_rr_body<true, true, TR>(base, ws, pd, info, ctr + pd.ctr, epoch * ctr_total[pd.ctr], smem, pdescs[jb.first].sky, fa, tid);
     } else if (jb.kind == 1) {
       double (*sX)[RR_MAXT][TS * TS] = (double (*)[RR_MAXT][TS * TS])smem;
diff --git a/cholesky_amd/csrc/chol_plan.h b/cholesky_amd/csrc/chol_plan.h
--- a/cholesky_amd/csrc/chol_plan.h
+++ b/cholesky_amd/csrc/chol_plan.h
@@ -147,6 +147,7 @@
 #define CHOL_FOLLOW_PAIR_MAXT 17
 #define CHOL_FOLLOW_SINGLE_TAIL 0
 #define CHOL_FOLLOW_OWN_BEFORE 2
+#define CHOL_FOLLOW_OWN 1
 #if defined(__HIPCC__)
 #define CHOL_HD __host__ __device__ __forceinline__
 #else
@@ -211,6 +212,7 @@
   int merge_targets;
   int leaf_envelope;
   int super_blocks;
+  int follow_own;
 } chol_sched_opts;
 #define CHOL_SUPER_BLOCKS 3
 #define CHOL_STAGE_CHUNK 0
diff --git a/cholesky_amd/csrc/chol_schedule.c b/cholesky_amd/csrc/chol_schedule.c
--- a/cholesky_amd/csrc/chol_schedule.c
+++ b/cholesky_amd/csrc/chol_schedule.c
@@ -93,7 +93,7 @@
 void chol_sched_opts_default(chol_sched_opts *o)
 {
   o->split_min = CHOL_SPLIT_MIN; o->split_nb = CHOL_SPLIT_NB; o->fuse = 1; o->fuse_update_max = CHOL_FUSE_UPDATE_MAX;
-  o->mt_min_tiles = CHOL_MT_MIN_TILES; o->trsm_wt_min = CHOL_TRSM_WT_MIN; o->trsm_group = 0; o->cells = 1; o->program = 1; o->follow = 1; o->super_blocks = CHOL_SUPER_BLOCKS; o->dist_top = 2; o->follow_tail = CHOL_FOLLOW_TAIL; o->follow_tail_split = CHOL_FOLLOW_TAIL; o->staged = 1; o->fine_upd = 1; o->skyline = 1; o->stage_chunk = CHOL_STAGE_CHUNK; o->merge_targets = 1; o->leaf_envelope = 1;
+  o->mt_min_tiles = CHOL_MT_MIN_TILES; o->trsm_wt_min = CHOL_TRSM_WT_MIN; o->trsm_group = 0; o->cells = 1; o->program = 1; o->follow = 1; o->super_blocks = CHOL_SUPER_BLOCKS; o->dist_top = 2; o->follow_tail = CHOL_FOLLOW_TAIL; o->follow_tail_split = CHOL_FOLLOW_TAIL; o->staged = 1; o->fine_upd = 1; o->skyline = 1; o->stage_chunk = CHOL_STAGE_CHUNK; o->merge_targets = 1; o->leaf_envelope = 1; o->follow_own = CHOL_FOLLOW_OWN;
 }
 void chol_sched_opts_from_env(chol_sched_opts *o)
 {
@@ -111,6 +111,7 @@
   o->super_blocks = env_int("CHOLAMD_SUPER_BLOCKS", o->super_blocks);
   o->follow_tail = env_int("CHOLAMD_FOLLOW_TAIL", o->follow_tail);
   o->follow_tail_split = env_int("CHOLAMD_FOLLOW_TAIL_SPLIT", o->follow_tail_split);
+  o->follow_own = env_int("CHOLAMD_FOLLOW_OWN", o->follow_own);
   o->staged = !env_int("CHOLAMD_NO_STAGED", 0);
   o->fine_upd = !env_int("CHOLAMD_NO_FINE_UPD", 0);
   o->skyline = !env_int("CHOLAMD_NO_SKYLINE", 0);
@@ -933,13 +934,13 @@
 #ifndef EARLY_CHUNK
 #define EARLY_CHUNK 2
 #endif
-static void emit_early_cells(pbuild *P, builder *B, const plan_t *p, int64_t c_off, int ldc, int lim, int blk, const early_src *es, int nes,
+static int emit_early_cells(pbuild *P, builder *B, const plan_t *p, int64_t c_off, int ldc, int lim, int blk, const early_src *es, int nes,
                              const int *c_upd, const int *c_updd, int *snap_upd, int *cnt_upd, int *cnt_updd)
 {
   chol_level_work *w = B->w;
   int nst = 0, maxch = 0;
   for (int q = 0; q < nes; q++) if (es[q].k > 0) { const int ch = ((es[q].k + CHOL_NB - 1) / CHOL_NB + EARLY_CHUNK - 1) / EARLY_CHUNK; nst += ch; if (ch > maxch) maxch = ch; }
-  if (nst == 0) return;
+  if (nst == 0) return 0;
   int *sc = malloc(nst * sizeof(int)), *sn = malloc(nst * sizeof(int)), *sq = malloc(nst * sizeof(int)), *sch = malloc(nst * sizeof(int));
   nst = 0;
   for (int c = 0; c < maxch; c++)
@@ -975,6 +976,7 @@
   snap_upd[col_sep] = cnt_upd[col_sep];
   emit_update_jobs(P, B, p, k0, c_upd, c_updd, snap_upd, cnt_upd, cnt_updd, sc, sn, nst, staged ? sq : NULL);
   free(sc); free(sn); free(sq); free(sch);
+  return w->n_task > k0;
 }
 
 static chol_sched_opts chol_program_opts(const chol_sched_opts *o)
@@ -1066,7 +1068,7 @@
     }
     est_start[p->tree[h]] = st0;
   }
-  #define EMIT_POTRF(s_, st_, ext_first_)                                                                        \
+  #define EMIT_POTRF(s_, st_, ext_first_, early_)                                                                       \
     do {                                                                                                          \
       pblock *b_ = &pb[s_][st_];                                                                                  \
       const int ld_ = p->panel_ld[s_];                                                                            \
@@ -1084,6 +1086,9 @@
       add_wait(P, c_updd[s_], cnt_updd[s_]);                                                                      \
       chol_job *j_ = add_job(P, 0, b_->potrf, 1, wf_);                                                            \
       j_->ext_first = (ext_first_); j_->n_ext = pg->n_ext - (ext_first_);                                         \
+      if (j_->n_ext > 0)                                                                                          \
+        j_->mode = j_->n_wait > 0 && (opts->follow_own == 2 || (opts->follow_own == 1 && (early_))) ? j_->n_ext   \
+                   : chol_follow_own_at(j_->n_ext, (b_->nb + CHOL_NB - 1) / CHOL_NB);                             \
       b_->emitted = 1;                                                                                            \
     } while (0)
 
@@ -1102,7 +1107,7 @@
     for (int st = 0; st < steps; st++) {
       for (int q = 0; q < nh; q++) {
         const int s = p->tree[hs[q]];
-        if (st < nblk_of[s] && !pb[s][st].emitted) EMIT_POTRF(s, st, pg->n_ext);
+        if (st < nblk_of[s] && !pb[s][st].emitted) EMIT_POTRF(s, st, pg->n_ext, 0);
       }
       for (int q = 0; q < nh; q++) {
         const int h = hs[q], s = p->tree[h], n = p->sep_size[s], ld = p->panel_ld[s];
@@ -1170,15 +1175,16 @@
           for (int i = (b->c0 + b->nb) / CHOL_NB; i * CHOL_NB < b->c0 + b->nb + nb1; i++) if (sky[s][i] < fmin) fmin = sky[s][i];
           if (fmin - b->c0 / CHOL_NB >= bt) bt = 0;
         }
+        int early = 0;
         if (bt > 0) {
           const early_src es = { e_off, ld, bt * CHOL_NB, b->ch_below + bt - 1, b->ns_below };
-          emit_early_cells(P, B, p, p->panel_off[s] + (b->c0 + b->nb) + (int64_t)(b->c0 + b->nb) * ld, ld, nb1, BIDX(p, s, s), &es, 1, c_upd, c_updd, snap_upd, cnt_upd, cnt_updd);
+          early = emit_early_cells(P, B, p, p->panel_off[s] + (b->c0 + b->nb) + (int64_t)(b->c0 + b->nb) * ld, ld, nb1, BIDX(p, s, s), &es, 1, c_upd, c_updd, snap_upd, cnt_upd, cnt_updd);
         }
         const int ef = pg->n_ext;
         push_ext_items(&items, &nit, &capit, e_off, ld, b->nb, b->ch_below, b->ns_below, 0, bt);
         for (int i = 0; i < nit; i++) add_ext(P, items[i].x);
         free(items);
-        EMIT_POTRF(s, st + 1, ef);
+        EMIT_POTRF(s, st + 1, ef, early);
       }
       {
         memcpy(snap_upd, cnt_upd, (ns + 1) * sizeof(int));
@@ -1334,16 +1340,17 @@
             before += nt;
           }
         }
+        int early = 0;
         if (nes > 0) {
           const chol_block *Bp = &p->blk[BIDX(p, par, par)];
-          emit_early_cells(P, B, p, Bp->off, Bp->ld, lim, BIDX(p, par, par), es, nes, c_upd, c_updd, snap_upd, cnt_upd, cnt_updd);
+          early = emit_early_cells(P, B, p, Bp->off, Bp->ld, lim, BIDX(p, par, par), es, nes, c_upd, c_updd, snap_upd, cnt_upd, cnt_updd);
         }
         qsort(items, nit, sizeof(ext_item), cmp_ext_item);
         for (int i = 0; i < nit; i++) add_ext(P, items[i].x);
         free(items);
         if (pg->n_ext == ef) continue;
         follow_lim[BIDX(p, par, par)] = pb[par][0].nb;
-        EMIT_POTRF(par, 0, ef);
+        EMIT_POTRF(par, 0, ef, early);
       }
     {
       int cap_u = 256, ntu = 0;
@@ -1511,6 +1518,11 @@
         if (val[wt->ctr] < wt->value) ok = 0;
       }
       if (rc) break;
+      if (jb->kind == 0 && jb->n_ext > 0) {
+        int at = 0;
+        while (at < jb->mode && at < jb->n_ext) at += chol_follow_round(at, jb->n_ext, (w.potrf[jb->first].n + CHOL_NB - 1) / CHOL_NB);
+        if (at != jb->mode) { chol_set_error("program job %d adds its own tiles at item %d of %d: not the start of a round", j, jb->mode, jb->n_ext); rc = CHOLAMD_ERR_ARG; break; }
+      }
       if (ok && jb->kind == 0)
         for (int x = 0; x < jb->n_ext && ok; x++) {
           const chol_ext *e = &g.ext[jb->ext_first + x];
@@ -1577,6 +1589,17 @@
   if (split_nb >= 0) o.split_nb = split_nb;
   return chol_program_check(p, &o, workers);
 }
+int cholamd_plan_program_check_follow(const cholamd_plan *p, int follow_tail, int follow_tail_split, int follow_own, int split_min, int split_nb, int workers)
+{
+  chol_sched_opts o;
+  chol_sched_opts_from_env(&o);
+  if (follow_tail >= 0) o.follow_tail = follow_tail;
+  if (follow_tail_split >= 0) o.follow_tail_split = follow_tail_split;
+  if (follow_own >= 0) o.follow_own = follow_own;
+  if (split_min >= 0) o.split_min = split_min;
+  if (split_nb >= 0) o.split_nb = split_nb;
+  return chol_program_check(p, &o, workers);
+}
 int64_t cholamd_plan_program_jobs(const cholamd_plan *p, int follow, int64_t cap, int *out)
 {
   chol_sched_opts o;
@@ -1625,6 +1648,135 @@
   }
   chol_level_work_free(&w); chol_program_free(&g);
   return n;
+}
+int64_t cholamd_plan_program_follow_own(const cholamd_plan *p, int follow_tail, int follow_tail_split, int follow_own, int split_min, int split_nb, int64_t cap, int *out)
+{
+  chol_sched_opts o;
+  chol_sched_opts_default(&o);
+  if (follow_tail >= 0) o.follow_tail = follow_tail;
+  if (follow_tail_split >= 0) o.follow_tail_split = follow_tail_split;
+  if (follow_own >= 0) o.follow_own = follow_own;
+  if (split_min >= 0) o.split_min = split_min;
+  if (split_nb >= 0) o.split_nb = split_nb;
+  chol_level_work w; chol_program g;
+  if (chol_build_program(p, &o, &w, &g)) return -1;
+  int64_t n = 0;
+  for (int j = 0; j < g.n_job; j++) {
+    const chol_job *jb = &g.job[j];
+    if (jb->kind != 0 || jb->n_ext <= 0) continue;
+    if (5 * n + 4 < cap) { out[5 * n] = j; out[5 * n + 1] = jb->n_ext; out[5 * n + 2] = (w.potrf[jb->first].n + CHOL_NB - 1) / CHOL_NB; out[5 * n + 3] = jb->mode; out[5 * n + 4] = jb->n_wait; }
+    n++;
+  }
+  chol_level_work_free(&w); chol_program_free(&g);
+  return n;
+}
+typedef struct { int job, add; } hz_sig;
+int cholamd_plan_program_hazards(const cholamd_plan *p, int follow_tail, int follow_tail_split, int follow_own, int split_min, int split_nb, int out[4])
+{
+  chol_sched_opts o;
+  chol_sched_opts_default(&o);
+  if (follow_tail >= 0) o.follow_tail = follow_tail;
+  if (follow_tail_split >= 0) o.follow_tail_split = follow_tail_split;
+  if (follow_own >= 0) o.follow_own = follow_own;
+  if (split_min >= 0) o.split_min = split_min;
+  if (split_nb >= 0) o.split_nb = split_nb;
+  chol_level_work w; chol_program g;
+  int rc = chol_build_program(p, &o, &w, &g);
+  if (rc) return rc;
+  const int nj = g.n_job, nw = (nj + 63) / 64;
+  int *ns = calloc(g.n_ctr + 1, sizeof(int)), *first = calloc(g.n_ctr + 2, sizeof(int));
+  hz_sig *sg = NULL;
+  for (int pass = 0; pass < 2; pass++) {
+    if (pass) { for (int c = 0; c < g.n_ctr; c++) { first[c + 1] = first[c] + ns[c]; ns[c] = 0; } sg = malloc((first[g.n_ctr] + 1) * sizeof(hz_sig)); }
+#define HZ_SIG(C_, J_, ADD_) do { if (pass) { hz_sig s_ = { J_, ADD_ }; sg[first[C_] + ns[C_]] = s_; } ns[C_]++; } while (0)
+    for (int j = 0; j < nj; j++) {
+      const chol_job *jb = &g.job[j];
+      if (jb->kind == 0) HZ_SIG(w.potrf[jb->first].ctr, j, g.ctr_total[w.potrf[jb->first].ctr]);
+      if (jb->kind == 1)
+        for (int t = 0; t < (w.trsm[jb->first].n + CHOL_NB - 1) / CHOL_NB; t++) {
+          int add = 0;
+          for (int i = jb->first; i < jb->first + jb->n; i++) add += w.trsm[i].chan >= 0 && w.trsm[i].m > 0;
+          if (add > 0) HZ_SIG(w.trsm[jb->first].chan + t, j, add);
+        }
+      for (int q = 0; q < 2; q++) if (jb->sig[q] >= 0 && jb->sig_add > 0) HZ_SIG(jb->sig[q], j, jb->sig_add);
+    }
+#undef HZ_SIG
+  }
+  int nwt = 0;
+  for (int j = 0; j < nj; j++) nwt += g.job[j].n_wait + (g.job[j].kind == 0 ? g.job[j].n_ext : g.job[j].kind == 1 ? 1 : 0);
+  typedef struct { int job, ctr, value, gating; } hz_wait;
+  hz_wait *wt = malloc((nwt + 1) * sizeof(hz_wait));
+  int *nwc = calloc(g.n_ctr + 1, sizeof(int)), *wfirst = calloc(g.n_ctr + 2, sizeof(int)), *wof = malloc((nwt + 1) * sizeof(int));
+  nwt = 0;
+  for (int j = 0; j < nj; j++) {
+    const chol_job *jb = &g.job[j];
+    for (int q = 0; q < jb->n_wait; q++) { hz_wait x = { j, g.wait[jb->wait_first + q].ctr, g.wait[jb->wait_first + q].value, jb->kind != 2 || q < jb->n_pre }; wt[nwt++] = x; }
+    if (jb->kind == 0) for (int q = 0; q < jb->n_ext; q++) { hz_wait x = { j, g.ext[jb->ext_first + q].ctr, g.ext[jb->ext_first + q].need, 1 }; wt[nwt++] = x; }
+    if (jb->kind == 1) { hz_wait x = { j, w.trsm[jb->first].flag, 1, 1 }; wt[nwt++] = x; }
+  }
+  for (int i = 0; i < nwt; i++) nwc[wt[i].ctr]++;
+  for (int c = 0; c < g.n_ctr; c++) { wfirst[c + 1] = wfirst[c] + nwc[c]; nwc[c] = 0; }
+  for (int i = 0; i < nwt; i++) wof[wfirst[wt[i].ctr] + nwc[wt[i].ctr]++] = i;
+  uint64_t *pre = calloc((size_t)nj * nw + 1, sizeof(uint64_t)), *start = calloc((size_t)nj * nw + 1, sizeof(uint64_t));
+  int *reqv = malloc((first[g.n_ctr] + 1) * sizeof(int));
+#define HZ_HAS(S_, J_, A_) ((S_[(size_t)(J_) * nw + (A_) / 64] >> ((A_) % 64)) & 1)
+  for (int changed = 1, sweep = 0; changed && sweep < 64; sweep++) {
+    changed = 0;
+    for (int c = 0; c < g.n_ctr; c++) {
+      for (int y = first[c]; y < first[c + 1]; y++) {
+        int m = 0;
+        for (int z = wfirst[c]; z < wfirst[c + 1]; z++) {
+          const hz_wait *x = &wt[wof[z]];
+          if (x->value > m && (x->job == sg[y].job || HZ_HAS(pre, sg[y].job, x->job))) m = x->value;
+        }
+        reqv[y] = m;
+      }
+      for (int z = wfirst[c]; z < wfirst[c + 1]; z++) {
+        const hz_wait *x = &wt[wof[z]];
+        uint64_t *pj = pre + (size_t)x->job * nw, *sj = start + (size_t)x->job * nw;
+        for (int a = first[c]; a < first[c + 1]; a++) {
+          const int A = sg[a].job;
+          if (HZ_HAS(pre, x->job, A) && (!x->gating || HZ_HAS(start, x->job, A))) continue;
+          int f = 0;
+          for (int y = first[c]; y < first[c + 1] && f < x->value; y++) if (sg[y].job != A && reqv[y] < x->value && !HZ_HAS(pre, sg[y].job, A)) f += sg[y].add;
+          if (f >= x->value) continue;
+          const uint64_t *pa = pre + (size_t)A * nw;
+          for (int k = 0; k < nw; k++) {
+            const uint64_t add = pa[k] | (k == A / 64 ? (uint64_t)1 << (A % 64) : 0);
+            if (add & ~pj[k]) { pj[k] |= add; changed = 1; }
+            if (x->gating && (add & ~sj[k])) { sj[k] |= add; changed = 1; }
+          }
+        }
+      }
+    }
+  }
+  free(wt); free(nwc); free(wfirst); free(wof); free(reqv);
+  int *last = malloc((size_t)(p->arena > 0 ? p->arena : 1) * sizeof(int));
+  for (int64_t e = 0; e < p->arena; e++) last[e] = -1;
+  uint64_t *seen = calloc((size_t)nj * nw + 1, sizeof(uint64_t));
+  out[0] = out[1] = 0; out[2] = out[3] = -1;
+  for (int j = 0; j < nj; j++) {
+    const chol_job *jb = &g.job[j];
+    if (jb->kind != 2) continue;
+    for (int t = jb->first; t < jb->first + jb->n; t++) {
+      const chol_upd_task *tk = &w.task[t];
+      for (int col = 0; col < tk->nv; col++)
+        for (int r = 0; r < tk->mv; r++) {
+          const int64_t e = tk->c_off + r + (int64_t)col * tk->ldc;
+          if (e < 0 || e >= p->arena) { chol_set_error("program task %d writes outside the arena", t); rc = CHOLAMD_ERR_ARG; continue; }
+          const int a = last[e];
+          last[e] = j;
+          if (a < 0 || a == j || HZ_HAS(seen, j, a)) continue;
+          seen[(size_t)j * nw + a / 64] |= (uint64_t)1 << (a % 64);
+          out[0]++;
+          if (!HZ_HAS(start, j, a)) { if (out[1]++ == 0) { out[2] = a; out[3] = j; } }
+        }
+    }
+  }
+#undef HZ_HAS
+  free(last); free(seen); free(pre); free(start); free(sg); free(ns); free(first);
+  chol_level_work_free(&w); chol_program_free(&g);
+  return rc;
 }
 int cholamd_plan_program_counts(const cholamd_plan *p, int follow, int out[6])
 {
diff --git a/cholesky_amd/plan.py b/cholesky_amd/plan.py
--- a/cholesky_amd/plan.py
+++ b/cholesky_amd/plan.py
@@ -258,8 +258,22 @@
     def program_check(self, follow=True, workers=64):
         check(self.L.cholamd_plan_program_check(self.h, int(follow), int(workers)), "cholamd_plan_program_check")
 
-    def program_check_opts(self, follow_tail=-1, split_min=-1, split_nb=-1, workers=64):
-        check(self.L.cholamd_plan_program_check_opts(self.h, follow_tail, split_min, split_nb, int(workers)), "cholamd_plan_program_check_opts")
+    def program_check_opts(self, follow_tail=-1, split_min=-1, split_nb=-1, workers=64, follow_tail_split=-1, follow_own=-1):
+        check(self.L.cholamd_plan_program_check_follow(self.h, follow_tail, follow_tail_split, follow_own, split_min, split_nb, int(workers)),
+              "cholamd_plan_program_check_follow")
+
+    def program_follow_own(self, follow_own=-1, follow_tail=-1, follow_tail_split=-1, split_min=-1, split_nb=-1):
+        n = self.L.cholamd_plan_program_follow_own(self.h, follow_tail, follow_tail_split, follow_own, split_min, split_nb, 0, None)
+        if n < 0:
+            check(int(n), "cholamd_plan_program_follow_own")
+        buf = np.zeros(5 * n + 5, dtype=np.int32)
+        self.L.cholamd_plan_program_follow_own(self.h, follow_tail, follow_tail_split, follow_own, split_min, split_nb, buf.size, buf.ctypes.data)
+        return [dict(zip(("job", "n_ext", "T", "own_at", "n_wait"), (int(v) for v in buf[5 * i:5 * i + 5]))) for i in range(n)]
+
+    def program_hazards(self, follow_own=-1, follow_tail=-1, follow_tail_split=-1, split_min=-1, split_nb=-1):
+        out = np.zeros(4, dtype=np.int32)
+        check(self.L.cholamd_plan_program_hazards(self.h, follow_tail, follow_tail_split, follow_own, split_min, split_nb, out.ctypes.data), "cholamd_plan_program_hazards")
+        return int(out[0]), int(out[1]), (int(out[2]), int(out[3]))
 
     def program_counts(self, follow=True):
         out = np.zeros(6, dtype=np.int32)
diff --git a/include/cholamd.h b/include/cholamd.h
--- a/include/cholamd.h
+++ b/include/cholamd.h
@@ -115,9 +115,12 @@
 int cholamd_plan_exchange_pieces(const cholamd_plan *p, int world, int dist_top, int max, int64_t (*out)[4]);
 int cholamd_plan_program_check(const cholamd_plan *p, int follow, int workers);
 int cholamd_plan_program_check_opts(const cholamd_plan *p, int follow_tail, int split_min, int split_nb, int workers);
+int cholamd_plan_program_check_follow(const cholamd_plan *p, int follow_tail, int follow_tail_split, int follow_own, int split_min, int split_nb, int workers);
 int cholamd_plan_program_counts(const cholamd_plan *p, int follow, int out[6]);
 int cholamd_follow_rounds(int n_ext, int tile_columns, int cap, int *rounds_out, int *own_at_out);
 int64_t cholamd_plan_program_followers(const cholamd_plan *p, int64_t cap, int *out);
+int64_t cholamd_plan_program_follow_own(const cholamd_plan *p, int follow_tail, int follow_tail_split, int follow_own, int split_min, int split_nb, int64_t cap, int *out);
+int cholamd_plan_program_hazards(const cholamd_plan *p, int follow_tail, int follow_tail_split, int follow_own, int split_min, int split_nb, int out[4]);
 int64_t cholamd_plan_program_jobs(const cholamd_plan *p, int follow, int64_t cap, int *out);
 int cholamd_plan_arena_to_dense(const cholamd_plan *p, const double *arena, double *dense);
 int cholamd_plan_write_matrix(const cholamd_plan *p, const double *arena, const char *file, int full_precision);
```
